# jnbraun/bcnn

Hardware: AMD Instinct MI355X
Metric: images/sec fwd+bwd (higher is better)
Workload: dtype f32; 1 GPU; ResNet-18 224x224 (BASELINE configs[2]), N=128 per GPU, fwd+bwd+SGD through bcnn_net C API; CIFAR-example topology + ImageNet stem, fc-1000; batch_per_gpu=128, global_batch=128, parallelism=dp1, comm=none (one rank)

## Files before the change

bcnn_amd/_lib.py:

```python
import ctypes as C
import os
import subprocess

_HERE = os.path.dirname(os.path.abspath(__file__))
LIB_PATH = os.environ.get("BCNN_HIP_LIB", os.path.join(_HERE, "lib", "libbcnn_hip.so"))
CSRC = os.path.join(_HERE, "csrc")

vp, i, f, sz, u64 = C.c_void_p, C.c_int, C.c_float, C.c_size_t, C.c_uint64

SIGNATURES = {
    "bcnn_hip_device_count": (i, []),
    "bcnn_hip_set_device": (None, [i]),
    "bcnn_hip_get_device": (i, []),
    "bcnn_hip_device_name": (C.c_char_p, []),
    "bcnn_hip_malloc_f32": (vp, [sz]),
    "bcnn_hip_malloc_i32": (vp, [sz]),
    "bcnn_hip_free": (None, [vp]),
    "bcnn_hip_memcpy_h2d": (None, [vp, vp, sz]),
    "bcnn_hip_memcpy_d2h": (None, [vp, vp, sz]),
    "bcnn_hip_memcpy_d2d": (None, [vp, vp, sz]),
    "bcnn_hip_fill_f32": (None, [vp, sz, f]),
    "bcnn_hip_sync": (None, []),
    "bcnn_hip_stream_create": (vp, []),
    "bcnn_hip_stream_destroy": (None, [vp]),
# ... 28 lines not shown
    "bcnn_hip_activation_backward": (None, [vp, vp, sz, i, vp, vp, i, i]),
    "bcnn_hip_activation_forward_keep": (None, [vp, vp, sz, i]),
    "bcnn_hip_activation_backward_from_input": (None, [vp, vp, sz, i]),
    "bcnn_hip_scale_channels_forward": (None, [vp, vp, vp, i, i, i, i]),
    "bcnn_hip_scale_channels_backward": (None, [vp, vp, vp, vp, vp, i, i, i, i]),
    "bcnn_hip_group_norm_forward": (None, [vp] * 6 + [i, i, i, i, f]),
    "bcnn_hip_group_norm_backward": (None, [vp] * 8 + [i, i, i, i, i]),
    "bcnn_hip_group_norm_path": (i, [i, i, i, i, i]),
    "bcnn_hip_batchnorm_forward": (None, [vp] * 10 + [i, i, i, i, i]),
    "bcnn_hip_batchnorm_backward": (None, [vp, vp, vp, i] + [vp] * 9 + [i, i, i]),
    "bcnn_hip_conv_workspace_size": (sz, [i] * 9),
    "bcnn_hip_conv_forward": (None, [vp, vp, vp, vp] + [i] * 10 + [vp, i, vp, vp, vp, vp, vp, vp, vp, i]),
    "bcnn_hip_conv_forward_bf16": (i, [vp, vp, vp, vp] + [i] * 10 + [vp, i, vp, vp, vp, vp, vp, vp, vp, i]),
    "bcnn_hip_conv_backward": (None, [vp] * 8 + [i] * 10 + [vp, vp, i] + [vp] * 8 + [vp, sz]),
    "bcnn_hip_maxpool_forward": (None, [vp, vp, vp] + [i] * 8),
    "bcnn_hip_maxpool_backward": (None, [vp, vp, vp] + [i] * 9),
    "bcnn_hip_avgpool_forward": (None, [vp, vp, i, i, i, i]),
    "bcnn_hip_avgpool_backward": (None, [vp, vp, i, i, i, i]),
    "bcnn_hip_pool2d_out_extent": (i, [vp, i]),
    "bcnn_hip_pool2d_forward": (None, [vp, vp, vp, vp, i, i, i, i]),
    "bcnn_hip_pool2d_backward": (None, [vp, vp, vp, vp, i, i, i, i, i]),
    "bcnn_hip_depthwise_forward": (None, [vp, vp, vp, vp] + [i] * 8),
    "bcnn_hip_depthwise_backward": (None, [vp] * 7 + [i] * 9),
    "bcnn_hip_depthwise_stats_size": (sz, [i] * 7),
    "bcnn_hip_depthwise_forward_stats": (i, [vp, vp, vp, vp] + [i] * 8 + [vp, sz]),
    "bcnn_hip_batchnorm_forward_stats": (None, [vp] * 10 + [i, i, i, i, i, vp, i]),
    "bcnn_hip_batchnorm_forward_stats_only": (None, [vp] * 7 + [i, i, i, vp, i]),
    "bcnn_hip_conv_bnfold_fusable": (i, [i] * 5), "bcnn_hip_conv_set_input_bnfold": (None, [vp] * 4),
    "bcnn_hip_depthwise_bn_fusable": (i, [i] * 8),
    "bcnn_hip_batchnorm_backward_sums": (None, [vp] * 9 + [i, i, i]),
    "bcnn_hip_depthwise_backward_bn": (None, [vp] * 7 + [i] * 9 + [vp] * 5),
    "bcnn_hip_batchnorm_backward_apply": (None, [vp] * 8 + [i, i, i]),
    "bcnn_hip_depthwise_bnin_fusable": (i, [i] * 9),
    "bcnn_hip_conv_bnsums_size": (sz, [i] * 4),
    "bcnn_hip_conv_backward_bnsums": (i, [vp] * 8 + [i] * 10 + [vp, vp, i] + [vp] * 8 + [vp, sz] + [vp, vp, vp, sz]),
    "bcnn_hip_batchnorm_backward_finalize": (None, [vp, i] + [vp] * 6 + [i]),
    "bcnn_hip_depthwise_forward_bnin": (i, [vp, vp, vp, vp] + [i] * 8 + [vp, sz] + [vp] * 4 + [i]),
    "bcnn_hip_depthwise_backward_bnin": (None, [vp] * 7 + [i] * 9 + [vp] * 4 + [i]),
    "bcnn_hip_depthwise_backward_bn_bnin": (None, [vp] * 7 + [i] * 9 + [vp] * 5 + [vp] * 4 + [i]),
    "bcnn_hip_conv_residual_fusable": (i, [i, i, i, i, vp, vp, vp]),
    "bcnn_hip_conv_forward_residual": (None, [vp, vp, vp] + [i] * 9 + [vp] * 7 + [sz, i, vp]),
    "bcnn_hip_conv_backward_residual": (None, [vp] * 7 + [i] * 9 + [vp] * 7 + [vp, sz, vp, vp, i, vp, vp, sz]),
    "bcnn_hip_batchnorm_apply": (None, [vp] * 6 + [i, i, i, i]),
    "bcnn_hip_conv_prepack": (None, [vp, i, i]),
    "bcnn_hip_maxpool_forward_bn_keep": (None, [vp, vp, vp] + [i] * 8 + [vp] * 4 + [i, vp]),
    "bcnn_hip_maxpool_bn_backward_fusable": (i, [i] * 9 + [vp] * 4),
    "bcnn_hip_maxpool_bn_backward": (None, [vp] * 5 + [i] * 8 + [vp] * 8 + [i]),
    "bcnn_hip_conv_backward_bn_done": (None, [vp] * 5 + [i] * 9 + [vp, sz]),
    "bcnn_hip_depthwise_insums_size": (sz, [i] * 7),
    "bcnn_hip_depthwise_backward_bnin_sums": (i, [vp] * 7 + [i] * 9 + [vp] * 5 + [vp] * 4 + [i] + [vp, sz]),
    "bcnn_hip_conv_backward_presummed": (i, [vp] * 8 + [i] * 10 + [vp, vp, i] + [vp] * 8 + [vp, sz] + [vp, i] + [vp, vp, vp, sz]),
    "bcnn_hip_conv_prepack_reset": (None, []),
    "bcnn_hip_conv_prepack_discard": (None, []),
    "bcnn_hip_maxpool_bn_fusable": (i, [i] * 9 + [vp]),
    "bcnn_hip_conv_forward_stats_only": (None, [vp, vp, vp] + [i] * 9 + [vp] * 6),
    "bcnn_hip_maxpool_forward_bn": (None, [vp, vp, vp] + [i] * 8 + [vp] * 4 + [i]),
    "bcnn_hip_sgd_update": (None, [vp, vp, vp, vp, sz, sz, i, f, f, f]),
    "bcnn_hip_sgd_update_chunks": (None, [vp, i, i, f, f, f]),
    "bcnn_hip_zero_chunks": (None, [vp, i]),
    "bcnn_hip_adam_update": (None, [vp, vp, vp, vp, vp, vp, sz, sz, i, i, f, f, f, f, f]),
    "bcnn_hip_eltwise_forward": (None, [vp, vp, vp, sz, sz, i]),
    "bcnn_hip_eltwise_backward": (None, [vp, vp, vp, vp, sz, sz, i, i]),
    "bcnn_hip_cost_metric": (None, [i, vp, vp, vp, i, i, vp]),
    "bcnn_hip_axpy_strided": (None, [i, f, vp, vp] + [i] * 11),
    "bcnn_hip_add_rowvec": (None, [vp, vp, i, i]),
    "bcnn_hip_softmax_forward": (None, [vp, vp, i, i, i]),
    "bcnn_hip_concat_forward": (None, [i, vp, vp, vp, i, i]),
    "bcnn_hip_concat_backward": (None, [i, vp, vp, vp, i, i]),
    "bcnn_hip_upsample_forward": (None, [vp, vp, i, i, i, i, i]),
    "bcnn_hip_upsample_backward": (None, [vp, vp, i, i, i, i, i]),
    "bcnn_hip_yolo_activate": (None, [vp, vp, i, i, i, i, i]),
    "bcnn_hip_yolo_nms_capacity": (i, []),
    "bcnn_hip_yolo_detect_result_words": (sz, [i, i, i]),
    "bcnn_hip_yolo_detect_batch": (i, [vp, i, i, vp, i, i, i, i, f, i, f, i, i, vp]),
    "bcnn_hip_yolo_train_workspace_size": (sz, [vp]),
    "bcnn_hip_yolo_train_forward": (i, [vp, vp, vp, vp, vp, vp, vp]),
    "bcnn_hip_fill_images": (i, [vp, i, i, i, i, i, vp, vp, vp, vp, i, f, i, f, f, f]),
    "bcnn_hip_jpeg_stage_begin": (i, [i, i, i, i, i, vp, i, vp, vp]),
    "bcnn_hip_jpeg_stage_run": (i, [vp, f, i, f, f, f]),
    "bcnn_hip_jpeg_stage_cancel": (None, []),
    "bcnn_hip_augment_batch": (i, [vp, i, i, i, i, i, i, i, vp, vp, vp, i]),
    "bcnn_hip_augment_label_batch": (i, [vp, i, i, i, i, vp, vp, vp, i]),
    "bcnn_hip_augment_jpeg_begin": (i, [i, i, i, i, i, vp, vp]),
    "bcnn_hip_augment_jpeg_run": (i, [vp, vp, vp, vp, vp, vp, i]),
    "bcnn_hip_augment_jpeg_cancel": (None, []),
    "bcnn_hip_augment_letterbox_batch": (i, [vp, i, i, i, i, i, vp, vp, vp, i]),
    "bcnn_hip_augment_effects_begin": (i, [i, i, i, vp, vp, vp, vp, i, vp, sz]),
    "bcnn_hip_augment_effects_cancel": (None, []),
    "bcnn_hip_deconv_workspace_size": (sz, [i] * 8),
    "bcnn_hip_deconv_forward": (None, [vp, vp, vp, vp] + [i] * 9),
    "bcnn_hip_deconv_backward": (None, [vp] * 7 + [i] * 9 + [vp, sz]),
    "bcnn_hip_dilated_conv_workspace_size": (sz, [i] * 10),
    "bcnn_hip_dilated_conv_forward": (None, [vp, vp, vp, vp] + [i] * 11),
    "bcnn_hip_dilated_conv_backward": (None, [vp] * 7 + [i] * 11 + [vp, sz]),
    "bcnn_hip_dilated_depthwise_workspace_size": (sz, [i] * 8),
    "bcnn_hip_dilated_depthwise_forward": (None, [vp, vp, vp, vp] + [i] * 9),
    "bcnn_hip_dilated_depthwise_backward": (None, [vp] * 7 + [i] * 10 + [vp, sz]),
    "bcnn_hip_dilated_depthwise_path": (i, [i] * 9),
    "bcnn_hip_interp_forward": (None, [vp, vp, vp, i, i, i, i]),
    "bcnn_hip_interp_backward": (None, [vp, vp, vp, i, i, i, i, i]),
    "bcnn_hip_interp_axis_taps": (None, [i, i, i, vp, vp, vp]),
    "bcnn_hip_softmax_loss_forward": (None, [vp, vp, vp, vp, vp, i, i, i]),
    "bcnn_hip_softmax_loss_backward": (None, [vp, vp, vp, vp, vp, i, i, i, i]),
    "bcnn_hip_softmax_loss_confusion": (None, [vp, vp, vp, vp, i, i, i]),
    "bcnn_hip_softmax_loss_c_reg": (i, []),
    "bcnn_hip_label_map_fit": (i, [i, i, i, i, i, vp]),
    "bcnn_hip_label_maps_plan": (i, [vp, i, i, i, i, i, vp, vp, vp]),
    "bcnn_hip_label_maps_batch": (i, [vp, i, i, i, i, i, vp, i, vp, vp, vp, vp, i, vp, vp, vp]),
    "bcnn_hip_label_maps_kernel_ms": (f, [i]),
    "bcnn_hip_lrn_forward": (None, [vp, vp] + [i] * 5 + [f] * 3),
    "bcnn_hip_lrn_backward": (None, [vp, vp, vp] + [i] * 5 + [f] * 3 + [i]),
    "bcnn_hip_dropout_forward": (None, [vp, sz, f, u64, u64]),
    "bcnn_hip_dropout_backward": (None, [vp, sz, f, u64, u64]),
    "bcnn_hip_lifted_struct_workspace_size": (sz, [i, i]),
    "bcnn_hip_lifted_struct_forward": (None, [vp, vp, vp, i, i, f, i, vp, vp]),
    "bcnn_hip_lifted_struct_backward": (None, [vp, i, i, f, vp]),
    "bcnn_hip_comm_init": (None, [i, i, C.c_char_p]),
    "bcnn_hip_comm_destroy": (None, []),
    "bcnn_hip_comm_retain": (None, []),
# ... 46 lines not shown
```

bcnn_amd/csrc/blas1.hip:

```cpp
#include "chan_reduce.h"

namespace bcnn_hip {

template <class Op>
__global__ __launch_bounds__(256) void map2_kernel(const float* __restrict__ x, float* __restrict__ y,
                                                   size_t n, Op op) {
    const size_t i = (size_t)blockIdx.x * blockDim.x + threadIdx.x;
    const size_t stride = (size_t)gridDim.x * blockDim.x;
    const bool al = ((reinterpret_cast<uintptr_t>(x) | reinterpret_cast<uintptr_t>(y)) & 15) == 0;
    if (al) {
        const size_t n4 = n / 4;
        const float4* x4 = reinterpret_cast<const float4*>(x);
        float4* y4 = reinterpret_cast<float4*>(y);
        for (size_t j = i; j < n4; j += stride) {
            const float4 a = x4[j];
            float4 b = y4[j];
            b.x = op(a.x, b.x); b.y = op(a.y, b.y); b.z = op(a.z, b.z); b.w = op(a.w, b.w);
            y4[j] = b;
        }
        for (size_t j = n4 * 4 + i; j < n; j += stride) y[j] = op(x[j], y[j]);
    } else {
        for (size_t j = i; j < n; j += stride) y[j] = op(x[j], y[j]);
    }
}
// ... 102 lines not shown
}

__global__ __launch_bounds__(256) void adam_kernel(float* __restrict__ w, float* __restrict__ g,
                                                   float* __restrict__ m, float* __restrict__ v, size_t n, float wd_b,
                                                   float one_m_b1, float b1, float one_m_b2, float b2, float step) {
    const size_t stride = (size_t)gridDim.x * blockDim.x;
    for (size_t i = (size_t)blockIdx.x * blockDim.x + threadIdx.x; i < n; i += stride) {
        float gi = g[i], wi = w[i];
        gi = __fadd_rn(__fmul_rn(wi, wd_b), gi);
        const float mi = __fadd_rn(__fmul_rn(one_m_b1, gi), __fmul_rn(b1, m[i]));
        const float vi = __fadd_rn(__fmul_rn(one_m_b2, __fmul_rn(gi, gi)), __fmul_rn(b2, v[i]));
        m[i] = mi;
        v[i] = vi;
        const float q = __fdiv_rn(mi, __fadd_rn(sqrtf(vi), 0.0000001f));
        w[i] = __fadd_rn(__fmul_rn(q, step), wi);
        g[i] = 0.f;
    }
}

__global__ __launch_bounds__(256) void sgd_chunks_kernel(const bcnn_hip_sgd_chunk* __restrict__ chunks, float wd_b,
                                                         float neg_lr_b, float momentum) {
    const bcnn_hip_sgd_chunk ch = chunks[blockIdx.x];
    const float wd = ch.use_decay ? wd_b : 0.f;
    for (unsigned i = threadIdx.x; i < ch.count; i += 256) {
        float gi = ch.g_d[i], wi = ch.w_d[i];
        if (wd != 0.f) gi = __fadd_rn(__fmul_rn(wi, wd), gi);
        wi = __fadd_rn(__fmul_rn(gi, neg_lr_b), wi);
        ch.w_d[i] = wi;
        ch.g_d[i] = (momentum == 0.0f) ? 0.f : ((momentum == 1.0f) ? gi : gi * momentum);
    }
}

__global__ __launch_bounds__(256) void zero_chunks_kernel(const bcnn_hip_fill_chunk* __restrict__ chunks) {
    const bcnn_hip_fill_chunk ch = chunks[blockIdx.x];
    float* p = ch.p_d;
    const unsigned n = ch.count;
    unsigned head = (unsigned)(((16 - (reinterpret_cast<uintptr_t>(p) & 15)) & 15) / 4);
    if (head > n) head = n;
    if (threadIdx.x < head) p[threadIdx.x] = 0.f;
    float4* b4 = reinterpret_cast<float4*>(p + head);
    const unsigned nb = n - head, n4 = nb / 4;
    for (unsigned j = threadIdx.x; j < n4; j += 256) b4[j] = make_float4(0.f, 0.f, 0.f, 0.f);
    for (unsigned j = n4 * 4 + threadIdx.x; j < nb; j += 256) p[head + j] = 0.f;
}

}

using namespace bcnn_hip;

extern "C" {

void bcnn_hip_axpy(size_t n, float a, const float* x, float* y) {
    if (!n) return;
    map2_kernel<<<stream_grid(n / 4 + 1, 256), 256, 0, current_stream()>>>(x, y, n, AxpyOp{a});
    KERNEL_CHECK();
}

void bcnn_hip_scal(size_t n, float a, float* x) {
    if (!n) return;
    if (a == 0.0f) { HIP_CHECK(hipMemsetAsync(x, 0, n * sizeof(float), current_stream())); return; }
    if (a == 1.0f) return;
    map2_kernel<<<stream_grid(n / 4 + 1, 256), 256, 0, current_stream()>>>((const float*)x, x, n, ScalOp{a});
    KERNEL_CHECK();
}

void bcnn_hip_copy_f32(size_t n, const float* x, float* y) {
    if (!n || x == y) return;
    HIP_CHECK(hipMemcpyAsync(y, x, n * sizeof(float), hipMemcpyDeviceToDevice, current_stream()));
}

void bcnn_hip_add_bias(float* y, const float* bias, int n, int c, int hw) {
    launch_chan_map(ChanMapBody{y, bias, 0, (reinterpret_cast<uintptr_t>(y) & 15) == 0}, n, c, hw);
}

void bcnn_hip_scales(float* y, const float* scales, int n, int c, int hw) {
    launch_chan_map(ChanMapBody{y, scales, 1, (reinterpret_cast<uintptr_t>(y) & 15) == 0}, n, c, hw);
}

void bcnn_hip_grad_bias(float* dbias, const float* g, int n, int c, int hw) {
    const long long M = (long long)n * hw;
    if (!M || !c) return;
    const int splits = chan_splits(c, M);
    float* part = scratch(SCRATCH_REDUCE, (size_t)c * splits);
    if ((reinterpret_cast<uintptr_t>(g) & 15) == 0) launch_chan_reduce<1>(SumF{g}, c, hw, M, splits, part);
    else launch_chan_reduce<1>(SumUnalignedF{g}, c, hw, M, splits, part);
    chan_accumulate_kernel<<<ceil_div(c, 256), 256, 0, current_stream()>>>(part, c, splits, dbias);
    KERNEL_CHECK();
}

}

namespace bcnn_hip {
void activation_backward_grad_bias(const float* y, float* dy, float* dbias, int n, int c, int hw, int act) {
    const long long M = (long long)n * hw;
    if (!M || !c) return;
    const bool al = ((reinterpret_cast<uintptr_t>(y) | reinterpret_cast<uintptr_t>(dy)) & 15) == 0;
    if (act == BCNN_HIP_ACT_NONE || !act_bwd_is_cheap(act) || act == BCNN_HIP_ACT_PRELU || !al) {
        bcnn_hip_activation_backward(y, dy, (size_t)(M * c), act, nullptr, nullptr, hw, c);
        bcnn_hip_grad_bias(dbias, dy, n, c, hw);
        return;
    }
    const int splits = chan_splits(c, M);
    float* part = scratch(SCRATCH_REDUCE, (size_t)c * splits);
    launch_chan_reduce<1>(ActBwdSumF{y, dy, act}, c, hw, M, splits, part);
    chan_accumulate_kernel<<<ceil_div(c, 256), 256, 0, current_stream()>>>(part, c, splits, dbias);
    KERNEL_CHECK();
}
}

extern "C" {

void bcnn_hip_grad_scales(const float* x_norm, const float* g, int n, int c, int hw, float* dscales) {
    const long long M = (long long)n * hw;
    if (!M || !c) return;
    const int splits = chan_splits(c, M);
    float* part = scratch(SCRATCH_REDUCE, (size_t)c * splits);
    if (((reinterpret_cast<uintptr_t>(x_norm) | reinterpret_cast<uintptr_t>(g)) & 15) == 0)
        launch_chan_reduce<1>(DotF{g, x_norm}, c, hw, M, splits, part);
    else launch_chan_reduce<1>(DotUnalignedF{g, x_norm}, c, hw, M, splits, part);
    chan_accumulate_kernel<<<ceil_div(c, 256), 256, 0, current_stream()>>>(part, c, splits, dscales);
// ... 54 lines not shown
```

bcnn_amd/csrc/common.h:

```cpp
#pragma once
#include <hip/hip_runtime.h>

#include <cstdio>
#include <cstdlib>

#include "../../include/bcnn_hip.h"

#define HIP_CHECK(expr)                                                                        \
    do {                                                                                       \
        hipError_t _e = (expr);                                                                \
        if (_e != hipSuccess) {                                                                \
            fprintf(stderr, "[bcnn_hip] %s:%d: %s failed: %s\n", __FILE__, __LINE__, #expr,    \
                    hipGetErrorString(_e));                                                    \
            exit((int)_e);                                                                     \
        }                                                                                      \
    } while (0)

#define KERNEL_CHECK() HIP_CHECK(hipGetLastError())

#ifdef BCNN_HIP_EXPERIMENT
#define BCNN_EXP_ENV(name) getenv(name)
#else
#define BCNN_EXP_ENV(name) ((const char*)nullptr)
#endif

namespace bcnn_hip {

hipStream_t current_stream();
void set_current_stream(hipStream_t st);

constexpr int kMaxDevices = 64;
int current_device();

enum ScratchSlot {
    SCRATCH_REDUCE,
    SCRATCH_BN_CONSTS,
    SCRATCH_FOLD_ROWCONST,
    SCRATCH_COL,
    SCRATCH_DMA,
    SCRATCH_DMA_DW,
    SCRATCH_WINO,
    SCRATCH_WINO_DW,
    SCRATCH_WINO43_U,
    SCRATCH_WINO43_TAIL,
    SCRATCH_WFUSED_U,
    SCRATCH_WFUSED_TAIL,
    SCRATCH_W43FF_U,
    SCRATCH_W43FF_TAIL,
    SCRATCH_DETECT,
    SCRATCH_IMAGES,
    SCRATCH_AUGMENT,
    SCRATCH_INTERP,
    SCRATCH_SOFTMAX_LOSS,
    SCRATCH_AUGMENT_LABEL,
    SCRATCH_LABEL_MAP,
    SCRATCH_SLOTS
};
float* scratch(ScratchSlot slot, size_t floats);
inline float4* scratch_f4(ScratchSlot slot, size_t n) { return reinterpret_cast<float4*>(scratch(slot, n * 4)); }

enum StageSlot {
    STAGE_IMAGES,
    STAGE_AUGMENT,
    STAGE_AUGMENT_LABEL,
    STAGE_LABEL_MAP,
    STAGE_SLOTS
};
uint8_t* host_stage(StageSlot slot, size_t bytes);
uint8_t* host_stage_extend(StageSlot slot, size_t keep, size_t bytes);
uint8_t* stage_upload(StageSlot slot, ScratchSlot device_slot, size_t upload_bytes, size_t device_bytes, hipStream_t st);
uint64_t stage_generation(StageSlot slot);

void activation_backward_grad_bias(const float* y, float* dy, float* dbias, int n, int c, int hw, int act);

enum KClass { K_CONV_FWD = 0, K_CONV_DW, K_CONV_DX, K_BN_FWD, K_BN_BWD, K_POOL, K_ELTWISE_ACT, K_GEMM, K_SGD,
              K_DEPTHWISE_FWD, K_DEPTHWISE_BWD,
              K_CONV_FWD_WINO, K_CONV_DX_WINO, K_CONV_DW_WINO,
              K_CONV_FWD_WINO43, K_CONV_DX_WINO43,
              K_CONV_DW_WINO43,
              K_NUM };
struct KTimer {
    int idx;
    KTimer(int cls, double flops, double bytes, double useful_flops = -1.0);
    ~KTimer();
};

extern thread_local bool g_trace_on;
void trace_kernel_slow(const char* name);
inline void trace_kernel(const char* name) { if (g_trace_on) trace_kernel_slow(name); }
inline void trace_kernel_count(const char* prefix, int count) {
    if (!g_trace_on) return;
    char name[64];
    snprintf(name, sizeof(name), "%s%d", prefix, count);
    trace_kernel_slow(name);
}

constexpr int kWave = 64;
constexpr int kCUs = 256;
constexpr int kXCDs = 8;

inline int ceil_div(long long a, long long b) { return (int)((a + b - 1) / b); }
inline size_t align_up(size_t v, size_t a) { return (v + a - 1) / a * a; }
inline bool al16(const void* p) { return (reinterpret_cast<uintptr_t>(p) & 15) == 0; }

#ifndef STREAM_GRID_PER_CU
#define STREAM_GRID_PER_CU 8
#endif
inline int stream_grid(size_t work_items, int block) {
    size_t need = (work_items + block - 1) / block;
    size_t cap = (size_t)kCUs * STREAM_GRID_PER_CU;
    if (need < 1) need = 1;
    return (int)(need < cap ? need : cap);
}

struct FastDiv {
    unsigned d, magic;
};
inline FastDiv make_fdiv(unsigned d, unsigned long long max_dividend) {
// ... 122 lines not shown
```

bcnn_amd/csrc/conv.hip:

```cpp
#include "batchnorm.h"
#include "conv_paths.h"
#include <algorithm>
#include <cstring>
#include <vector>

namespace bcnn_hip {
static thread_local BnFold g_fold_pending = {nullptr, nullptr, nullptr, nullptr};
static BnFold take_fold() {
    const BnFold f = g_fold_pending;
    g_fold_pending = BnFold{nullptr, nullptr, nullptr, nullptr};
    return f;
}
static bool bnfold_shape_ok(const ConvShape& s) {
    return s.ksz == 1 && s.stride == 1 && s.pad == 0 && s.groups == 1 && conv_dma_fwd_wanted(s) &&
           conv_dw_dma_workspace_floats(s) > 0;
}
__global__ __launch_bounds__(256) void bnfold_rowconst_kernel(const float* __restrict__ w, const BnFold fold, int F, int C,
                                                              float* __restrict__ rowc) {
    const int f = blockIdx.x * 4 + (threadIdx.x >> 6), lane = threadIdx.x & 63;
    if (f >= F) return;
    double acc = 0.0;
    for (int c = lane; c < C; c += 64) {
        float bv = fold.bias[c];
        if (bv == 1.0f) bv = 0.f;
        const float b = bv - fold.mean[c] * bnfold_a(fold.var, fold.scales, c);
        acc += (double)w[(size_t)f * C + c] * (double)b;
    }
#pragma unroll
    for (int o = 32; o > 0; o >>= 1) acc += __shfl_xor(acc, o);
    if (lane == 0) rowc[f] = (float)acc;
}
static float* fold_rowconst(const BnFold& fold, const float* w, int C, int F) {
    float* rowc = scratch(SCRATCH_FOLD_ROWCONST, (size_t)F);
    bnfold_rowconst_kernel<<<ceil_div(F, 4), 256, 0, current_stream()>>>(w, fold, F, C, rowc);
    KERNEL_CHECK();
    return rowc;
}


struct SideStream {
    hipStream_t stream = nullptr;
    hipEvent_t ready = nullptr, done = nullptr;
    bool pending = false;
};
static thread_local SideStream g_side[kMaxDevices];
static thread_local int g_side_mode = 0;
bool conv_side_stream_deferred() { return g_side_mode == 2; }
static SideStream* side_stream() {
    SideStream& ss = g_side[current_device()];
    if (ss.stream == nullptr) {
        int prio_lo = 0, prio_hi = 0;
        HIP_CHECK(hipDeviceGetStreamPriorityRange(&prio_lo, &prio_hi));
        HIP_CHECK(hipStreamCreateWithPriority(&ss.stream, hipStreamNonBlocking, BCNN_EXP_ENV("BCNN_HIP_SIDE_PRIO_SAME") ? prio_hi : prio_lo));
        HIP_CHECK(hipEventCreateWithFlags(&ss.ready, hipEventDisableTiming));
        HIP_CHECK(hipEventCreateWithFlags(&ss.done, hipEventDisableTiming));
    }
    return &ss;
}

struct PrepackEntry {
    const float* w;
    int kind, mode;
    float* buf;
    size_t cap, floats;
    unsigned long long epoch;
    bool fresh;
};
struct PrepackStore {
    std::vector<PrepackEntry> entries;
    unsigned long long epoch = 0;
    int dev = -1;
    void* table_dev[PREPACK_KINDS][2] = {{nullptr, nullptr}, {nullptr, nullptr}};
    size_t table_cap[PREPACK_KINDS][2] = {{0, 0}, {0, 0}};
    std::vector<char> table_host[PREPACK_KINDS][2];
};
static thread_local PrepackStore g_prepack;

float* prepack_take(const float* w, int kind, int mode, size_t floats) {
    PrepackStore& st = g_prepack;
    for (PrepackEntry& e : st.entries)
        if (e.w == w && e.kind == kind && e.mode == mode && e.fresh && e.epoch == st.epoch && e.floats == floats) {
            e.fresh = false;
            return e.buf;
        }
    return nullptr;
}

static void prepack_free_all(PrepackStore& st) {
    HIP_CHECK(hipDeviceSynchronize());
    for (PrepackEntry& e : st.entries)
        if (e.buf) HIP_CHECK(hipFree(e.buf));
    st.entries.clear();
    for (int k = 0; k < PREPACK_KINDS; ++k)
        for (int m = 0; m < 2; ++m) {
            if (st.table_dev[k][m]) HIP_CHECK(hipFree(st.table_dev[k][m]));
            st.table_dev[k][m] = nullptr;
            st.table_cap[k][m] = 0;
            st.table_host[k][m].clear();
        }
}

static PrepackEntry* prepack_entry(PrepackStore& st, const float* w, int kind, int mode, size_t floats) {
    PrepackEntry* e = nullptr;
    for (PrepackEntry& c : st.entries)
        if (c.w == w && c.kind == kind && c.mode == mode) { e = &c; break; }
    if (!e) {
        st.entries.push_back(PrepackEntry{w, kind, mode, nullptr, 0, 0, 0, false});
        e = &st.entries.back();
    }
    if (e->cap < floats) {
        if (e->buf) {
            HIP_CHECK(hipStreamSynchronize(current_stream()));
            HIP_CHECK(hipFree(e->buf));
        }
        HIP_CHECK(hipMalloc((void**)&e->buf, floats * sizeof(float)));
        e->cap = floats;
    }
    e->floats = floats;
    e->epoch = st.epoch;
    e->fresh = true;
    return e;
}

static const void* prepack_table(PrepackStore& st, int kind, int mode, const void* jobs, size_t bytes) {
    std::vector<char>& host = st.table_host[kind][mode];
    if (host.size() == bytes && memcmp(host.data(), jobs, bytes) == 0) return st.table_dev[kind][mode];
    HIP_CHECK(hipStreamSynchronize(current_stream()));
    if (st.table_cap[kind][mode] < bytes) {
        if (st.table_dev[kind][mode]) HIP_CHECK(hipFree(st.table_dev[kind][mode]));
        HIP_CHECK(hipMalloc(&st.table_dev[kind][mode], bytes * 2));
        st.table_cap[kind][mode] = bytes * 2;
    }
    HIP_CHECK(hipMemcpy(st.table_dev[kind][mode], jobs, bytes, hipMemcpyHostToDevice));
    host.assign((const char*)jobs, (const char*)jobs + bytes);
    return st.table_dev[kind][mode];
}

enum ConvGate { GATE_NONE, GATE_WINDOW, GATE_DMA, GATE_SMALLC_DX, GATE_COUNT };
static bool gate_open(ConvGate g) {
    static const bool off[GATE_COUNT] = {false, BCNN_EXP_ENV("BCNN_HIP_NO_WINDOW") != nullptr,
                                         BCNN_EXP_ENV("BCNN_HIP_NO_DMA") != nullptr,
                                         BCNN_EXP_ENV("BCNN_HIP_NO_SMALLC_DX") != nullptr};
    return !off[g];
}
struct ConvPack {
    bool (*wino)(const ConvShape& s, int dx_mode, WinoPackJob* job, size_t* floats);
    bool (*igemm)(const ConvShape& s, int dx_mode, IgemmPackJob* job, size_t* floats);
};
constexpr ConvPack kNoPack = {nullptr, nullptr};
template <class Call>
struct ConvFamily {
    bool (*wanted)(const ConvShape& s, int raw);
    bool (*usable)(const Call& c);
    void (*run)(const Call& c);
    ConvPack pack;
    ConvGate gate;
};
static const ConvFamily<ConvFwdCall> kConvFwdFamilies[] = {
    {conv_window_fwd_wanted, nullptr, conv_forward_window, kNoPack, GATE_WINDOW},
    {conv_stem_fwd_wanted, nullptr, conv_forward_stem, kNoPack, GATE_WINDOW},
    {conv_direct_fwd_wanted, nullptr, conv_forward_direct, kNoPack, GATE_NONE},
    {conv_winograd43_fwd_wanted, conv_winograd43_fwd_usable, conv_forward_winograd43, {wino43_pack_plan, nullptr}, GATE_NONE},
    {conv_winograd_fused_fwd_wanted, nullptr, conv_forward_winograd_fused, {wino_fused_pack_plan, nullptr}, GATE_NONE},
    {conv_winograd_fwd_wanted, nullptr, conv_forward_winograd, kNoPack, GATE_NONE},
    {conv_large_wanted, nullptr, conv_forward_large, kNoPack, GATE_NONE},
    {conv_dma_fwd_wanted, nullptr, conv_forward_dma_timed, {nullptr, dma_pack_plan}, GATE_DMA},
    {conv_small_c_fwd_wanted, nullptr, conv_forward_small_c, kNoPack, GATE_DMA},
    {[](const ConvShape&, int) { return true; }, nullptr, conv_forward_igemm, kNoPack, GATE_NONE},
};
static const ConvFamily<ConvDxCall> kConvDxFamilies[] = {
    {conv_winograd43_dx_wanted, conv_winograd43_dx_usable, conv_backward_data_winograd43, {wino43_pack_plan, nullptr}, GATE_NONE},
    {conv_winograd_fused_dx_wanted, nullptr, conv_backward_data_winograd_fused, {wino_fused_pack_plan, nullptr}, GATE_NONE},
    {conv_winograd_dx_wanted, nullptr, conv_backward_data_winograd, kNoPack, GATE_NONE},
// ... 152 lines not shown
            bcnn_hip_activation_backward(nd.y, nd.dy, ysize, act, nd.slopes, nd.dslopes, s.OHOW, f);
            b.act = BCNN_HIP_ACT_NONE;
        }
        if (nd.own_sums && nd.own_splits > 0 && b.act == act && act_bwd_is_cheap(act)) {
            b.sums = nd.own_sums; b.splits = nd.own_splits;
        }
        batchnorm_backward_impl(b);
    } else {
        bcnn_hip_activation_backward(nd.y, nd.dy, ysize, act, nd.slopes, nd.dslopes, s.OHOW, f);
    }
    SideStream* side = (nd.side_mode == 2 || (nd.side_mode == 1 && nd.dx)) ? side_stream() : nullptr;
    hipStream_t main_stream = current_stream();
    if (side) {
        HIP_CHECK(hipEventRecord(side->ready, main_stream));
        HIP_CHECK(hipStreamWaitEvent(side->stream, side->ready, 0));
        set_current_stream(side->stream);
    }
    bool bias_done = false;
    if (fold.mean) {
        trace_kernel("bnfold:dw");
        KTimer kt(K_CONV_DW, conv_gemm_flops(s), conv_gemm_bytes(s));
        if (!conv_backward_weights_dma(nd.x, nd.dy, nd.dw, s, nd.workspace, nd.workspace_elems, &fold)) {
            fprintf(stderr, "[bcnn_hip] conv backward: the LDS-DMA weight-gradient kernel refused a folded layer\n");
            exit(1);
        }
    } else {
        for (const DwFamily& fam : kDwFamilies)
            if (gate_open(fam.gate) && fam.run(nd.x, nd.dy, nd.dw, batch_norm ? nullptr : nd.g.dbias, s, nd.workspace,
                                               nd.workspace_elems, &bias_done))
                break;
    }
    if (side) {
        HIP_CHECK(hipEventRecord(side->done, side->stream));
        set_current_stream(main_stream);
    }
    if (!batch_norm && !bias_done) bcnn_hip_grad_bias(nd.g.dbias, nd.dy, n, f, s.OHOW);
    if (nd.dx) conv_dx_any(nd.w, nd.dy, nd.dx, s, nd.bs);
    else if (nd.bs) nd.bs->splits = 0;
    if (side) {
        if (nd.side_mode == 2) side->pending = true;
        else HIP_CHECK(hipStreamWaitEvent(main_stream, side->done, 0));
    }
}
static int side_mode_now() {
    static const int side_env = BCNN_EXP_ENV("BCNN_HIP_SIDE_STREAM") ? 1 : 0;
    return g_side_mode ? g_side_mode : side_env;
}
}

using namespace bcnn_hip;

extern "C" {

void bcnn_hip_conv_prepack(const bcnn_hip_conv_desc* layers, int count, int data_gradient) {
    PrepackStore& st = g_prepack;
    int dev = 0;
    HIP_CHECK(hipGetDevice(&dev));
    if (st.dev != dev) {
        if (st.dev >= 0) prepack_free_all(st);
        st.dev = dev;
    }
    ++st.epoch;
    (void)take_fold();
    const int mode = data_gradient ? 1 : 0;
    std::vector<WinoPackJob> wj;
    std::vector<IgemmPackJob> ij;
    int wmax = 0, imax = 0;
    for (int i = 0; i < count; ++i) {
        const bcnn_hip_conv_desc& d = layers[i];
        if (!d.w_d || d.groups <= 0 || d.n <= 0) continue;
        const ConvShape s = make_conv_shape(d.n, d.c, d.h, d.w, d.f, d.k, d.stride, d.pad, d.groups);
        if (s.total_q <= 0 || s.Mg == 0 || s.Cg == 0) continue;
        const ConvPack pack = mode ? conv_planned_pack(kConvDxFamilies, s) : conv_planned_pack(kConvFwdFamilies, s);
        WinoPackJob w1;
        IgemmPackJob i1;
        memset(&w1, 0, sizeof(w1));
        memset(&i1, 0, sizeof(i1));
        size_t floats = 0;
        if (pack.wino && pack.wino(s, mode, &w1, &floats)) {
            PrepackEntry* e = prepack_entry(st, d.w_d, PREPACK_WINO, mode, floats);
            w1.w = d.w_d; w1.u = e->buf;
            if (w1.blocks > wmax) wmax = w1.blocks;
            wj.push_back(w1);
        }
        if (pack.igemm && pack.igemm(s, mode, &i1, &floats)) {
            PrepackEntry* e = prepack_entry(st, d.w_d, PREPACK_IGEMM, mode, floats);
            i1.w = d.w_d; i1.at = e->buf;
            const int blocks = i1.gx * i1.gy * i1.gz;
            if (blocks > imax) imax = blocks;
            ij.push_back(i1);
        }
    }
    if (!wj.empty()) {
        const void* t = prepack_table(st, PREPACK_WINO, mode, wj.data(), wj.size() * sizeof(WinoPackJob));
        wino_fused_pack_launch((const WinoPackJob*)t, (int)wj.size(), wmax);
    }
    if (!ij.empty()) {
        const void* t = prepack_table(st, PREPACK_IGEMM, mode, ij.data(), ij.size() * sizeof(IgemmPackJob));
        dma_pack_launch((const IgemmPackJob*)t, (int)ij.size(), imax);
    }
}

void bcnn_hip_conv_prepack_discard(void) { ++g_prepack.epoch; }

void bcnn_hip_conv_prepack_reset(void) {
    PrepackStore& st = g_prepack;
    if (st.dev < 0) return;
    prepack_free_all(st);
    ++st.epoch;
}

size_t bcnn_hip_conv_workspace_size(int n, int c, int h, int w, int f, int k, int stride, int pad, int groups) {
    const ConvShape s = make_conv_shape(n, c, h, w, f, k, stride, pad, groups);
    size_t m = 0;
    for (const DwFamily& fam : kDwFamilies) m = std::max(m, fam.workspace_floats(s));
    return m;
}

int bcnn_hip_conv_bnfold_fusable(int n, int c, int h, int wd, int f) {
    if (n <= 0 || c <= 0 || h <= 0 || wd <= 0 || f <= 0) return 0;
    return bnfold_shape_ok(make_conv_shape(n, c, h, wd, f, 1, 1, 0, 1)) ? 1 : 0;
}

void bcnn_hip_conv_set_input_bnfold(const float* mean, const float* var, const float* scales, const float* bias) {
    g_fold_pending = BnFold{mean, var, scales, bias};
}

void bcnn_hip_conv_forward(const float* x, const float* w, const float* bias, float* y, int n, int c, int h,
                           int wd, int f, int k, int stride, int pad, int groups, int act, const float* slopes,
                           int batch_norm, float* run_mean, float* run_var, const float* scales,
                           float* saved_mean, float* saved_var, float* x_norm, float* bn_workspace, int mode) {
    ConvNodeFwd nd{};
    nd.s = make_conv_shape(n, c, h, wd, f, k, stride, pad, groups); nd.fold = take_fold();
    nd.x = x; nd.w = w; nd.y = y; nd.act = act; nd.slopes = slopes; nd.batch_norm = batch_norm; nd.mode = mode;
    nd.p.scales = scales; nd.p.bias = bias; nd.saved_mean = saved_mean; nd.saved_var = saved_var;
    nd.run.run_mean = run_mean; nd.run.run_var = run_var; nd.bn_workspace = bn_workspace;
    conv_forward_impl(nd);
}

int bcnn_hip_conv_forward_bf16(const float* x, const float* w, const float* bias, float* y, int n, int c, int h,
                               int wd, int f, int k, int stride, int pad, int groups, int act, const float* slopes,
                               int batch_norm, float* run_mean, float* run_var, const float* scales,
                               float* saved_mean, float* saved_var, float* x_norm, float* bn_workspace, int mode) {
    if (mode != BCNN_HIP_MODE_PREDICT && mode != BCNN_HIP_MODE_VALID) return 0;
    ConvNodeFwd nd{};
    nd.s = make_conv_shape(n, c, h, wd, f, k, stride, pad, groups); nd.fold = take_fold(); nd.bf16 = true;
    nd.x = x; nd.w = w; nd.y = y; nd.act = act; nd.slopes = slopes; nd.batch_norm = batch_norm; nd.mode = mode;
    nd.p.scales = scales; nd.p.bias = bias; nd.saved_mean = saved_mean; nd.saved_var = saved_var;
    nd.run.run_mean = run_mean; nd.run.run_var = run_var; nd.bn_workspace = bn_workspace;
    conv_forward_impl(nd);
    return 1;
}

// ... 127 lines not shown
```

bcnn_amd/csrc/gemm.hip:

```cpp
#include "conv_common.h"
#include "chan_reduce.h"

namespace bcnn_hip {

struct GemmArgs {
    const float* A;
    const float* B;
    float* C;
    int m, n, k;
    long long ars, acs, brs, bcs;
    int ldc;
    float alpha, beta;
    float* partials;
    int tiles_per_split;
};

__global__ __launch_bounds__(256) void gemm_kernel(const GemmArgs a) {
    constexpr int BM = 64, BN = 64, BK = 16;
    __shared__ float As[2][BK][BM + 1];
    __shared__ float Bs[2][BK][BN + 1];
    const int tid = threadIdx.x, lane = tid & 63, wid = tid >> 6;
    const int wm = wid >> 1, wn = wid & 1;
    const int i0 = blockIdx.y * BM, j0 = blockIdx.x * BN;
    const int nk_all = (a.k + BK - 1) / BK;
// ... 5 lines not shown
    const int ars_i = a_kc ? 16 : 0, aks_i = a_kc ? 0 : 4, brs_i = b_kc ? 16 : 0, bks_i = b_kc ? 0 : 4;
    float ra[4], rb[4];
    auto load = [&](int kt) {
#pragma unroll
        for (int i = 0; i < 4; ++i) {
            const int la = (kt0 + kt) * BK + ak + aks_i * i, rowa = i0 + ar + ars_i * i;
            const int lb = (kt0 + kt) * BK + bk + bks_i * i, rowb = j0 + br + brs_i * i;
            ra[i] = (rowa < a.m && la < a.k) ? a.A[(long long)rowa * a.ars + (long long)la * a.acs] : 0.f;
            rb[i] = (rowb < a.n && lb < a.k) ? a.B[(long long)lb * a.brs + (long long)rowb * a.bcs] : 0.f;
        }
    };
    auto store = [&](int buf) {
#pragma unroll
        for (int i = 0; i < 4; ++i) {
            As[buf][ak + aks_i * i][ar + ars_i * i] = ra[i];
            Bs[buf][bk + bks_i * i][br + brs_i * i] = rb[i];
        }
    };
    f32x16 acc;
#pragma unroll
    for (int q = 0; q < 16; ++q) acc[q] = 0.f;
    load(0);
    store(0);
    __syncthreads();
    const int l31 = lane & 31, lhi = lane >> 5;
    for (int kt = 0; kt < nk; ++kt) {
        const int cur = kt & 1;
        if (kt + 1 < nk) load(kt + 1);
#pragma unroll
        for (int ks = 0; ks < BK / 2; ++ks)
            acc = mfma32(As[cur][2 * ks + lhi][wm * 32 + l31], Bs[cur][2 * ks + lhi][wn * 32 + l31], acc);
        if (kt + 1 < nk) store(cur ^ 1);
        __syncthreads();
    }
    const int j = j0 + wn * 32 + l31;
    if (j < a.n) {
#pragma unroll
        for (int q = 0; q < 16; ++q) {
            const int i = i0 + wm * 32 + mfma_row(q, lane);
            if (i >= a.m) continue;
            if (gridDim.z > 1) {
                a.partials[((long long)blockIdx.z * a.m + i) * a.n + j] = acc[q];
                continue;
            }
            float* cp = a.C + (long long)i * a.ldc + j;
            float v = a.alpha * acc[q];
            if (a.beta != 0.0f) v += a.beta * (*cp);
            *cp = v;
        }
    }
}

__global__ __launch_bounds__(256) void gemm_splitk_finalize_kernel(const float* __restrict__ partials, int splits, float* C,
                                                                   int m, int n, int ldc, float alpha, float beta) {
    const long long total = (long long)m * n, stride = (long long)gridDim.x * blockDim.x;
    for (long long e = (long long)blockIdx.x * blockDim.x + threadIdx.x; e < total; e += stride) {
        float sum = partials[e];
        for (int sp = 1; sp < splits; ++sp) sum += partials[(long long)sp * total + e];
        float* cp = C + (e / n) * ldc + (e % n);
        float v = alpha * sum;
        if (beta != 0.0f) v += beta * (*cp);
        *cp = v;
    }
}

__global__ __launch_bounds__(256) void gemm_scale_kernel(float* C, int m, int n, int ldc, float beta) {
    const long long total = (long long)m * n, stride = (long long)gridDim.x * blockDim.x;
    for (long long i = (long long)blockIdx.x * blockDim.x + threadIdx.x; i < total; i += stride) {
        float* p = C + (i / n) * ldc + (i % n);
        *p = (beta == 0.0f) ? 0.f : (*p) * beta;
    }
}

__global__ __launch_bounds__(256) void im2col_kernel(const float* __restrict__ im, float* __restrict__ col, int C,
                                                     int H, int W, int ksz, int pad, int stride, int OH,
                                                     int OW, unsigned total) {
    const unsigned gs = gridDim.x * blockDim.x;
    for (unsigned i = blockIdx.x * blockDim.x + threadIdx.x; i < total; i += gs) {
        const unsigned ow = i % (unsigned)OW, t = i / (unsigned)OW;
        const unsigned oh = t % (unsigned)OH, row = t / (unsigned)OH;
        const int kc = (int)(row % (unsigned)ksz), kr = (int)((row / (unsigned)ksz) % (unsigned)ksz);
        const int c = (int)(row / (unsigned)(ksz * ksz));
        const int ih = (int)oh * stride - pad + kr, iw = (int)ow * stride - pad + kc;
        col[i] = ((unsigned)ih < (unsigned)H && (unsigned)iw < (unsigned)W) ? im[(c * H + ih) * W + iw] : 0.f;
    }
}

__global__ __launch_bounds__(256) void col2im_kernel(const float* __restrict__ col, float* __restrict__ im, int C,
                                                     int H, int W, int ksz, int pad, int stride, int OH,
                                                     int OW, unsigned total) {
    const unsigned gs = gridDim.x * blockDim.x;
    for (unsigned i = blockIdx.x * blockDim.x + threadIdx.x; i < total; i += gs) {
        const int iw = (int)(i % (unsigned)W), t = (int)(i / (unsigned)W);
        const int ih = t % H, c = t / H;
        float acc = 0.f;
        for (int kr = 0; kr < ksz; ++kr) {
            const int th = ih + pad - kr;
            if (th < 0 || th % stride) continue;
            const int oh = th / stride;
            if (oh >= OH) continue;
            for (int kc = 0; kc < ksz; ++kc) {
                const int tw = iw + pad - kc;
                if (tw < 0 || tw % stride) continue;
                const int ow = tw / stride;
                if (ow >= OW) continue;
                acc += col[(((long long)c * ksz + kr) * ksz + kc) * OH * OW + oh * OW + ow];
            }
        }
        im[i] = acc;
    }
}

}

using namespace bcnn_hip;

extern "C" {

void bcnn_hip_gemm(int ta, int tb, int m, int n, int k, float alpha, const float* A, int lda, const float* B,
                   int ldb, float beta, float* C, int ldc) {
    if (m <= 0 || n <= 0) return;
    if (k <= 0 || alpha == 0.0f) {
        if (beta != 1.0f) {
            gemm_scale_kernel<<<stream_grid((size_t)m * n, 256), 256, 0, current_stream()>>>(C, m, n, ldc, beta);
            KERNEL_CHECK();
        }
        return;
    }
    GemmArgs a;
    a.A = A; a.B = B; a.C = C; a.m = m; a.n = n; a.k = k; a.ldc = ldc; a.alpha = alpha; a.beta = beta;
    a.ars = ta ? 1 : lda; a.acs = ta ? lda : 1;
    a.brs = tb ? 1 : ldb; a.bcs = tb ? ldb : 1;
    const int tiles = ceil_div(n, 64) * ceil_div(m, 64), ktiles = ceil_div(k, 16);
    int splits = 1;
    if (tiles < kCUs / 2 && ktiles >= 16) {
        splits = (2 * kCUs) / tiles;
        if (splits > ktiles / 4) splits = ktiles / 4;
        if (splits > 32) splits = 32;
        if (splits < 1) splits = 1;
    }
    a.tiles_per_split = ceil_div(ktiles, splits);
    splits = ceil_div(ktiles, a.tiles_per_split);
    a.partials = splits > 1 ? scratch(SCRATCH_REDUCE, (size_t)splits * m * n) : nullptr;
    dim3 grid((unsigned)ceil_div(n, 64), (unsigned)ceil_div(m, 64), (unsigned)splits);
    gemm_kernel<<<grid, 256, 0, current_stream()>>>(a);
    KERNEL_CHECK();
    if (splits > 1) {
        gemm_splitk_finalize_kernel<<<stream_grid((size_t)m * n, 256), 256, 0, current_stream()>>>(a.partials, splits, C, m, n, ldc,
                                                                                                alpha, beta);
        KERNEL_CHECK();
    }
}

void bcnn_hip_im2col(const float* im, int channels, int height, int width, int ksize, int pad, int stride,
                     float* col) {
    const int oh = (height + 2 * pad - ksize) / stride + 1, ow = (width + 2 * pad - ksize) / stride + 1;
    if (oh <= 0 || ow <= 0) return;
    const long long total = (long long)channels * ksize * ksize * oh * ow;
    if (total <= 0) return;
    im2col_kernel<<<stream_grid((size_t)total, 256), 256, 0, current_stream()>>>(
        im, col, channels, height, width, ksize, pad, stride, oh, ow, (unsigned)total);
    KERNEL_CHECK();
}

void bcnn_hip_col2im(const float* col, int channels, int height, int width, int ksize, int pad, int stride,
                     float* im) {
    const int oh = (height + 2 * pad - ksize) / stride + 1, ow = (width + 2 * pad - ksize) / stride + 1;
    const long long total = (long long)channels * height * width;
    if (total <= 0) return;
    col2im_kernel<<<stream_grid((size_t)total, 256), 256, 0, current_stream()>>>(
        col, im, channels, height, width, ksize, pad, stride, oh, ow, (unsigned)total);
    KERNEL_CHECK();
}

}
```

bcnn_amd/csrc/next.hip:

```cpp
#include <cfloat>

#include "chan_reduce.h"
#include "common.h"

namespace bcnn_hip {

__global__ __launch_bounds__(256) void axpy_strided_kernel(float a, const float* __restrict__ x, float* __restrict__ y,
                                                           int sy, int sx, int xc, int xh, int xw, int yc, int yh,
                                                           int yw, int mc, int mh, int mw, unsigned total) {
    const unsigned gs = gridDim.x * blockDim.x;
    for (unsigned t = blockIdx.x * blockDim.x + threadIdx.x; t < total; t += gs) {
        const unsigned i = t % (unsigned)mw, t1 = t / (unsigned)mw;
        const unsigned j = t1 % (unsigned)mh, t2 = t1 / (unsigned)mh;
        const unsigned k = t2 % (unsigned)mc, n = t2 / (unsigned)mc;
        const size_t di = (size_t)i * sy + (size_t)yw * ((size_t)j * sy + (size_t)yh * ((size_t)yc * n + k));
        const size_t si = (size_t)i * sx + (size_t)xw * ((size_t)j * sx + (size_t)xh * ((size_t)xc * n + k));
        y[di] += a * x[si];
    }
}

__global__ __launch_bounds__(256) void add_rowvec_kernel(float* __restrict__ y, const float* __restrict__ v, int cols,
                                                         unsigned total) {
    const unsigned gs = gridDim.x * blockDim.x;
    for (unsigned t = blockIdx.x * blockDim.x + threadIdx.x; t < total; t += gs) y[t] += v[t % (unsigned)cols];
// ... 94 lines not shown
    double acc = 0.0;
    if (metric == 0) {
        for (int i = row0; i < B; i += nrow) {
            const float* row = pred + (size_t)i * per;
            float pm = FLT_MIN;
            int best = 0;
            for (int j = lane; j < per; j += 64)
                if (row[j] > pm) { pm = row[j]; best = j; }
#pragma unroll
            for (int off = 32; off > 0; off >>= 1) {
                const float om = __shfl_xor(pm, off);
                const int ob = __shfl_xor(best, off);
                if (om > pm || (om == pm && ob < best)) { pm = om; best = ob; }
            }
            if (lane == 0 && label[(size_t)i * per + best] == 0) acc += 1.0;
        }
    } else if (metric == 5) {
        for (int i = row0; i < B; i += nrow) {
            int n = 0, d = 0;
            for (int j = lane; j < per; j += 64) {
                const float l = label[(size_t)i * per + j];
                const float t = pred[(size_t)i * per + j] > 0.5f ? 1.f : 0.f;
                n += (int)(l * t);
                d += (int)(l + t);
            }
#pragma unroll
            for (int off = 32; off > 0; off >>= 1) { n += __shfl_xor(n, off); d += __shfl_xor(d, off); }
            if (lane == 0) acc += (2.0f * n + 1.0f) / (d + 1.0f);
        }
    } else {
        const size_t sz = (size_t)B * per;
        for (size_t i = (size_t)blockIdx.x * 1024 + threadIdx.x; i < sz; i += (size_t)gridDim.x * 1024) {
            if (metric == 1) {
                if (label[i] > 0.0f) {
                    float q = pred[i];
                    q = q < 1e-8f ? 1e-8f : (q > 1.0f - 1e-8f ? 1.0f - 1e-8f : q);
                    acc += -log((double)q);
                }
            } else {
                acc += (double)grad[i] * grad[i];
            }
        }
#pragma unroll
        for (int off = 32; off > 0; off >>= 1) acc += __shfl_xor(acc, off);
    }
    if (lane == 0) red[wave] = acc;
    __syncthreads();
    if (threadIdx.x == 0) {
        double t = 0.0;
        for (int w = 0; w < 16; ++w) t += red[w];
        partials[blockIdx.x] = t;
    }
}
__global__ void cost_metric_final_kernel(int metric, const double* __restrict__ partials, int n, int per,
                                         float* __restrict__ out) {
    double t = 0.0;
    for (int i = 0; i < n; ++i) t += partials[i];
    out[0] = (float)(metric == 3 ? t / per : t);
}

}

using namespace bcnn_hip;

extern "C" {

void bcnn_hip_axpy_strided(int num_batches, float a, const float* x, float* y, int stride_y, int stride_x, int x_c,
                           int x_h, int x_w, int y_c, int y_h, int y_w, int min_c, int min_h, int min_w) {
    const long long total = (long long)num_batches * min_c * min_h * min_w;
    if (total <= 0) return;
    axpy_strided_kernel<<<stream_grid((size_t)total, 256), 256, 0, current_stream()>>>(
        a, x, y, stride_y, stride_x, x_c, x_h, x_w, y_c, y_h, y_w, min_c, min_h, min_w, (unsigned)total);
    KERNEL_CHECK();
}

void bcnn_hip_add_rowvec(float* y, const float* v, int rows, int cols) {
    const long long total = (long long)rows * cols;
    if (total <= 0) return;
    add_rowvec_kernel<<<stream_grid((size_t)total, 256), 256, 0, current_stream()>>>(y, v, cols, (unsigned)total);
    KERNEL_CHECK();
}

void bcnn_hip_softmax_forward(const float* x, float* y, int n, int c, int hw) {
    const long long total = (long long)n * hw;
    if (total <= 0) return;
    softmax_kernel<<<stream_grid((size_t)total * 64, 256), 256, 0, current_stream()>>>(x, y, c, hw, (unsigned)total);
    KERNEL_CHECK();
}

static bool aligned16(const void* p) { return p == nullptr || (reinterpret_cast<uintptr_t>(p) & 15) == 0; }

void bcnn_hip_eltwise_forward(const float* a, const float* b, float* y, size_t n, size_t b_count, int act) {
    if (!n) return;
    if (!act_is_cheap(act) || !aligned16(a) || !aligned16(b) || !aligned16(y)) {
        bcnn_hip_copy_f32(n, a, y);
        bcnn_hip_axpy(b_count, 1.0f, b, y);
        bcnn_hip_activation_forward(y, n, act, nullptr, 1, 1);
        return;
    }
    eltwise_fwd_kernel<<<stream_grid(n / 4 + 1, 256), 256, 0, current_stream()>>>(a, b, y, n, b_count, act);
    KERNEL_CHECK();
}

void bcnn_hip_eltwise_backward(const float* y, float* dy, float* da, float* db, size_t n, size_t b_count, int act,
                               int overwrite_a) {
    if (!n) return;
    if (!act_bwd_is_cheap(act) || !aligned16(y) || !aligned16(dy) || !aligned16(da) || !aligned16(db)) {
        bcnn_hip_activation_backward(y, dy, n, act, nullptr, nullptr, 1, 1);
        if (da && overwrite_a) bcnn_hip_fill_f32(da, n, 0.f);
        if (da) bcnn_hip_axpy(n, 1.0f, dy, da);
        if (db) bcnn_hip_axpy(b_count, 1.0f, dy, db);
        return;
    }
    eltwise_bwd_kernel<<<stream_grid(n / 4 + 1, 256), 256, 0, current_stream()>>>(y, dy, da, db, n, b_count, act,
                                                                                   overwrite_a);
    KERNEL_CHECK();
}

void bcnn_hip_cost_metric(int metric, const float* pred, const float* label, const float* grad, int batch, int per,
                          float* out) {
    const long long sz = (long long)batch * per;
    int blocks = (int)((sz + 8191) / 8192);
    if (blocks > 64) blocks = 64;
    if (blocks < 1) blocks = 1;
    double* partials = reinterpret_cast<double*>(scratch(SCRATCH_REDUCE, 2 * 64));
    cost_metric_kernel<<<blocks, 1024, 0, current_stream()>>>(metric, pred, label, grad, batch, per, partials);
    KERNEL_CHECK();
    cost_metric_final_kernel<<<1, 1, 0, current_stream()>>>(metric, partials, blocks, per, out);
    KERNEL_CHECK();
}

}
```

bcnn_amd/csrc/runtime.hip:

```cpp
#include "common.h"

#include <cstring>
#include <vector>

namespace bcnn_hip {
static thread_local hipStream_t g_stream = nullptr;
hipStream_t current_stream() { return g_stream; }
void set_current_stream(hipStream_t st) { g_stream = st; }

int current_device() {
    int dev = 0;
    HIP_CHECK(hipGetDevice(&dev));
    if (dev < 0 || dev >= kMaxDevices) { fprintf(stderr, "[bcnn_hip] device ordinal %d out of range\n", dev); exit(1); }
    return dev;
}

struct ScratchPolicy { size_t min_floats; unsigned grow_num, grow_den; };
static constexpr ScratchPolicy kScratchPolicy[] = {
     {1u << 16, 2, 1},
     {4096 * 4, 2, 1},
     {8192, 2, 1},
     {0, 1, 1},
     {1u << 20, 3, 2},
     {1u << 20, 3, 2},
// ... 158 lines not shown
int bcnn_hip_device_count(void) {
    int n = 0;
    if (hipGetDeviceCount(&n) != hipSuccess) return 0;
    return n;
}

void bcnn_hip_set_device(int id) {
    HIP_CHECK(hipSetDevice(id));
    warm_device_keeping_rand_state();
}

int bcnn_hip_get_device(void) {
    int id = 0;
    HIP_CHECK(hipGetDevice(&id));
    return id;
}

const char* bcnn_hip_device_name(void) {
    static thread_local char name[256];
    hipDeviceProp_t prop;
    HIP_CHECK(hipGetDeviceProperties(&prop, bcnn_hip_get_device()));
    snprintf(name, sizeof(name), "%s", prop.gcnArchName);
    return name;
}

float* bcnn_hip_malloc_f32(size_t n) {
    float* p = nullptr;
    if (n == 0) return nullptr;
    warm_device_keeping_rand_state();
    HIP_CHECK(hipMalloc((void**)&p, n * sizeof(float)));
    HIP_CHECK(hipMemsetAsync(p, 0, n * sizeof(float), current_stream()));
    return p;
}

int* bcnn_hip_malloc_i32(size_t n) {
    int* p = nullptr;
    if (n == 0) return nullptr;
    warm_device_keeping_rand_state();
    HIP_CHECK(hipMalloc((void**)&p, n * sizeof(int)));
    HIP_CHECK(hipMemsetAsync(p, 0, n * sizeof(int), current_stream()));
    return p;
}

void bcnn_hip_free(void* p) {
    if (p) HIP_CHECK(hipFree(p));
}

void bcnn_hip_memcpy_h2d(void* dst, const void* src, size_t bytes) {
    HIP_CHECK(hipMemcpyAsync(dst, src, bytes, hipMemcpyHostToDevice, current_stream()));
    HIP_CHECK(hipStreamSynchronize(current_stream()));
}

void bcnn_hip_memcpy_d2h(void* dst, const void* src, size_t bytes) {
    HIP_CHECK(hipMemcpyAsync(dst, src, bytes, hipMemcpyDeviceToHost, current_stream()));
    HIP_CHECK(hipStreamSynchronize(current_stream()));
}

void bcnn_hip_memcpy_d2d(void* dst, const void* src, size_t bytes) {
    HIP_CHECK(hipMemcpyAsync(dst, src, bytes, hipMemcpyDeviceToDevice, current_stream()));
}

void bcnn_hip_fill_f32(float* x, size_t n, float value) {
    if (n == 0) return;
    if (value == 0.0f) {
        HIP_CHECK(hipMemsetAsync(x, 0, n * sizeof(float), current_stream()));
        return;
    }
    fill_f32_kernel<<<stream_grid(n / 4 + 1, 256), 256, 0, current_stream()>>>(x, n, value);
    KERNEL_CHECK();
}

void bcnn_hip_sync(void) { HIP_CHECK(hipStreamSynchronize(current_stream())); }

void* bcnn_hip_stream_create(void) {
    hipStream_t s;
    warm_device_keeping_rand_state();
    int prio_lo = 0, prio_hi = 0;
    HIP_CHECK(hipDeviceGetStreamPriorityRange(&prio_lo, &prio_hi));
    HIP_CHECK(hipStreamCreateWithPriority(&s, hipStreamNonBlocking, prio_hi));
    return (void*)s;
}

void bcnn_hip_stream_destroy(void* stream) {
    if (stream) HIP_CHECK(hipStreamDestroy((hipStream_t)stream));
}

void bcnn_hip_set_stream(void* stream) { g_stream = (hipStream_t)stream; }
void* bcnn_hip_get_stream(void) { return (void*)g_stream; }

void* bcnn_hip_event_create(void) {
    hipEvent_t e;
    HIP_CHECK(hipEventCreate(&e));
    return (void*)e;
}

void bcnn_hip_event_destroy(void* ev) {
    if (ev) HIP_CHECK(hipEventDestroy((hipEvent_t)ev));
}

void bcnn_hip_event_record(void* ev) { HIP_CHECK(hipEventRecord((hipEvent_t)ev, current_stream())); }
void bcnn_hip_event_sync(void* ev) { HIP_CHECK(hipEventSynchronize((hipEvent_t)ev)); }

float bcnn_hip_event_elapsed_ms(void* start, void* stop) {
    float ms = 0.f;
    HIP_CHECK(hipEventElapsedTime(&ms, (hipEvent_t)start, (hipEvent_t)stop));
    return ms;
}

// ... 62 lines not shown
```

bcnn_amd/host/bcnn_core.c:

```c
#include <math.h>
#include <stdarg.h>
#include <string.h>

#include "bcnn_internal.h"
#include "../../include/bcnn_hip.h"

#ifndef BCNN_USE_HIP
#error "this runtime is the device build: compile with -DBCNN_USE_HIP"
#endif

void bcnn_log(bcnn_log_context ctx, bcnn_log_level level, const char *fmt, ...) {
    if (level < ctx.lvl) return;
    char msg[2048];
    va_list ap;
    va_start(ap, fmt);
    vsnprintf(msg, sizeof(msg), fmt, ap);
    va_end(ap);
    if (ctx.fct) {
        ctx.fct("%s", msg);
        return;
    }
    static const char *tag[] = {"[INFO] ", "[WARNING] ", "[ERROR] ", ""};
    fprintf(stderr, "%s%s", tag[level > 3 ? 3 : level], msg);
}
// ... 198 lines not shown
    p->inputs = (int *)calloc(1, sizeof(int));
    p->num_threads = 1;
    *net = p;
    return BCNN_SUCCESS;
}

void bcnn_end_net(bcnn_net **pnet) {
    bcnn_net *net = *pnet;
    if (!net) return;
    bcnn_hip_sync();
    bcnn_hip_conv_prepack_reset();
    bcnn_hip_context *hc = hctx(net);
    if (hc->comm_active) bcnn_hip_comm_destroy();
    if (hc->compiled) {
        for (int i = 0; i < hc->arena_members; ++i) {
            bcnn_tensor *t = &net->tensors[hc->param_ids[i]];
            t->data_gpu = NULL;
            t->grad_data_gpu = NULL;
        }
        bcnn_hip_free(hc->param_arena_gpu);
        bcnn_hip_free(hc->grad_arena_gpu);
        bcnn_hip_free(hc->sgd_chunks_gpu);
        bcnn_hip_free(hc->fill_chunks_gpu);
        free(hc->sgd_chunks_host);
        free(hc->grad_fill_dead);
        free(hc->node_grad_first);
    }
    for (int i = 0; i < net->num_nodes; ++i) {
        bcnn_node *nd = &net->nodes[i];
        if (nd->release_param) nd->release_param(nd);
        free(nd->src); free(nd->dst); free(nd->param);
    }
    free(net->nodes);
    for (int i = 0; i < net->num_tensors; ++i) bcnn_tensor_destroy(&net->tensors[i]);
    free(net->tensors);
    bcnn_hip_free(hc->workspace_gpu);
    bcnn_free_loader_stage(net);
    free(hc->param_ids);
    free(hc);
    free(net->learner); free(net->data_aug); bcnn_destroy_data_loader(net); free(net->inputs);
    free(net);
    *pnet = NULL;
}

bcnn_status bcnn_set_num_threads(bcnn_net *net, int num_threads, const int *cpu_ids) {
    (void)cpu_ids;
    net->num_threads = num_threads > 0 ? num_threads : 1;
    return BCNN_SUCCESS;
}
int bcnn_get_num_threads(bcnn_net *net) { return net->num_threads; }
int bcnn_get_batch_size(bcnn_net *net) { return net->batch_size; }

void bcnn_set_input_shape(bcnn_net *net, int width, int height, int channels, int batch_size) {
    net->batch_size = batch_size;
    bcnn_tensor_set_shape(&net->tensors[0], batch_size, channels, height, width, 0);
}

bcnn_status bcnn_add_input(bcnn_net *net, int width, int height, int channels, const char *name) {
    bcnn_tensor t = {0};
    bcnn_tensor_set_shape(&t, net->batch_size, channels, height, width, 0);
    BCNN_CHECK_STATUS(bcnn_tensor_allocate(&t, net->mode));
    t.name = dup_name(name);
    BCNN_CHECK_STATUS(bcnn_net_add_tensor(net, t));
    int *p = (int *)realloc(net->inputs, (size_t)(net->num_inputs + 1) * sizeof(int));
    if (!p) return BCNN_FAILED_ALLOC;
    net->inputs = p;
    net->inputs[net->num_inputs++] = net->num_tensors - 1;
    return BCNN_SUCCESS;
}

static void build_arenas(bcnn_net *net) {
    bcnn_hip_context *hc = hctx(net);
    size_t total = 0;
    for (int i = 0; i < hc->num_params; ++i) {
        total += ((size_t)bcnn_tensor_size(&net->tensors[hc->param_ids[i]]) + 3) & ~(size_t)3;
    }
    if (total == 0) return;
    float *old_p = hc->param_arena_gpu, *old_g = hc->grad_arena_gpu;
    float *new_p = bcnn_hip_malloc_f32(total);
    float *new_g = (net->mode != BCNN_MODE_PREDICT) ? bcnn_hip_malloc_f32(total) : NULL;
    size_t off = 0;
    for (int i = 0; i < hc->num_params; ++i) {
        bcnn_tensor *t = &net->tensors[hc->param_ids[i]];
        const size_t sz = (size_t)bcnn_tensor_size(t);
        const int member = i < hc->arena_members;
        bcnn_hip_memcpy_d2d(new_p + off, t->data_gpu, sz * sizeof(float));
        bcnn_hip_sync();
        if (!member) bcnn_hip_free(t->data_gpu);
        t->data_gpu = new_p + off;
        if (new_g && t->grad_data_gpu) {
            bcnn_hip_memcpy_d2d(new_g + off, t->grad_data_gpu, sz * sizeof(float));
            bcnn_hip_sync();
            if (!member) bcnn_hip_free(t->grad_data_gpu);
            t->grad_data_gpu = new_g + off;
        }
        off += (sz + 3) & ~(size_t)3;
    }
    bcnn_hip_free(old_p);
    bcnn_hip_free(old_g);
    hc->param_arena_gpu = new_p;
    hc->grad_arena_gpu = new_g;
    hc->arena_size = total;
    hc->arena_members = hc->num_params;
}

static void mark_dead_grad_fills(bcnn_net *net) {
// ... 35 lines not shown
        if (nd->type == BCNN_LAYER_BATCHNORM) {
            hc->grad_fill_dead[t] = 1;
            continue;
        }
        if (nd->type != BCNN_LAYER_CONV2D) continue;
        const bcnn_conv_param *p = (const bcnn_conv_param *)nd->param;
        const bcnn_tensor *x = &net->tensors[t], *y = &net->tensors[nd->dst[0]];
        if (p->size == 1 && y->h * y->w != x->h * x->w) continue;
        hc->grad_fill_dead[t] = 1;
    }
}

int bcnn_grad_sole_writer(bcnn_net *net, int tensor) {
    const bcnn_hip_context *hc = hctx(net);
    return hc->grad_fill_dead && tensor >= 0 && tensor < hc->grad_fill_count && hc->grad_fill_dead[tensor] == 2;
}

static void comm_sync_parameters(bcnn_net *net);

bcnn_status bcnn_compile_net(bcnn_net *net) {
    bcnn_hip_context *hc = hctx(net);
    BCNN_CHECK_STATUS(bcnn_tensor_allocate(&net->tensors[0], net->mode));
    size_t need = 0;
    for (int i = 0; i < net->num_nodes; ++i) {
        if (net->nodes[i].type != BCNN_LAYER_CONV2D) continue;
        bcnn_conv_param *p = (bcnn_conv_param *)net->nodes[i].param;
        const bcnn_tensor *s = &net->tensors[net->nodes[i].src[0]];
        const size_t ws = bcnn_hip_conv_workspace_size(s->n, s->c, s->h, s->w, p->num, p->size, p->stride, p->pad,
                                                       p->num_groups);
        if (ws > need) need = ws;
    }
    if (need > hc->workspace_size) {
        bcnn_hip_free(hc->workspace_gpu);
        hc->workspace_gpu = bcnn_hip_malloc_f32(need);
        hc->workspace_size = need;
    }
    for (int i = 0; i < net->num_nodes; ++i)
        if (net->nodes[i].type == BCNN_LAYER_CONV2D)
            ((bcnn_conv_param *)net->nodes[i].param)->conv_workspace_gpu = hc->workspace_gpu;
    if (!hc->compiled || hc->num_params != hc->arena_members) {
        invalidate_sgd_table(net);
        build_arenas(net);
        hc->compiled = 1;
        if (hc->grad_ready_fn) bcnn_set_gradient_ready_callback(net, hc->grad_ready_fn, hc->grad_ready_user);
        comm_sync_parameters(net);
    }
    relink_graph(net);
    bcnn_hip_sync();
    return BCNN_SUCCESS;
}

static void relink_graph(bcnn_net *net) {
    bcnn_hip_context *hc = hctx(net);
    mark_dead_grad_fills(net);
    for (int i = 0; i < net->num_nodes; ++i) {
        if (net->nodes[i].type != BCNN_LAYER_CONV2D) continue;
        const int t = net->nodes[i].dst[0];
        int rewritten = 0;
        for (int j = 0; j < net->num_nodes; ++j)
            rewritten |= net->nodes[j].type == BCNN_LAYER_DROPOUT && net->nodes[j].dst[0] == t;
        ((bcnn_conv_param *)net->nodes[i].param)->out_rewritten = rewritten;
    }
    bcnn_link_depthwise_batchnorm(net);
    bcnn_link_conv_eltwise(net);
    bcnn_link_conv_maxpool(net);
    bcnn_link_conv_depthwise(net);
    bcnn_link_batchnorm_conv(net);
    if (hc->fill_chunks_gpu) {
        bcnn_hip_sync();
        bcnn_hip_free(hc->fill_chunks_gpu);
        hc->fill_chunks_gpu = NULL;
    }
    hc->num_fill_chunks = -1;
}

bcnn_status bcnn_reserve_device(void **buf, size_t *capacity, size_t elems, size_t elem_size, int may_grow) {
    if (!*buf || elems <= *capacity) return BCNN_SUCCESS;
    if (!may_grow) return BCNN_INVALID_PARAMETER;
    bcnn_hip_sync();
    bcnn_hip_free(*buf);
    *buf = bcnn_hip_malloc_f32((elems * elem_size + sizeof(float) - 1) / sizeof(float));
    *capacity = *buf ? elems : 0;
    return *buf ? BCNN_SUCCESS : BCNN_FAILED_ALLOC;
}

static bcnn_status node_reserve_buffers(const bcnn_node *nd, const bcnn_tensor *d, int may_grow) {
    size_t elems = (size_t)bcnn_tensor_size(d);
#define RESERVE(T, buf, cap) \
    bcnn_reserve_device((void **)&((T *)nd->param)->buf, &((T *)nd->param)->cap, elems, sizeof(*((T *)nd->param)->buf), may_grow)
    if (nd->type == BCNN_LAYER_GROUPNORM) {
        elems = 2 * (size_t)d->n * (size_t)((const bcnn_groupnorm_param *)nd->param)->num_groups;
        return RESERVE(bcnn_groupnorm_param, stats_gpu, stats_capacity);
    }
    switch (nd->type) {
        case BCNN_LAYER_CONV2D: return RESERVE(bcnn_conv_param, bn_workspace_gpu, bn_workspace_capacity);
        case BCNN_LAYER_BATCHNORM: return RESERVE(bcnn_batchnorm_param, workspace_gpu, workspace_capacity);
        case BCNN_LAYER_POOL2D: return RESERVE(bcnn_pool2d_param, indexes_gpu, indexes_capacity);
        case BCNN_LAYER_ACTIVATION: return RESERVE(bcnn_activation_param, x_saved_gpu, x_saved_capacity);
        case BCNN_LAYER_MAXPOOL:
            BCNN_CHECK_STATUS(RESERVE(bcnn_maxpool_param, indexes_gpu, indexes_capacity));
            return RESERVE(bcnn_maxpool_param, raw_at_max_gpu, raw_at_max_capacity);
        default: return BCNN_SUCCESS;
    }
#undef RESERVE
}

static int keeps_producer_shape(const bcnn_node *nd) {
    return nd->type == BCNN_LAYER_DROPOUT ||
           (nd->type == BCNN_LAYER_ACTIVATION && bcnn_act_needs_input(((const bcnn_activation_param *)nd->param)->activation));
}

static int node_dst_shape(const bcnn_node *nd, const bcnn_tensor *s, bcnn_tensor *d) {
    int oc = s->c, oh = s->h, ow = s->w;
    if (nd->type == BCNN_LAYER_CONV2D) {
        const bcnn_conv_param *p = (const bcnn_conv_param *)nd->param;
        oc = p->num;
        oh = (s->h + 2 * p->pad - p->size) / p->stride + 1;
        ow = (s->w + 2 * p->pad - p->size) / p->stride + 1;
    } else if (nd->type == BCNN_LAYER_MAXPOOL) {
        const bcnn_maxpool_param *p = (const bcnn_maxpool_param *)nd->param;
// ... 40 lines not shown
                           nd->type != BCNN_LAYER_SOFTMAX_LOSS || need_realloc ||
                               (size_t)d->n * d->h * d->w <= ((const bcnn_softmax_loss_param *)nd->param)->label_capacity,
                           BCNN_INVALID_PARAMETER,
                           "bcnn_resize_net: the label map of softmax-loss node %d would outgrow its allocation; call with "
                           "need_realloc\n", i);
    }
    return BCNN_SUCCESS;
}

static bcnn_status resize_commit(bcnn_net *net, int w, int h, int c, int need_realloc) {
    bcnn_set_input_shape(net, w, h, c, 1);
    for (int i = 0; i < net->num_nodes; ++i) {
        const bcnn_node *nd = &net->nodes[i];
        if (nd->num_src < 1 || nd->num_dst < 1) continue;
        bcnn_tensor *d = &net->tensors[nd->dst[0]];
        if (!keeps_producer_shape(nd)) {
            node_dst_shape(nd, &net->tensors[nd->src[0]], d);
            if (need_realloc && bcnn_tensor_allocate(d, net->mode) != BCNN_SUCCESS) return BCNN_FAILED_ALLOC;
        }
        if (nd->type == BCNN_LAYER_SOFTMAX_LOSS) {
            bcnn_softmax_loss_param *p = (bcnn_softmax_loss_param *)nd->param;
            bcnn_tensor *label = &net->tensors[1];
            bcnn_tensor_set_shape(label, d->n, 1, d->h, d->w, 0);
            if (need_realloc) {
                if (bcnn_tensor_allocate(label, net->mode) != BCNN_SUCCESS) return BCNN_FAILED_ALLOC;
                p->label_capacity = (size_t)d->n * d->h * d->w;
            }
        }
        if (!need_realloc) continue;
        if (node_reserve_buffers(nd, d, 1) != BCNN_SUCCESS) return BCNN_FAILED_ALLOC;
        if (nd->type == BCNN_LAYER_MAXPOOL) {
            bcnn_maxpool_param *p = (bcnn_maxpool_param *)nd->param;
            int *host = (int *)realloc(p->indexes, p->indexes_capacity * sizeof(int));
            if (!host) return BCNN_FAILED_ALLOC;
            p->indexes = host;
        }
    }
    return BCNN_SUCCESS;
}

bcnn_status bcnn_resize_net(bcnn_net *net, int w, int h, int c, int need_realloc) {
    if (!net || net->num_tensors < 1 || w <= 0 || h <= 0 || c <= 0) return BCNN_INVALID_PARAMETER;
    bcnn_tensor *plan = (bcnn_tensor *)malloc((size_t)net->num_tensors * sizeof(*plan));
    if (!plan) return BCNN_FAILED_ALLOC;
    const bcnn_status planned = resize_plan(net, w, h, c, need_realloc, plan);
    free(plan);
    BCNN_CHECK_STATUS(planned);
    BCNN_CHECK_STATUS(resize_commit(net, w, h, c, need_realloc));
    return hctx(net)->compiled ? bcnn_compile_net(net) : BCNN_SUCCESS;
}

bcnn_status bcnn_set_mode(bcnn_net *net, bcnn_mode mode) {
    if (net->mode == mode) return BCNN_SUCCESS;
    if (mode == BCNN_MODE_TRAIN && !hctx(net)->detector_training)
        for (int i = 0; i < net->num_nodes; ++i)
            BCNN_CHECK_AND_LOG(net->log_ctx, net->nodes[i].type != BCNN_LAYER_YOLOV3, BCNN_INVALID_PARAMETER,
                               "bcnn_set_mode: the net holds a YOLO node, whose TRAIN-mode loss is not built\n");
    if (mode == BCNN_MODE_TRAIN)
        BCNN_CHECK_AND_LOG(net->log_ctx, bcnn_yolo_heads_trainable(net), BCNN_INVALID_PARAMETER,
                           "bcnn_set_mode: a YOLO node was built without detector training or has no gradient buffer\n");
    net->mode = mode;
    if (net->data_loader) bcnn_switch_data_handles(net, net->data_loader);
    return BCNN_SUCCESS;
}

static void build_fill_table(bcnn_net *net) {
    bcnn_hip_context *hc = hctx(net);
    int cap = 256, n = 0;
    bcnn_hip_fill_chunk *tab = (bcnn_hip_fill_chunk *)malloc((size_t)cap * sizeof(*tab));
    unsigned char *seen = (unsigned char *)calloc((size_t)net->num_tensors + 1, 1);
    for (int i = 0; i < net->num_nodes; ++i)
        for (int d = 0; d < net->nodes[i].num_dst; ++d) {
            const int id = net->nodes[i].dst[d];
            bcnn_tensor *t = &net->tensors[id];
            if (seen[id] || !t->grad_data_gpu) continue;
            seen[id] = 1;
            if (hc->grad_fill_dead && id < hc->grad_fill_count && hc->grad_fill_dead[id]) continue;
            const size_t sz = (size_t)bcnn_tensor_size(t);
            for (size_t off = 0; off < sz; off += BCNN_HIP_FILL_CHUNK) {
                if (n == cap) {
                    cap *= 2;
                    tab = (bcnn_hip_fill_chunk *)realloc(tab, (size_t)cap * sizeof(*tab));
                }
                tab[n].p_d = t->grad_data_gpu + off;
                tab[n].count = (unsigned int)((sz - off < BCNN_HIP_FILL_CHUNK) ? (sz - off) : BCNN_HIP_FILL_CHUNK);
                tab[n].reserved = 0;
                ++n;
            }
        }
    free(seen);
    hc->num_fill_chunks = n;
    if (n > 0) {
        hc->fill_chunks_gpu = bcnn_hip_malloc_f32(((size_t)n * sizeof(*tab) + 3) / 4);
        bcnn_hip_memcpy_h2d(hc->fill_chunks_gpu, tab, (size_t)n * sizeof(*tab));
    }
    free(tab);
}

void bcnn_forward(bcnn_net *net) {
    bcnn_hip_context *hc = hctx(net);
    if (net->mode == BCNN_MODE_TRAIN) {
        if (hc->num_fill_chunks < 0) build_fill_table(net);
        bcnn_hip_zero_chunks((const bcnn_hip_fill_chunk *)hc->fill_chunks_gpu, hc->num_fill_chunks);
    }
    bcnn_drop_pending_gradients(net);
    bcnn_prepack_conv_weights(net, 0);
    hc->in_pass = 1;
    for (int i = 0; i < net->num_nodes; ++i) net->nodes[i].forward(net, &net->nodes[i]);
    hc->in_pass = 0;
    bcnn_hip_conv_prepack_discard();
}

static void comm_flush(bcnn_hip_context *hc) {
    if (hc->comm_lo < hc->comm_hi) {
        bcnn_hip_allreduce_sum(hc->grad_arena_gpu + hc->comm_lo, hc->comm_hi - hc->comm_lo);
        hc->comm_hi = hc->comm_lo;
    }
}

static void comm_on_ready(size_t first, size_t count, void *user) {
    bcnn_hip_context *hc = (bcnn_hip_context *)user;
    (void)count;
    hc->comm_lo = first;
    if (hc->comm_hi - hc->comm_lo >= hc->comm_bucket) comm_flush(hc);
}

void bcnn_backward(bcnn_net *net) {
    bcnn_hip_context *hc = hctx(net);
    size_t ready_from = hc->arena_size;
    if (hc->comm_active) hc->comm_lo = hc->comm_hi = hc->arena_size;
    bcnn_prepack_conv_weights(net, 1);
    hc->in_pass = 2;
    const int side_prev = bcnn_hip_conv_side_stream_mode((hc->no_side_stream || BCNN_EXP_ENV("BCNN_NO_SIDE_STREAM")) ? 0 : 2);
    for (int i = net->num_nodes - 1; i >= 0; --i) {
        net->nodes[i].backward(net, &net->nodes[i]);
        if (hc->grad_ready_fn && hc->node_grad_first && hc->node_grad_first[i] < ready_from) {
            bcnn_hip_conv_side_join();
            hc->grad_ready_fn(hc->node_grad_first[i], ready_from - hc->node_grad_first[i], hc->grad_ready_user);
            ready_from = hc->node_grad_first[i];
        }
    }
    hc->in_pass = 0;
    bcnn_hip_conv_side_join();
    bcnn_hip_conv_side_stream_mode(side_prev);
    bcnn_hip_conv_prepack_discard();
    if (hc->grad_ready_fn && ready_from > 0 && hc->arena_size > 0)
        hc->grad_ready_fn(0, ready_from, hc->grad_ready_user);
    if (hc->comm_active) {
        comm_flush(hc);
        bcnn_hip_comm_join();
    }
}

void bcnn_set_weight_gradient_stream(bcnn_net *net, int enable) { hctx(net)->no_side_stream = enable ? 0 : 1; }

bcnn_status bcnn_set_inference_precision(bcnn_net *net, bcnn_precision p) {
    if (!net || (p != BCNN_PRECISION_FP32 && p != BCNN_PRECISION_BF16)) return BCNN_INVALID_PARAMETER;
    hctx(net)->inference_precision = (int)p;
    return BCNN_SUCCESS;
}

bcnn_precision bcnn_get_inference_precision(const bcnn_net *net) {
    return (bcnn_precision)((const bcnn_hip_context *)net->hip_ctx)->inference_precision;
}

bcnn_status bcnn_set_loader_on_device(bcnn_net *net, int on) {
    if (!net) return BCNN_INVALID_PARAMETER;
    hctx(net)->loader_on_device = on ? 1 : 0;
    return BCNN_SUCCESS;
}

int bcnn_get_loader_on_device(const bcnn_net *net) {
    return net ? ((const bcnn_hip_context *)net->hip_ctx)->loader_on_device : 0;
}

bcnn_status bcnn_set_loader_decode_on_device(bcnn_net *net, int on) {
    if (!net) return BCNN_INVALID_PARAMETER;
    hctx(net)->loader_decode_on_device = on ? 1 : 0;
    return BCNN_SUCCESS;
}

int bcnn_get_loader_decode_on_device(const bcnn_net *net) {
    return net ? ((const bcnn_hip_context *)net->hip_ctx)->loader_decode_on_device : 0;
}
// ... 61 lines not shown
        hc->node_grad_first[i] = first;
    }
}

static void step_learning_rate(bcnn_net *net) {
    bcnn_learner *ln = net->learner;
    const int global_batch = net->batch_size * hctx(net)->dp_world;
    ln->seen += global_batch;
    const int iter = ln->seen / global_batch;
    switch (ln->decay_type) {
        case BCNN_LR_DECAY_STEP:
            ln->learning_rate = ln->base_learning_rate * (float)pow(ln->scale, iter / ln->step);
            break;
        case BCNN_LR_DECAY_INV:
            ln->learning_rate = ln->base_learning_rate * (float)pow(1.0f + ln->gamma * iter, -ln->power);
            break;
        case BCNN_LR_DECAY_EXP:
            ln->learning_rate = ln->base_learning_rate * (float)pow(ln->gamma, iter);
            break;
        case BCNN_LR_DECAY_POLY:
            ln->learning_rate = ln->base_learning_rate * (float)pow(1 - (float)iter / ln->max_batches, ln->power);
            break;
        case BCNN_LR_DECAY_SIGMOID:
            ln->learning_rate = ln->base_learning_rate * (1.0f / (1.0f + (float)exp(ln->gamma * (iter - ln->step))));
            break;
        default:
            break;
    }
}

static void sgd_table_add(bcnn_hip_context *hc, float *w, float *g, size_t n, int use_decay) {
    for (size_t off = 0; off < n; off += BCNN_HIP_SGD_CHUNK) {
        if (hc->num_sgd_chunks == hc->cap_sgd_chunks) {
            hc->cap_sgd_chunks = hc->cap_sgd_chunks ? 2 * hc->cap_sgd_chunks : 1024;
            hc->sgd_chunks_host = (bcnn_hip_sgd_chunk *)realloc(hc->sgd_chunks_host,
                                                                (size_t)hc->cap_sgd_chunks * sizeof(bcnn_hip_sgd_chunk));
        }
        bcnn_hip_sgd_chunk *c = &hc->sgd_chunks_host[hc->num_sgd_chunks++];
        c->w_d = w + off;
        c->g_d = g + off;
        c->count = (unsigned int)((n - off < BCNN_HIP_SGD_CHUNK) ? (n - off) : BCNN_HIP_SGD_CHUNK);
        c->use_decay = (unsigned int)use_decay;
    }
}

static int update_is_tabled(const bcnn_node *nd) {
    return nd->update == bcnn_update_conv_layer || nd->update == bcnn_update_depthwise_conv_layer ||
           nd->update == bcnn_update_fullc_layer || nd->update == bcnn_update_deconv_layer ||
           nd->update == bcnn_update_dilated_conv_layer || nd->update == bcnn_update_dilated_depthwise_layer;
}

void bcnn_update(bcnn_net *net) {
    bcnn_hip_context *hc = hctx(net);
    step_learning_rate(net);
    if (net->learner->optimizer == BCNN_OPTIM_ADAM) {
        for (int i = 0; i < net->num_nodes; ++i)
            if (net->nodes[i].update) net->nodes[i].update(net, &net->nodes[i]);
        return;
    }
    if (hc->sgd_chunks_gpu == NULL) {
        hc->sgd_collecting = 1;
        hc->num_sgd_chunks = 0;
        for (int i = 0; i < net->num_nodes; ++i)
            if (net->nodes[i].update && update_is_tabled(&net->nodes[i])) net->nodes[i].update(net, &net->nodes[i]);
        hc->sgd_collecting = 0;
        if (hc->num_sgd_chunks > 0) {
            hc->sgd_chunks_gpu = bcnn_hip_malloc_f32(((size_t)hc->num_sgd_chunks * sizeof(bcnn_hip_sgd_chunk) + 3) / 4);
            bcnn_hip_memcpy_h2d(hc->sgd_chunks_gpu, hc->sgd_chunks_host,
                                (size_t)hc->num_sgd_chunks * sizeof(bcnn_hip_sgd_chunk));
        }
    }
    const bcnn_learner *ln = net->learner;
    if (hc->num_sgd_chunks > 0)
        bcnn_hip_sgd_update_chunks((const bcnn_hip_sgd_chunk *)hc->sgd_chunks_gpu, hc->num_sgd_chunks,
                                   net->batch_size * hc->dp_world, ln->learning_rate,
                                   ln->momentum / (float)hc->dp_world, ln->decay);
    for (int i = 0; i < net->num_nodes; ++i)
        if (net->nodes[i].update && !update_is_tabled(&net->nodes[i])) net->nodes[i].update(net, &net->nodes[i]);
}

void bcnn_node_sgd_step(bcnn_net *net, bcnn_tensor *weights, bcnn_tensor *biases) {
    const bcnn_learner *ln = net->learner;
    const int world = hctx(net)->dp_world;
    if (hctx(net)->sgd_collecting) {
        if (biases && biases->data_gpu && biases->grad_data_gpu)
            sgd_table_add(hctx(net), biases->data_gpu, biases->grad_data_gpu, (size_t)bcnn_tensor_size(biases), 0);
        if (weights && weights->data_gpu && weights->grad_data_gpu)
            sgd_table_add(hctx(net), weights->data_gpu, weights->grad_data_gpu, (size_t)bcnn_tensor_size(weights), 1);
        return;
    }
    bcnn_hip_sgd_update(weights ? weights->data_gpu : NULL, biases ? biases->data_gpu : NULL,
                        weights ? weights->grad_data_gpu : NULL, biases ? biases->grad_data_gpu : NULL,
                        weights ? (size_t)bcnn_tensor_size(weights) : 0, biases ? (size_t)bcnn_tensor_size(biases) : 0,
                        net->batch_size * world, ln->learning_rate, ln->momentum / (float)world, ln->decay);
}

void bcnn_node_optim_step(bcnn_net *net, bcnn_tensor *weights, bcnn_tensor *biases, float **adam_m_gpu,
                          float **adam_v_gpu) {
    const bcnn_learner *ln = net->learner;
    if (ln->optimizer != BCNN_OPTIM_ADAM || adam_m_gpu == NULL) {
        bcnn_node_sgd_step(net, weights, biases);
        return;
    }
    const int world = hctx(net)->dp_world;
    const size_t wsz = (size_t)bcnn_tensor_size(weights);
    if (*adam_m_gpu == NULL) {
// ... 18 lines not shown
            loss += ((const bcnn_yolo_param *)net->nodes[i].param)->cost[0];
            ++n;
        } else if (net->nodes[i].type == BCNN_LAYER_SOFTMAX_LOSS) {
            loss += bcnn_softmax_loss_read_loss(net, &net->nodes[i]);
            ++n;
        }
    return n ? loss / n : 0.f;
}

static void next_batch_or_die(bcnn_net *net) {
    const bcnn_status st = bcnn_loader_next(net);
    if (st != BCNN_SUCCESS) {
        fprintf(stderr, "[bcnn] the data loader could not fill a batch (status %d)\n", (int)st);
        exit(1);
    }
}

float bcnn_train_on_batch(bcnn_net *net) {
    next_batch_or_die(net);
    bcnn_forward(net);
    bcnn_backward(net);
    bcnn_update(net);
    return current_loss(net);
}

float bcnn_predict_on_batch(bcnn_net *net, bcnn_tensor **out) {
    next_batch_or_die(net);
    bcnn_forward(net);
    const bcnn_node *last = &net->nodes[net->num_nodes - 1];
    const int out_id = (last->type == BCNN_LAYER_COST) ? last->src[0] : last->dst[0];
    bcnn_tensor *t = &net->tensors[out_id];
    bcnn_hip_memcpy_d2h(t->data, t->data_gpu, (size_t)bcnn_tensor_size(t) * sizeof(float));
    *out = t;
    return current_loss(net);
}

int bcnn_get_tensor_index_by_name(bcnn_net *net, const char *name) { return bcnn_net_find_tensor(net, name); }

bcnn_tensor *bcnn_get_tensor_by_index(bcnn_net *net, int index) {
    if (index < 0 || index >= net->num_tensors) return NULL;
    bcnn_download_tensor(net, index, 1);
    return &net->tensors[index];
}

bcnn_tensor *bcnn_get_tensor_by_name(bcnn_net *net, const char *name) {
    return bcnn_get_tensor_by_index(net, bcnn_net_find_tensor(net, name));
}

bcnn_status bcnn_upload_tensor(bcnn_net *net, int index, int with_grad) {
    if (index < 0 || index >= net->num_tensors) return BCNN_INVALID_PARAMETER;
    bcnn_tensor *t = &net->tensors[index];
    const size_t bytes = (size_t)bcnn_tensor_size(t) * sizeof(float);
    bcnn_materialize_data(net, index);
    if (t->data && t->data_gpu) bcnn_hip_memcpy_h2d(t->data_gpu, t->data, bytes);
    if (with_grad) bcnn_materialize_gradients(net, -1);
    if (with_grad && t->grad_data && t->grad_data_gpu) bcnn_hip_memcpy_h2d(t->grad_data_gpu, t->grad_data, bytes);
    return BCNN_SUCCESS;
}

bcnn_status bcnn_fill_tensor_with_images(bcnn_net *net, int tensor_index, int num_images, const uint8_t *const *images,
                                         const int *widths, const int *heights, const int *strides, int c,
                                         bcnn_image_fit fit, float norm_coeff, int swap_to_bgr, float mean_r,
                                         float mean_g, float mean_b) {
    BCNN_CHECK_AND_LOG(net->log_ctx, tensor_index >= 0 && tensor_index < net->num_tensors, BCNN_INVALID_PARAMETER,
                       "Fill with images: invalid tensor index %d\n", tensor_index);
    bcnn_tensor *t = &net->tensors[tensor_index];
    BCNN_CHECK_AND_LOG(net->log_ctx, t->data_gpu != NULL, BCNN_INVALID_PARAMETER,
                       "Fill with images: tensor %d has no device buffer\n", tensor_index);
    BCNN_CHECK_AND_LOG(net->log_ctx, num_images >= 1 && num_images <= t->n, BCNN_INVALID_PARAMETER,
                       "Fill with images: %d images for a batch of %d\n", num_images, t->n);
    BCNN_CHECK_AND_LOG(net->log_ctx, c == t->c && c >= 1 && c <= 4, BCNN_INVALID_PARAMETER,
                       "Fill with images: %d channels (tensor: %d; supported: 1 to 4)\n", c, t->c);
    BCNN_CHECK_AND_LOG(net->log_ctx, images && widths && heights, BCNN_INVALID_PARAMETER,
                       "Fill with images: NULL images, widths or heights\n");
    BCNN_CHECK_AND_LOG(net->log_ctx, fit == BCNN_IMAGE_FIT_STRETCH || fit == BCNN_IMAGE_FIT_LETTERBOX,
                       BCNN_INVALID_PARAMETER, "Fill with images: unknown fit %d\n", (int)fit);
    for (int b = 0; b < num_images; ++b) {
        BCNN_CHECK_AND_LOG(net->log_ctx, images[b] && widths[b] >= 1 && heights[b] >= 1, BCNN_INVALID_PARAMETER,
                           "Fill with images: image %d is NULL or has an extent below 1\n", b);
        BCNN_CHECK_AND_LOG(net->log_ctx, !strides || (long long)strides[b] >= (long long)widths[b] * c,
                           BCNN_INVALID_PARAMETER, "Fill with images: image %d: stride %d below width * channels\n", b,
                           strides[b]);
    }
    bcnn_materialize_data(net, tensor_index);
    if (bcnn_hip_fill_images(t->data_gpu, t->n, t->c, t->h, t->w, num_images, images, widths, heights, strides, (int)fit,
                             norm_coeff, swap_to_bgr, mean_r, mean_g, mean_b) != 0)
        BCNN_ERROR(net->log_ctx, BCNN_INVALID_PARAMETER,
                   "Fill with images: an image does not fit the %d x %d input (letterbox extent of 0, or more than 2 GiB "
                   "to stage)\n", t->w, t->h);
    return BCNN_SUCCESS;
}

bcnn_status bcnn_download_tensor(bcnn_net *net, int index, int with_grad) {
    if (index < 0 || index >= net->num_tensors) return BCNN_INVALID_PARAMETER;
    bcnn_tensor *t = &net->tensors[index];
    const size_t bytes = (size_t)bcnn_tensor_size(t) * sizeof(float);
    bcnn_materialize_data(net, index);
    if (t->data && t->data_gpu) bcnn_hip_memcpy_d2h(t->data, t->data_gpu, bytes);
    if (with_grad) bcnn_materialize_gradients(net, index);
    if (with_grad && t->grad_data && t->grad_data_gpu) bcnn_hip_memcpy_d2h(t->grad_data, t->grad_data_gpu, bytes);
    return BCNN_SUCCESS;
}

bcnn_tensor *bcnn_peek_tensor(bcnn_net *net, int index) {
    return (index < 0 || index >= net->num_tensors) ? NULL : &net->tensors[index];
}

int bcnn_get_num_nodes(bcnn_net *net) { return net->num_nodes; }

int bcnn_get_node_tensor(bcnn_net *net, int node, int is_dst, int slot) {
    if (node < 0 || node >= net->num_nodes || slot < 0) return -1;
    const bcnn_node *nd = &net->nodes[node];
    if (is_dst) return slot < nd->num_dst ? nd->dst[slot] : -1;
    return slot < nd->num_src ? nd->src[slot] : -1;
}

int bcnn_get_node_type(bcnn_net *net, int node) {
    return (node < 0 || node >= net->num_nodes) ? -1 : (int)net->nodes[node].type;
}

int bcnn_get_node_activation(bcnn_net *net, int node) {
    if (node < 0 || node >= net->num_nodes) return -1;
    const bcnn_node *nd = &net->nodes[node];
    if (nd->type == BCNN_LAYER_DILATED_CONV2D)
        return (int)((const bcnn_dilated_conv_param *)nd->param)->activation;
    if (nd->type == BCNN_LAYER_DILATED_DEPTHWISE_CONV2D)
        return (int)((const bcnn_dilated_depthwise_param *)nd->param)->activation;
    switch (nd->type) {
        case BCNN_LAYER_CONV2D: return (int)((const bcnn_conv_param *)nd->param)->activation;
        case BCNN_LAYER_TRANSPOSE_CONV2D: return (int)((const bcnn_deconv_param *)nd->param)->activation;
        case BCNN_LAYER_DEPTHWISE_CONV2D: return (int)((const bcnn_depthwise_conv_param *)nd->param)->activation;
        case BCNN_LAYER_ACTIVATION: return (int)((const bcnn_activation_param *)nd->param)->activation;
        case BCNN_LAYER_FULL_CONNECTED: return (int)((const bcnn_fullc_param *)nd->param)->activation;
        case BCNN_LAYER_ELTWISE: return (int)((const bcnn_eltwise_param *)nd->param)->activation;
        default: return -1;
    }
}
// ... 14 lines not shown
    } else if (nd->type == BCNN_LAYER_BATCHNORM) {
        sm = &((bcnn_batchnorm_param *)nd->param)->saved_mean;
        sv = &((bcnn_batchnorm_param *)nd->param)->saved_variance;
    }
    if (!sm) return NULL;
    if (which == 5) {
        if (nd->type == BCNN_LAYER_CONV2D) return ((bcnn_conv_param *)nd->param)->bn_workspace_gpu;
        const bcnn_batchnorm_param *bp = (const bcnn_batchnorm_param *)nd->param;
        return (bp->input_kept || !bp->workspace_gpu) ? net->tensors[nd->src[0]].data_gpu : bp->workspace_gpu;
    }
    switch (which) {
        case 1: return sm->data_gpu;
        case 2: return sv->data_gpu;
        case 3: return sm->grad_data_gpu;
        case 4: return sv->grad_data_gpu;
    }
    return NULL;
}

bcnn_status bcnn_forward_node(bcnn_net *net, int node) {
    if (node < 0 || node >= net->num_nodes || !net->nodes[node].forward) return BCNN_INVALID_PARAMETER;
    bcnn_materialize_data(net, -1);
    net->nodes[node].forward(net, &net->nodes[node]);
    return BCNN_SUCCESS;
}

bcnn_status bcnn_backward_node(bcnn_net *net, int node) {
    if (node < 0 || node >= net->num_nodes || !net->nodes[node].backward) return BCNN_INVALID_PARAMETER;
    bcnn_hip_context *hc = hctx(net);
    bcnn_materialize_data(net, -1);
    bcnn_materialize_gradients(net, -1);
    unsigned char *saved = hc->grad_fill_dead;
    hc->grad_fill_dead = NULL;
    net->nodes[node].backward(net, &net->nodes[node]);
    hc->grad_fill_dead = saved;
    return BCNN_SUCCESS;
}

void bcnn_synchronize(bcnn_net *net) {
    (void)net;
    bcnn_hip_sync();
}

bcnn_status bcnn_set_data_parallel(bcnn_net *net, int rank, int world_size) {
    if (world_size < 1 || rank < 0 || rank >= world_size) return BCNN_INVALID_PARAMETER;
    hctx(net)->dp_rank = rank;
    hctx(net)->dp_world = world_size;
    return BCNN_SUCCESS;
}

static void comm_sync_parameters(bcnn_net *net) {
    bcnn_hip_context *hc = hctx(net);
    if (!hc->comm_active || !hc->param_arena_gpu || hc->arena_size == 0) return;
    bcnn_hip_broadcast(hc->param_arena_gpu, hc->arena_size, 0);
    bcnn_hip_comm_join();
}

bcnn_status bcnn_set_data_parallel_comm(bcnn_net *net, int rank, int world_size, const char *id_path) {
    if (world_size < 1 || rank < 0 || rank >= world_size) return BCNN_INVALID_PARAMETER;
    if (world_size > 1 && (!id_path || !id_path[0])) return BCNN_INVALID_PARAMETER;
    bcnn_hip_context *hc = hctx(net);
    if (hc->comm_active)
        return (bcnn_hip_comm_world() == world_size && bcnn_hip_comm_rank() == rank) ? BCNN_SUCCESS
                                                                                       : BCNN_INVALID_PARAMETER;
    if (bcnn_hip_comm_world() == 0) {
        bcnn_hip_comm_init(rank, world_size, id_path);
    } else {
        if (bcnn_hip_comm_world() != world_size || bcnn_hip_comm_rank() != rank) return BCNN_INVALID_PARAMETER;
        bcnn_hip_comm_retain();
    }
    hc->dp_rank = rank;
    hc->dp_world = world_size;
    hc->comm_active = 1;
    hc->comm_bucket = (size_t)(8u << 20) / sizeof(float);
    bcnn_set_gradient_ready_callback(net, comm_on_ready, hc);
    comm_sync_parameters(net);
    return BCNN_SUCCESS;
}

float *bcnn_get_gradient_arena(bcnn_net *net, size_t *num_floats) {
    if (num_floats) *num_floats = hctx(net)->arena_size;
    return hctx(net)->grad_arena_gpu;
}

float *bcnn_get_parameter_arena(bcnn_net *net, size_t *num_floats) {
    if (num_floats) *num_floats = hctx(net)->arena_size;
    return hctx(net)->param_arena_gpu;
}

static bcnn_learner *learner_of(bcnn_net *net) {
    if (!net->learner) net->learner = (bcnn_learner *)calloc(1, sizeof(bcnn_learner));
    return net->learner;
}

void bcnn_set_learning_rate_policy(bcnn_net *net, bcnn_lr_decay decay_type, float gamma, float scale, float power,
                                   int max_batches, int step) {
    bcnn_learner *ln = learner_of(net);
    ln->decay_type = decay_type; ln->gamma = gamma; ln->scale = scale; ln->power = power;
    ln->max_batches = max_batches; ln->step = step;
}

void bcnn_set_adam_optimizer(bcnn_net *net, float learning_rate, float beta1, float beta2) {
    bcnn_learner *ln = learner_of(net);
    ln->base_learning_rate = ln->learning_rate = learning_rate;
    ln->beta1 = beta1; ln->beta2 = beta2;
    ln->momentum = 0.9f;
// ... 10 lines not shown
```

bcnn_amd/host/bcnn_internal.h:

```cpp
#ifndef BCNN_INTERNAL_H
#define BCNN_INTERNAL_H

#include <stdbool.h>
#include <stdio.h>
#include <stdlib.h>

#include <bcnn/bcnn.h>
#include <bip/bip.h>

#ifdef __cplusplus
extern "C" {
#endif

typedef struct {
    bcnn_log_callback fct;
    bcnn_log_level lvl;
} bcnn_log_context;

void bcnn_log(bcnn_log_context ctx, bcnn_log_level level, const char *fmt, ...);

#define BCNN_CHECK(exp, err) do { if (!(exp)) return (err); } while (0)
#define BCNN_CHECK_AND_LOG(ctx, exp, err, fmt, ...) \
    do { if (!(exp)) { bcnn_log((ctx), BCNN_LOG_ERROR, (fmt), ##__VA_ARGS__); return (err); } } while (0)
#define BCNN_CHECK_STATUS(s) do { bcnn_status ret_ = (s); if (ret_ != BCNN_SUCCESS) return ret_; } while (0)
// ... 79 lines not shown
bcnn_status bcnn_open_dataset(bcnn_loader *iter, struct bcnn_net *net, const char *train_path, const char *train_path_extra,
                              const char *test_path, const char *test_path_extra, bool has_extra);
bcnn_status bcnn_switch_data_handles(struct bcnn_net *net, bcnn_loader *iter);
void bcnn_fill_input_tensor(struct bcnn_net *net, bcnn_loader *iter, char *path_img, int idx);
void bcnn_destroy_data_loader(struct bcnn_net *net);
void bcnn_free_loader_stage(struct bcnn_net *net);
struct bcnn_hip_augment_record;
int bcnn_loader_line_tokens(FILE *f, char ***tok);
void bcnn_loader_free_tokens(char **tok, int n);
void bcnn_loader_crop_origin(struct bcnn_net *net, int wi, int hi, int w, int h, int *x_ul, int *y_ul);
bcnn_status bcnn_loader_crop_to_input(unsigned char *buf, int wi, int hi, int x_ul, int y_ul, unsigned char *img, int w, int h,
                                      int c);
int bcnn_loader_effects_on(const struct bcnn_net *net);
int bcnn_loader_staging(struct bcnn_net *net);
bcnn_status bcnn_loader_stage_sample(struct bcnn_net *net, bcnn_loader *it, int idx,
                                     const struct bcnn_hip_augment_record **record, const int32_t **taps);
void bcnn_loader_staged_records(struct bcnn_net *net, const struct bcnn_hip_augment_record **records, const int32_t **taps);
bcnn_status bcnn_loader_augment_recorded(struct bcnn_net *net, unsigned char *img, int w, int h, int c,
                                         struct bcnn_hip_augment_record *record, int32_t *taps);
void bcnn_loader_fill_record(int flip, int shift, int x_ul, int y_ul, int scale, float scale_factor, int rotate, float theta,
                             int w, int h, struct bcnn_hip_augment_record *record, int32_t *taps);
bcnn_status bcnn_segmentation_init(bcnn_loader *it, struct bcnn_net *net);
bcnn_status bcnn_segmentation_check(struct bcnn_net *net);
bcnn_status bcnn_segmentation_next(bcnn_loader *it, struct bcnn_net *net, int idx);
int bcnn_segmentation_labels(struct bcnn_net *net, bcnn_loader *it, int device_ok);

typedef struct bcnn_hip_context {
    size_t workspace_size;
    float *workspace_gpu;
    float *param_arena_gpu;
    float *grad_arena_gpu;
    size_t arena_size;
    int *param_ids;
    int num_params;
    int arena_members;
    int dp_rank;
    int dp_world;
    int compiled;
    void (*grad_ready_fn)(size_t, size_t, void *);
    void *grad_ready_user;
    size_t *node_grad_first;
    unsigned char *grad_fill_dead;
    int grad_fill_count;
    struct bcnn_hip_sgd_chunk *sgd_chunks_host;
    void *sgd_chunks_gpu;
    int num_sgd_chunks, cap_sgd_chunks;
    int sgd_collecting;
    void *fill_chunks_gpu;
    int num_fill_chunks;
    int comm_active;
    size_t comm_bucket, comm_lo, comm_hi;
    int in_pass;
    int no_side_stream;
    uint64_t dropout_seed;
    int inference_precision;
    int loader_on_device;
    void *loader_stage;
    int loader_decode_on_device;
    int loader_device_decoded;
    int loader_detection_on_device;
    int loader_device_letterboxed;
    int loader_effects;
    int loader_device_labels;
    int detector_training;
    int detect_capacity;
} bcnn_hip_context;

struct bcnn_net {
    int batch_size;
    int num_nodes;
    int num_tensors;
    int num_inputs;
    int *inputs;
    bcnn_mode mode;
    bcnn_log_context log_ctx;
    bcnn_node *nodes;
    bcnn_tensor *tensors;
    bcnn_learner *learner;
    bcnn_loader *data_loader;
    bcnn_data_augmenter *data_aug;
    void *gemm_ctx;
#ifdef BCNN_USE_HIP
    void *hip_ctx;
#endif
    int num_threads;
};

bcnn_status bcnn_net_add_node(bcnn_net *net, bcnn_node node);
bcnn_status bcnn_net_add_tensor(bcnn_net *net, bcnn_tensor tensor);
bcnn_status bcnn_node_add_input(bcnn_net *net, bcnn_node *node, int index);
bcnn_status bcnn_node_add_output(bcnn_net *net, bcnn_node *node, int index);
bcnn_status bcnn_node_new_output(bcnn_net *net, bcnn_node *node, int n, int c, int h, int w, const char *dst_id);
bcnn_status bcnn_node_new_vector_param(bcnn_net *net, bcnn_node *node, int count, int has_grad, const char *src_id,
                                       const char *suffix, float fill, int trainable);

typedef struct tensor_filler {
    int range;
    float value;
    bcnn_filler_type type;
} bcnn_tensor_filler;

void bcnn_tensor_create(bcnn_tensor *t, int n, int c, int h, int w, int has_grad, const char *name, int net_state);
void bcnn_tensor_fill(bcnn_tensor *t, bcnn_tensor_filler filler);
void bcnn_tensor_destroy(bcnn_tensor *t);
void bcnn_tensor_set_shape(bcnn_tensor *t, int n, int c, int h, int w, int has_grad);
bcnn_status bcnn_tensor_allocate_buffer(bcnn_tensor *t, int net_state, size_t size);
bcnn_status bcnn_tensor_allocate(bcnn_tensor *t, int net_state);
bcnn_status bcnn_reserve_device(void **buf, size_t *capacity, size_t elems, size_t elem_size, int may_grow);
void bcnn_tensor_free(bcnn_tensor *t);
int bcnn_tensor_size(const bcnn_tensor *t);
int bcnn_tensor_size3d(const bcnn_tensor *t);
int bcnn_tensor_size2d(const bcnn_tensor *t);

void bcnn_net_register_param(bcnn_net *net, int index);
int bcnn_net_find_tensor(bcnn_net *net, const char *name);

bcnn_status bcnn_loader_next(bcnn_net *net);
void bcnn_convert_img_to_float(const uint8_t *src, int w, int h, int c, float norm_coeff, int swap_to_bgr,
                               float mean_r, float mean_g, float mean_b, float *dst);
// ... 114 lines not shown
} bcnn_maxpool_param;

typedef struct bcnn_activation_param {
    bcnn_activation activation;
#ifdef BCNN_USE_HIP
    float *x_saved_gpu;
    size_t x_saved_capacity;
#endif
} bcnn_activation_param;

typedef struct bcnn_scale_channels_param {
    int same_shape;
} bcnn_scale_channels_param;

typedef struct bcnn_groupnorm_param {
    int num_groups;
    float eps;
#ifdef BCNN_USE_HIP
    float *stats_gpu;
    size_t stats_capacity;
    float *adam_m_gpu, *adam_v_gpu;
#endif
} bcnn_groupnorm_param;

typedef struct bcnn_eltwise_param {
    bcnn_activation activation;
    int stride[2];
    int min_dim[3];
#ifdef BCNN_USE_HIP
    int conv_node;
    int done_forward;
    int deferred;
    int grad_pending;
#endif
} bcnn_eltwise_param;

typedef struct bcnn_fullc_param {
    bcnn_activation activation;
    float *adam_m, *adam_v;
#ifdef BCNN_USE_HIP
    float *adam_m_gpu, *adam_v_gpu;
#endif
} bcnn_fullc_param;

typedef struct bcnn_cost_param {
    float scale;
    bcnn_loss loss;
    bcnn_loss_metric loss_metric;
    float num_constraints;
#ifdef BCNN_USE_HIP
    float *lifted_workspace_gpu;
    size_t lifted_workspace_size;
    void *lifted_record_gpu;
#endif
} bcnn_cost_param;

typedef struct bcnn_upsample_param {
    int size;
} bcnn_upsample_param;

typedef struct bcnn_deconv_param {
    int num, size, stride, pad;
    bcnn_activation activation;
    float *conv_workspace;
    float *adam_m, *adam_v;
#ifdef BCNN_USE_HIP
    float *conv_workspace_gpu;
    size_t workspace_size;
    float *adam_m_gpu, *adam_v_gpu;
#endif
} bcnn_deconv_param;

typedef struct bcnn_dilated_conv_param {
    int num, size, stride, pad, dilation, num_groups;
    bcnn_activation activation;
    int section_bn;
#ifdef BCNN_USE_HIP
    float *conv_workspace_gpu;
    size_t workspace_size;
    float *adam_m_gpu, *adam_v_gpu;
#endif
} bcnn_dilated_conv_param;

typedef struct bcnn_dilated_depthwise_param {
    int size, stride, pad, dilation;
    bcnn_activation activation;
#ifdef BCNN_USE_HIP
    float *workspace_gpu;
    size_t workspace_size;
    float *adam_m_gpu, *adam_v_gpu;
#endif
} bcnn_dilated_depthwise_param;

typedef struct bcnn_lrn_param {
    int local_size;
    float alpha;
    float beta;
    float k;
} bcnn_lrn_param;

typedef struct bcnn_pool2d_param {
    bcnn_pool2d_kind kind;
    int size, stride, pad, ceil_mode, count_include_pad;
#ifdef BCNN_USE_HIP
    int *indexes_gpu;
    size_t indexes_capacity;
#endif
} bcnn_pool2d_param;
// ... 67 lines not shown
void bcnn_release_param_cost_layer(bcnn_node *node);
void bcnn_forward_concat_layer(bcnn_net *net, bcnn_node *node);
void bcnn_backward_concat_layer(bcnn_net *net, bcnn_node *node);
void bcnn_forward_upsample_layer(bcnn_net *net, bcnn_node *node);
void bcnn_backward_upsample_layer(bcnn_net *net, bcnn_node *node);
void bcnn_forward_yolo_layer(bcnn_net *net, bcnn_node *node);
void bcnn_backward_yolo_layer(bcnn_net *net, bcnn_node *node);
void bcnn_release_param_yolo_layer(bcnn_node *node);
int bcnn_yolo_heads_trainable(bcnn_net *net);
int bcnn_yolo_refresh_costs(bcnn_net *net);
bcnn_status bcnn_yolo_detections_batch_worker(bcnn_net *net, const int *widths, const int *heights, int netw, int neth,
                                              float thresh, int relative, int record_cap, int nms_cap,
                                              bcnn_output_detection **dets, int *num_dets, int *passes);
void bcnn_forward_deconv_layer(bcnn_net *net, bcnn_node *node);
void bcnn_backward_deconv_layer(bcnn_net *net, bcnn_node *node);
void bcnn_update_deconv_layer(bcnn_net *net, bcnn_node *node);
void bcnn_release_param_deconv_layer(bcnn_node *node);
void bcnn_forward_dilated_conv_layer(bcnn_net *net, bcnn_node *node);
void bcnn_backward_dilated_conv_layer(bcnn_net *net, bcnn_node *node);
void bcnn_update_dilated_conv_layer(bcnn_net *net, bcnn_node *node);
void bcnn_release_param_dilated_conv_layer(bcnn_node *node);
void bcnn_forward_dilated_depthwise_layer(bcnn_net *net, bcnn_node *node);
void bcnn_backward_dilated_depthwise_layer(bcnn_net *net, bcnn_node *node);
void bcnn_update_dilated_depthwise_layer(bcnn_net *net, bcnn_node *node);
void bcnn_release_param_dilated_depthwise_layer(bcnn_node *node);
void bcnn_forward_lrn_layer(bcnn_net *net, bcnn_node *node);
void bcnn_backward_lrn_layer(bcnn_net *net, bcnn_node *node);
void bcnn_release_param_lrn_layer(bcnn_node *node);
void bcnn_forward_dropout_layer(bcnn_net *net, bcnn_node *node);
void bcnn_backward_dropout_layer(bcnn_net *net, bcnn_node *node);
void bcnn_release_param_dropout_layer(bcnn_node *node);
uint64_t bcnn_dropout_key(uint64_t seed, int node, int rank);
void bcnn_forward_scale_channels_layer(bcnn_net *net, bcnn_node *node);
void bcnn_backward_scale_channels_layer(bcnn_net *net, bcnn_node *node);
void bcnn_forward_groupnorm_layer(bcnn_net *net, bcnn_node *node);
void bcnn_backward_groupnorm_layer(bcnn_net *net, bcnn_node *node);
void bcnn_update_groupnorm_layer(bcnn_net *net, bcnn_node *node);
void bcnn_release_param_groupnorm_layer(bcnn_node *node);
void bcnn_release_param_activation_layer(bcnn_node *node);
void bcnn_forward_pool2d_layer(bcnn_net *net, bcnn_node *node);
void bcnn_backward_pool2d_layer(bcnn_net *net, bcnn_node *node);
void bcnn_release_param_pool2d_layer(bcnn_node *node);
int bcnn_pool2d_out_extents(const bcnn_pool2d_param *p, int h, int w, int *out_h, int *out_w);
void bcnn_forward_interp_layer(bcnn_net *net, bcnn_node *node);
void bcnn_backward_interp_layer(bcnn_net *net, bcnn_node *node);
int bcnn_interp_out_extents(const bcnn_interp_param *p, int h, int w, int *out_h, int *out_w);
void bcnn_forward_softmax_loss_layer(bcnn_net *net, bcnn_node *node);
void bcnn_backward_softmax_loss_layer(bcnn_net *net, bcnn_node *node);
void bcnn_release_param_softmax_loss_layer(bcnn_node *node);
float bcnn_softmax_loss_read_loss(bcnn_net *net, bcnn_node *node);

void bcnn_link_depthwise_batchnorm(bcnn_net *net);
void bcnn_link_conv_eltwise(bcnn_net *net);
void bcnn_link_conv_maxpool(bcnn_net *net);
void bcnn_link_conv_depthwise(bcnn_net *net);
void bcnn_link_batchnorm_conv(bcnn_net *net);
int bcnn_jpeg_read_batch(int num_images, const uint8_t *const *buffers, const size_t *lengths, const bip_jpeg_info *infos,
                         int16_t *const *coeff, int num_threads);
struct bcnn_hip_jpeg_frame;
void bcnn_jpeg_frame_from_info(const bip_jpeg_info *info, struct bcnn_hip_jpeg_frame *f);
int bcnn_jpeg_read_batch_each(int num_images, const uint8_t *const *buffers, const size_t *lengths,
                              const bip_jpeg_info *infos, int16_t *const *coeff, int num_threads, int *status);
void bcnn_materialize_data(bcnn_net *net, int tensor);
void bcnn_materialize_gradients(bcnn_net *net, int tensor);
void bcnn_drop_pending_gradients(bcnn_net *net);
void bcnn_prepack_conv_weights(bcnn_net *net, int data_gradient);
int bcnn_grad_sole_writer(bcnn_net *net, int tensor);
void bcnn_node_sgd_step(bcnn_net *net, bcnn_tensor *weights, bcnn_tensor *biases);
void bcnn_node_optim_step(bcnn_net *net, bcnn_tensor *weights, bcnn_tensor *biases, float **adam_m_gpu,
                          float **adam_v_gpu);

#ifdef __cplusplus
}
#endif
#endif
```

bcnn_amd/host/bcnn_layers_hot.c:

```c
#include <math.h>
#include <string.h>

#include "bcnn_internal.h"
#include "../../include/bcnn_hip.h"

static bcnn_hip_context *hctx(bcnn_net *net) { return (bcnn_hip_context *)net->hip_ctx; }

static bcnn_status attach_source(bcnn_net *net, bcnn_node *node, const char *src_id, const char *what) {
    if (net->num_nodes == 0) return bcnn_node_add_input(net, node, 0);
    const int idx = bcnn_net_find_tensor(net, src_id);
    BCNN_CHECK_AND_LOG(net->log_ctx, idx >= 0, BCNN_INVALID_PARAMETER, "%s layer: invalid input node name %s\n",
                       what, src_id);
    return bcnn_node_add_input(net, node, idx);
}

bcnn_status bcnn_node_new_vector_param(bcnn_net *net, bcnn_node *node, int count, int has_grad, const char *src_id,
                                       const char *suffix, float fill, int trainable) {
    char name[256];
    snprintf(name, sizeof(name), "%s_%s", src_id, suffix);
    bcnn_tensor t = {0};
    bcnn_tensor_create(&t, 1, 1, 1, count, has_grad, name, net->mode);
    if (fill != 0.0f) {
        bcnn_tensor_filler f = {.value = fill, .type = BCNN_FILLER_FIXED};
        bcnn_tensor_fill(&t, f);
// ... 195 lines not shown
                                     p->saved_mean.grad_data_gpu, p->saved_variance.grad_data_gpu, (int)p->activation);
        bcnn_hip_conv_backward_bn_done(xin, io.w->data_gpu, io.y->grad_data_gpu, io.x->grad_data_gpu,
                                       io.w->grad_data_gpu, io.x->n, io.x->c, io.x->h, io.x->w, p->num, p->size, p->stride,
                                       p->pad, p->num_groups, p->conv_workspace_gpu, hctx(net)->workspace_size);
        return;
    }
    if (hctx(net)->in_pass == 2 && p->elt_node >= 0 && ((bcnn_eltwise_param *)net->nodes[p->elt_node].param)->deferred) {
        bcnn_node *en = &net->nodes[p->elt_node];
        bcnn_eltwise_param *ep = (bcnn_eltwise_param *)en->param;
        bcnn_tensor *r = &net->tensors[en->src[1]], *out = &net->tensors[en->dst[0]];
        ep->deferred = 0;
        ep->grad_pending = 1;
        bcnn_hip_conv_backward_residual(xin, io.w->data_gpu, io.b->data_gpu, io.y->grad_data_gpu, io.x->grad_data_gpu,
                                        io.w->grad_data_gpu, io.b->grad_data_gpu, io.x->n, io.x->c, io.x->h, io.x->w,
                                        p->num, p->size, p->stride, p->pad, p->num_groups, io.scales->data_gpu,
                                        io.scales->grad_data_gpu, p->saved_mean.data_gpu, p->saved_variance.data_gpu,
                                        p->saved_mean.grad_data_gpu, p->saved_variance.grad_data_gpu, p->bn_workspace_gpu,
                                        p->conv_workspace_gpu, hctx(net)->workspace_size, out->data_gpu,
                                        out->grad_data_gpu, (int)ep->activation, r->data_gpu, r->grad_data_gpu,
                                        (size_t)ep->min_dim[0] * out->h * out->w);
        return;
    }
    const int own_splits = hctx(net)->in_pass == 2 ? p->insums_splits : 0;
    p->insums_splits = 0;
    const int to_bn = hctx(net)->in_pass == 2 && p->bnsums_node >= 0 && io.x->grad_data_gpu;
    if (to_bn || own_splits > 0) {
        bcnn_node *bn = to_bn ? &net->nodes[p->bnsums_node] : NULL;
        bcnn_batchnorm_param *bp = bn ? (bcnn_batchnorm_param *)bn->param : NULL;
        const int splits = bcnn_hip_conv_backward_presummed(
            xin, io.w->data_gpu, p->out_rewritten ? NULL : io.b->data_gpu, io.y->data_gpu, io.y->grad_data_gpu, io.x->grad_data_gpu,
            io.w->grad_data_gpu, io.b->grad_data_gpu, io.x->n, io.x->c, io.x->h, io.x->w, p->num, p->size, p->stride, p->pad,
            p->num_groups, (int)p->activation, io.slopes ? io.slopes->data_gpu : NULL,
            io.slopes ? io.slopes->grad_data_gpu : NULL, p->batch_norm, io.scales ? io.scales->data_gpu : NULL,
            io.scales ? io.scales->grad_data_gpu : NULL, p->saved_mean.data_gpu, p->saved_variance.data_gpu,
            p->saved_mean.grad_data_gpu, p->saved_variance.grad_data_gpu, p->x_norm_gpu, p->bn_workspace_gpu,
            p->conv_workspace_gpu, hctx(net)->workspace_size, own_splits > 0 ? p->insums_gpu : NULL, own_splits,
            bn ? net->tensors[bn->src[0]].data_gpu : NULL, bp ? bp->saved_mean.data_gpu : NULL, bp ? bp->bsums_gpu : NULL,
            bp ? bp->bsums_floats : 0);
        if (bp) bp->bsums_splits = splits;
        return;
    }
    bcnn_hip_conv_backward(xin, io.w->data_gpu, p->out_rewritten ? NULL : io.b->data_gpu ,
                           io.y->data_gpu, io.y->grad_data_gpu,
                           io.x->grad_data_gpu , io.w->grad_data_gpu,
                           io.b->grad_data_gpu, io.x->n, io.x->c, io.x->h, io.x->w, p->num, p->size, p->stride,
                           p->pad, p->num_groups, (int)p->activation, io.slopes ? io.slopes->data_gpu : NULL,
                           io.slopes ? io.slopes->grad_data_gpu : NULL, p->batch_norm,
                           io.scales ? io.scales->data_gpu : NULL, io.scales ? io.scales->grad_data_gpu : NULL,
                           p->saved_mean.data_gpu, p->saved_variance.data_gpu, p->saved_mean.grad_data_gpu,
                           p->saved_variance.grad_data_gpu, p->x_norm_gpu, p->bn_workspace_gpu,
                           p->conv_workspace_gpu, hctx(net)->workspace_size);
}

void bcnn_prepack_conv_weights(bcnn_net *net, int data_gradient) {
    int n = 0;
    if (BCNN_EXP_ENV("BCNN_NO_PREPACK")) return;
    if (net->num_nodes < 1) return;
    const int none = !data_gradient && bcnn_bf16_inference(net);
    bcnn_hip_conv_desc *d = (bcnn_hip_conv_desc *)malloc((size_t)net->num_nodes * sizeof(*d));
    if (!d) return;
    for (int i = 0; i < net->num_nodes; ++i) {
        bcnn_node *node = &net->nodes[i];
        if (node->type != BCNN_LAYER_CONV2D || none) continue;
        const bcnn_conv_param *p = (const bcnn_conv_param *)node->param;
        const bcnn_tensor *x = &net->tensors[node->src[0]], *w = &net->tensors[node->src[1]];
        if (!w->data_gpu || (data_gradient && !x->grad_data_gpu)) continue;
        if (!data_gradient && net->mode == BCNN_MODE_TRAIN && p->fold_bn >= 0) continue;
        d[n].w_d = w->data_gpu;
        d[n].n = x->n; d[n].c = x->c; d[n].h = x->h; d[n].w = x->w;
        d[n].f = p->num; d[n].k = p->size; d[n].stride = p->stride; d[n].pad = p->pad; d[n].groups = p->num_groups;
        ++n;
    }
    bcnn_hip_conv_prepack(d, n, data_gradient);
    free(d);
}

void bcnn_update_conv_layer(bcnn_net *net, bcnn_node *node) {
    bcnn_conv_param *p = (bcnn_conv_param *)node->param;
    bcnn_node_optim_step(net, &net->tensors[node->src[1]], &net->tensors[node->src[2]], &p->adam_m_gpu, &p->adam_v_gpu);
}

void bcnn_release_param_conv_layer(bcnn_node *node) {
    bcnn_conv_param *p = (bcnn_conv_param *)node->param;
    bcnn_tensor_destroy(&p->saved_mean);
    bcnn_tensor_destroy(&p->saved_variance);
    bcnn_hip_free(p->bn_workspace_gpu);
    bcnn_hip_free(p->insums_gpu);
    bcnn_hip_free(p->x_norm_gpu);
    bcnn_hip_free(p->adam_m_gpu);
    bcnn_hip_free(p->adam_v_gpu);
}

bcnn_status bcnn_add_depthwise_conv_layer(bcnn_net *net, int size, int stride, int pad, int batch_norm,
                                          bcnn_filler_type init, bcnn_activation activation, const char *src_id,
                                          const char *dst_id) {
    (void)batch_norm;
    bcnn_node node = {0};
    BCNN_REFUSE_INPUT_ACTIVATION(net, activation, "Depthwise convolution");
    BCNN_CHECK_STATUS(attach_source(net, &node, src_id, "Depthwise convolution"));
    const bcnn_tensor s = net->tensors[node.src[0]];
    char name[256];
    snprintf(name, sizeof(name), "%s_w", src_id);
    bcnn_tensor weights = {0};
    bcnn_tensor_create(&weights, 1, 1, 1, s.c * size * size, 1, name, net->mode);
    bcnn_tensor_filler wf = {.range = size * size * s.c, .type = init};
    bcnn_tensor_fill(&weights, wf);
    BCNN_CHECK_STATUS(bcnn_net_add_tensor(net, weights));
    BCNN_CHECK_STATUS(bcnn_node_add_input(net, &node, net->num_tensors - 1));
    bcnn_net_register_param(net, net->num_tensors - 1);
    BCNN_CHECK_STATUS(bcnn_node_new_vector_param(net, &node, s.c, 1, src_id, "b", 0.0f, 1));
    node.type = BCNN_LAYER_DEPTHWISE_CONV2D;
    node.param_size = sizeof(bcnn_depthwise_conv_param);
    bcnn_depthwise_conv_param *param = (bcnn_depthwise_conv_param *)calloc(1, node.param_size);
    node.param = param;
    param->activation = activation; param->size = size; param->stride = stride; param->pad = pad;
    param->bn_node = -1;
    param->conv_node = -1;
    node.forward = bcnn_forward_depthwise_conv_layer;
    node.backward = bcnn_backward_depthwise_conv_layer;
    node.update = bcnn_update_depthwise_conv_layer;
    node.release_param = bcnn_release_param_depthwise_conv_layer;
    const int oh = (s.h + 2 * pad - size) / stride + 1, ow = (s.w + 2 * pad - size) / stride + 1;
    BCNN_CHECK_STATUS(add_output(net, &node, s.n, s.c, oh, ow, dst_id));
    BCNN_CHECK_STATUS(bcnn_net_add_node(net, node));
    BCNN_INFO(net->log_ctx, "[DepthwiseConv2D] %-8s (%4d x%4d x%4d) -> %-8s (%4d x%4d x%4d) %d x %d / %d\n", src_id,
              s.w, s.h, s.c, dst_id, ow, oh, s.c, size, size, stride);
// ... 681 lines not shown
```

bcnn_amd/host/bcnn_layers_next.c:

```c
#include <float.h>
#include <math.h>
#include <string.h>

#include "bcnn_internal.h"
#include "../../include/bcnn_hip.h"

static int imin(int a, int b) { return a < b ? a : b; }
static int imax(int a, int b) { return a > b ? a : b; }

bcnn_status bcnn_node_new_output(bcnn_net *net, bcnn_node *node, int n, int c, int h, int w, const char *dst_id) {
    bcnn_tensor t = {0};
    bcnn_tensor_set_shape(&t, n, c, h, w, 1);
    BCNN_CHECK_STATUS(bcnn_tensor_allocate(&t, net->mode));
    t.name = (char *)malloc(strlen(dst_id) + 1);
    strcpy(t.name, dst_id);
    BCNN_CHECK_STATUS(bcnn_net_add_tensor(net, t));
    return bcnn_node_add_output(net, node, net->num_tensors - 1);
}

static bcnn_hip_context *hctx(bcnn_net *net) { return (bcnn_hip_context *)net->hip_ctx; }

bcnn_status bcnn_add_eltwise_layer(bcnn_net *net, bcnn_activation activation, const char *src_id1,
                                   const char *src_id2, const char *dst_id) {
    bcnn_node node = {0};
// ... 70 lines not shown
                              y->w, b->c, b->h, b->w, p->min_dim[0], p->min_dim[1], p->min_dim[2]);
    }
}

bcnn_status bcnn_add_fullc_layer(bcnn_net *net, int output_size, bcnn_filler_type init, bcnn_activation activation,
                                 int quantize, const char *src_id, const char *dst_id) {
    (void)quantize;
    bcnn_node node = {0};
    BCNN_REFUSE_INPUT_ACTIVATION(net, activation, "Full-connected");
    if (net->num_nodes > 0) {
        const int idx = bcnn_net_find_tensor(net, src_id);
        BCNN_CHECK_AND_LOG(net->log_ctx, idx >= 0, BCNN_INVALID_PARAMETER,
                           "Full-connected layer: invalid input node name %s\n", src_id);
        bcnn_node_add_input(net, &node, idx);
    } else {
        bcnn_node_add_input(net, &node, 0);
    }
    const bcnn_tensor s = net->tensors[node.src[0]];
    char name[256];
    snprintf(name, sizeof(name), "%s_w", src_id);
    bcnn_tensor weights = {0};
    bcnn_tensor_create(&weights, output_size, s.c, s.h, s.w, 1, name, net->mode);
    bcnn_tensor_filler wf = {.range = bcnn_tensor_size3d(&s), .type = init};
    bcnn_tensor_fill(&weights, wf);
    BCNN_CHECK_STATUS(bcnn_net_add_tensor(net, weights));
    BCNN_CHECK_STATUS(bcnn_node_add_input(net, &node, net->num_tensors - 1));
    bcnn_net_register_param(net, net->num_tensors - 1);
    snprintf(name, sizeof(name), "%s_b", src_id);
    bcnn_tensor biases = {0};
    bcnn_tensor_create(&biases, 1, 1, 1, output_size, 1, name, net->mode);
    BCNN_CHECK_STATUS(bcnn_net_add_tensor(net, biases));
    BCNN_CHECK_STATUS(bcnn_node_add_input(net, &node, net->num_tensors - 1));
    bcnn_net_register_param(net, net->num_tensors - 1);
    BCNN_CHECK_STATUS(bcnn_node_new_output(net, &node, s.n, output_size, 1, 1, dst_id));
    node.type = BCNN_LAYER_FULL_CONNECTED;
    node.param_size = sizeof(bcnn_fullc_param);
    bcnn_fullc_param *param = (bcnn_fullc_param *)calloc(1, node.param_size);
    node.param = param;
    param->activation = activation;
    node.forward = bcnn_forward_fullc_layer;
    node.backward = bcnn_backward_fullc_layer;
    node.update = bcnn_update_fullc_layer;
    node.release_param = bcnn_release_param_fullc_layer;
    BCNN_CHECK_STATUS(bcnn_net_add_node(net, node));
    BCNN_INFO(net->log_ctx, "[Dense] %-8s (%4d x%4d x%4d) -> %-8s (%d)\n", src_id, s.w, s.h, s.c, dst_id, output_size);
    return BCNN_SUCCESS;
}

void bcnn_forward_fullc_layer(bcnn_net *net, bcnn_node *node) {
    bcnn_fullc_param *p = (bcnn_fullc_param *)node->param;
    bcnn_tensor *x = &net->tensors[node->src[0]], *w = &net->tensors[node->src[1]];
    bcnn_tensor *b = &net->tensors[node->src[2]], *y = &net->tensors[node->dst[0]];
    const int B = y->n, S = bcnn_tensor_size3d(x), P = y->c;
    bcnn_hip_gemm(0, 1, B, P, S, 1.0f, x->data_gpu, S, w->data_gpu, S, 0.0f, y->data_gpu, P);
    bcnn_hip_add_rowvec(y->data_gpu, b->data_gpu, B, P);
    bcnn_hip_activation_forward(y->data_gpu, (size_t)B * P, (int)p->activation, NULL, 1, P);
}

void bcnn_backward_fullc_layer(bcnn_net *net, bcnn_node *node) {
    bcnn_fullc_param *p = (bcnn_fullc_param *)node->param;
    bcnn_tensor *x = &net->tensors[node->src[0]], *w = &net->tensors[node->src[1]];
    bcnn_tensor *b = &net->tensors[node->src[2]], *y = &net->tensors[node->dst[0]];
    const int B = y->n, S = bcnn_tensor_size3d(x), P = y->c;
    bcnn_hip_activation_backward(y->data_gpu, y->grad_data_gpu, (size_t)B * P, (int)p->activation, NULL, NULL, 1, P);
    bcnn_hip_grad_bias(b->grad_data_gpu, y->grad_data_gpu, B, P, 1);
    bcnn_hip_gemm(1, 0, P, S, B, 1.0f, y->grad_data_gpu, P, x->data_gpu, S, 1.0f, w->grad_data_gpu, S);
    if (x->grad_data_gpu)
        bcnn_hip_gemm(0, 0, B, S, P, 1.0f, y->grad_data_gpu, P, w->data_gpu, S, 1.0f, x->grad_data_gpu, S);
}

void bcnn_update_fullc_layer(bcnn_net *net, bcnn_node *node) {
    bcnn_fullc_param *p = (bcnn_fullc_param *)node->param;
    bcnn_node_optim_step(net, &net->tensors[node->src[1]], &net->tensors[node->src[2]], &p->adam_m_gpu, &p->adam_v_gpu);
}

void bcnn_release_param_fullc_layer(bcnn_node *node) {
    bcnn_fullc_param *p = (bcnn_fullc_param *)node->param;
    bcnn_hip_free(p->adam_m_gpu);
    bcnn_hip_free(p->adam_v_gpu);
}

bcnn_status bcnn_add_softmax_layer(bcnn_net *net, const char *src_id, const char *dst_id) {
    bcnn_node node = {0};
    if (net->num_nodes > 0) {
        const int idx = bcnn_net_find_tensor(net, src_id);
        BCNN_CHECK_AND_LOG(net->log_ctx, idx >= 0, BCNN_INVALID_PARAMETER, "Softmax layer: invalid input node name %s\n", src_id);
        bcnn_node_add_input(net, &node, idx);
    } else {
        bcnn_node_add_input(net, &node, 0);
    }
    const bcnn_tensor s = net->tensors[node.src[0]];
    BCNN_CHECK_STATUS(bcnn_node_new_output(net, &node, s.n, s.c, s.h, s.w, dst_id));
    node.type = BCNN_LAYER_SOFTMAX;
    node.forward = bcnn_forward_softmax_layer;
    node.backward = bcnn_backward_softmax_layer;
    BCNN_CHECK_STATUS(bcnn_net_add_node(net, node));
    BCNN_INFO(net->log_ctx, "[Softmax] %-8s -> %-8s (%4d x%4d x%4d)\n", src_id, dst_id, s.w, s.h, s.c);
    return BCNN_SUCCESS;
}

void bcnn_forward_softmax_layer(bcnn_net *net, bcnn_node *node) {
    bcnn_tensor *x = &net->tensors[node->src[0]], *y = &net->tensors[node->dst[0]];
    bcnn_hip_softmax_forward(x->data_gpu, y->data_gpu, x->n, x->c, x->h * x->w);
}

void bcnn_backward_softmax_layer(bcnn_net *net, bcnn_node *node) {
    bcnn_tensor *x = &net->tensors[node->src[0]], *y = &net->tensors[node->dst[0]];
    if (x->grad_data_gpu) bcnn_hip_axpy((size_t)bcnn_tensor_size(x), 1.0f, y->grad_data_gpu, x->grad_data_gpu);
}

bcnn_status bcnn_add_cost_layer(bcnn_net *net, bcnn_loss loss, bcnn_loss_metric loss_metric, float scale,
                                const char *src_id, const char *label_id, const char *dst_id) {
    (void)label_id;
    bcnn_node node = {0};
    BCNN_CHECK_AND_LOG(net->log_ctx, net->num_nodes >= 1, BCNN_INVALID_PARAMETER,
                       "Cost layer can't be the first layer of the network\n");
    BCNN_CHECK_AND_LOG(net->log_ctx, loss == BCNN_LOSS_EUCLIDEAN || loss == BCNN_LOSS_LIFTED_STRUCT, BCNN_INVALID_PARAMETER,
                       "Cost layer: unknown loss %d\n", (int)loss);
    const int idx = bcnn_net_find_tensor(net, src_id);
    BCNN_CHECK_AND_LOG(net->log_ctx, idx >= 0, BCNN_INVALID_PARAMETER, "Cost layer: invalid input node name %s\n", src_id);
    BCNN_CHECK_AND_LOG(net->log_ctx,
                       loss != BCNN_LOSS_LIFTED_STRUCT || (net->tensors[idx].h == 1 && net->tensors[idx].w == 1),
                       BCNN_INVALID_PARAMETER,
                       "Cost layer: the lifted-structure loss needs a [n][c][1][1] embedding, %s is %d x %d x %d\n", src_id,
                       net->tensors[idx].w, net->tensors[idx].h, net->tensors[idx].c);
    bcnn_node_add_input(net, &node, idx);
    node.type = BCNN_LAYER_COST;
    node.param_size = sizeof(bcnn_cost_param);
    bcnn_cost_param *param = (bcnn_cost_param *)calloc(1, node.param_size);
    node.param = param;
    param->scale = scale; param->loss = loss; param->loss_metric = loss_metric;
    node.forward = bcnn_forward_cost_layer;
    node.backward = bcnn_backward_cost_layer;
    node.release_param = bcnn_release_param_cost_layer;
    const bcnn_tensor s = net->tensors[idx];
    bcnn_tensor_set_shape(&net->tensors[1], s.n, s.c, s.h, s.w, 0);
    BCNN_CHECK_STATUS(bcnn_tensor_allocate(&net->tensors[1], net->mode));
    bcnn_node_add_input(net, &node, 1);
    BCNN_CHECK_STATUS(bcnn_node_new_output(net, &node, s.n, s.c, s.h, s.w, dst_id));
    return bcnn_net_add_node(net, node);
}

static float host_metric(const bcnn_cost_param *p, const bcnn_tensor *pred, const bcnn_tensor *label,
                         const bcnn_tensor *dst) {
    const int per = pred->w * pred->h * pred->c, B = pred->n, sz = per * B;
    double acc = 0.0;
    switch (p->loss_metric) {
        case BCNN_METRIC_ERROR_RATE:
            for (int i = 0; i < B; ++i) {
                float pm = FLT_MIN;
                int best = 0;
                for (int j = 0; j < per; ++j)
                    if (pred->data[i * per + j] > pm) { pm = pred->data[i * per + j]; best = j; }
                if (label->data[i * per + best] == 0) acc += 1.0;
            }
            return (float)acc;
        case BCNN_METRIC_LOGLOSS:
            for (int i = 0; i < sz; ++i)
                if (label->data[i] > 0.0f) {
                    float q = pred->data[i];
                    q = q < 1e-8f ? 1e-8f : (q > 1.0f - 1e-8f ? 1.0f - 1e-8f : q);
                    acc += -log(q);
                }
            return (float)acc;
        case BCNN_METRIC_MSE:
        case BCNN_METRIC_SSE:
        case BCNN_METRIC_CRPS:
            for (int i = 0; i < sz; ++i) acc += (double)dst->grad_data[i] * dst->grad_data[i];
            return (float)(p->loss_metric == BCNN_METRIC_MSE ? acc / per : acc);
        case BCNN_METRIC_DICE:
            for (int i = 0; i < B; ++i) {
                int n = 0, d = 0;
                for (int j = 0; j < per; ++j) {
                    n += (int)(label->data[i * per + j] * (pred->data[i * per + j] > 0.5f));
                    d += (int)(label->data[i * per + j] + (pred->data[i * per + j] > 0.5f));
                }
                acc += (2.0f * n + 1.0f) / (d + 1.0f);
            }
            return (float)acc;
    }
    return 0.f;
}

void bcnn_forward_cost_layer(bcnn_net *net, bcnn_node *node) {
    bcnn_cost_param *p = (bcnn_cost_param *)node->param;
    bcnn_tensor *pred = &net->tensors[node->src[0]], *label = &net->tensors[1], *dst = &net->tensors[node->dst[0]];
    if (!label->data) return;
    const size_t sz = (size_t)bcnn_tensor_size(pred);
    if (p->loss == BCNN_LOSS_LIFTED_STRUCT) {
        if (pred->grad_data_gpu && label->data_gpu && net->mode != BCNN_MODE_PREDICT) {
            const size_t need = bcnn_hip_lifted_struct_workspace_size(pred->n, pred->c);
            if (p->lifted_workspace_size < need) {
                bcnn_hip_sync();
                bcnn_hip_free(p->lifted_workspace_gpu);
                p->lifted_workspace_gpu = bcnn_hip_malloc_f32(need);
                p->lifted_workspace_size = need;
            }
            if (!p->lifted_record_gpu) p->lifted_record_gpu = bcnn_hip_malloc_f32(2);
            bcnn_hip_lifted_struct_forward(pred->data_gpu, label->data_gpu, pred->grad_data_gpu, pred->n, pred->c, 1.0f, 1,
                                           (bcnn_hip_lifted_struct_record *)p->lifted_record_gpu,
                                           p->lifted_workspace_gpu);
        }
    } else if (dst->grad_data_gpu) {
        bcnn_hip_copy_f32(sz, pred->data_gpu, dst->grad_data_gpu);
        bcnn_hip_axpy(sz, -1.0f, label->data_gpu, dst->grad_data_gpu);
    }
    if (net->mode == BCNN_MODE_PREDICT) return;
    static int host_loop = -1;
    if (host_loop < 0) host_loop = BCNN_EXP_ENV("BCNN_HOST_COST_METRIC") != NULL;
    if (host_loop || !label->data_gpu || !dst->grad_data_gpu) {
        if (dst->grad_data_gpu) bcnn_hip_memcpy_d2h(dst->grad_data, dst->grad_data_gpu, sz * sizeof(float));
        bcnn_hip_memcpy_d2h(pred->data, pred->data_gpu, sz * sizeof(float));
        dst->data[0] = host_metric(p, pred, label, dst);
        bcnn_hip_memcpy_h2d(dst->data_gpu, dst->data, sizeof(float));
        return;
    }
    bcnn_hip_cost_metric((int)p->loss_metric, pred->data_gpu, label->data_gpu, dst->grad_data_gpu, pred->n,
                         pred->w * pred->h * pred->c, dst->data_gpu);
    bcnn_hip_memcpy_d2h(dst->data, dst->data_gpu, sizeof(float));
}

void bcnn_backward_cost_layer(bcnn_net *net, bcnn_node *node) {
    bcnn_cost_param *p = (bcnn_cost_param *)node->param;
    bcnn_tensor *pred = &net->tensors[node->src[0]], *dst = &net->tensors[node->dst[0]];
    if (p->loss == BCNN_LOSS_LIFTED_STRUCT) {
        if (pred->grad_data_gpu && p->lifted_record_gpu)
            bcnn_hip_lifted_struct_backward(pred->grad_data_gpu, pred->n, pred->c, p->scale,
                                            (const bcnn_hip_lifted_struct_record *)p->lifted_record_gpu);
        return;
    }
    if (pred->grad_data_gpu)
        bcnn_hip_axpy((size_t)bcnn_tensor_size(pred), p->scale, dst->grad_data_gpu, pred->grad_data_gpu);
}

void bcnn_release_param_cost_layer(bcnn_node *node) {
    bcnn_cost_param *p = (bcnn_cost_param *)node->param;
    bcnn_hip_free(p->lifted_workspace_gpu);
    bcnn_hip_free(p->lifted_record_gpu);
}

bcnn_status bcnn_get_lifted_struct_loss(bcnn_net *net, float *loss, int *num_constraints) {
    if (!net) return BCNN_INVALID_PARAMETER;
    for (int i = net->num_nodes - 1; i >= 0; --i) {
        if (net->nodes[i].type != BCNN_LAYER_COST) continue;
        bcnn_cost_param *p = (bcnn_cost_param *)net->nodes[i].param;
        if (p->loss != BCNN_LOSS_LIFTED_STRUCT) continue;
        bcnn_hip_lifted_struct_record rec = {0.f, 0};
        if (p->lifted_record_gpu) bcnn_hip_memcpy_d2h(&rec, p->lifted_record_gpu, sizeof(rec));
        p->num_constraints = (float)rec.num_constraints;
        if (loss) *loss = rec.loss;
        if (num_constraints) *num_constraints = rec.num_constraints;
        return BCNN_SUCCESS;
    }
    return BCNN_INVALID_PARAMETER;
}
```

bcnn_amd/host/bcnn_weights_io.c:

```c
#include <math.h>
#include <stdint.h>
#include <stdio.h>
#include <string.h>

#include "bcnn_internal.h"
#include "bcnn_hip.h"

static const char kMagic[4] = {0x42, 0x43, 0x4E, 0x4E};

static void pull(bcnn_tensor *t, int count) {
    if (t->data && t->data_gpu) bcnn_hip_memcpy_d2h(t->data, t->data_gpu, (size_t)count * sizeof(float));
}
static void push(bcnn_tensor *t, int count) {
    if (t->data && t->data_gpu) bcnn_hip_memcpy_h2d(t->data_gpu, t->data, (size_t)count * sizeof(float));
}
static int put(FILE *fp, bcnn_tensor *t, int count) {
    pull(t, count);
    return fwrite(t->data, sizeof(float), (size_t)count, fp) == (size_t)count;
}

bcnn_status bcnn_save_weights(bcnn_net *net, const char *filename) {
    FILE *fp = filename ? fopen(filename, "wb") : NULL;
    BCNN_CHECK_AND_LOG(net->log_ctx, fp, BCNN_INVALID_PARAMETER, "Could not open model file %s\n",
                       filename ? filename : "(null)");
// ... 86 lines not shown
}

static bcnn_status load_batchnorm(bcnn_net *net, bcnn_node *nd, FILE *fp, int format) {
    bcnn_tensor *m = &net->tensors[nd->src[1]], *v = &net->tensors[nd->src[2]], *s = &net->tensors[nd->src[3]],
                *b = &net->tensors[nd->src[4]];
    const int c = net->tensors[nd->dst[0]].c;
    if (format == 1) READ_OR_FAIL(net, fp, s, c, "scales");
    READ_OR_FAIL(net, fp, m, c, "means");
    READ_OR_FAIL(net, fp, v, c, "variances");
    if (format == 0) {
        READ_OR_FAIL(net, fp, s, c, "scales");
        READ_OR_FAIL(net, fp, b, c, "biases");
    }
    if (net->mode == BCNN_MODE_PREDICT) fold_batchnorm(m, v, s, b, c);
    push(m, c); push(v, c); push(s, c); push(b, c);
    return BCNN_SUCCESS;
}

static bcnn_status load_groupnorm(bcnn_net *net, bcnn_node *nd, FILE *fp, int format) {
    if (format != 0) return BCNN_SUCCESS;
    bcnn_tensor *s = &net->tensors[nd->src[1]], *b = &net->tensors[nd->src[2]];
    const int c = net->tensors[nd->dst[0]].c;
    READ_OR_FAIL(net, fp, b, c, "group-norm biases");
    READ_OR_FAIL(net, fp, s, c, "group-norm scales");
    push(s, c); push(b, c);
    return BCNN_SUCCESS;
}

static void transpose_inplace(float *a, int rows, int cols) {
    float *t = (float *)calloc((size_t)rows * cols, sizeof(float));
    if (!t) return;
    for (int x = 0; x < rows; ++x)
        for (int y = 0; y < cols; ++y) t[(size_t)y * rows + x] = a[(size_t)x * cols + y];
    memcpy(a, t, (size_t)rows * cols * sizeof(float));
    free(t);
}

static bcnn_status load_fullc(bcnn_net *net, bcnn_node *nd, FILE *fp, int need_transpose) {
    bcnn_tensor *w = &net->tensors[nd->src[1]], *b = &net->tensors[nd->src[2]];
    const int w_sz = bcnn_tensor_size(w), b_sz = bcnn_tensor_size(b);
    READ_OR_FAIL(net, fp, b, b_sz, "biases");
    READ_OR_FAIL(net, fp, w, w_sz, "weights");
    if (need_transpose) {
        const bcnn_tensor *x = &net->tensors[nd->src[0]], *y = &net->tensors[nd->dst[0]];
        transpose_inplace(w->data, x->c * x->h * x->w, y->c * y->h * y->w);
    }
    push(w, w_sz); push(b, b_sz);
    return BCNN_SUCCESS;
}

bcnn_status bcnn_load_weights(bcnn_net *net, const char *filename) {
    BCNN_CHECK_AND_LOG(net->log_ctx, filename, BCNN_INVALID_PARAMETER, "Can not open file %s\n", "(null)");
    const int format = model_format(filename);
    for (int i = 0; format == 1 && i < net->num_nodes; ++i)
        BCNN_CHECK_AND_LOG(net->log_ctx,
                           net->nodes[i].type != BCNN_LAYER_DILATED_CONV2D ||
                               !((const bcnn_dilated_conv_param *)net->nodes[i].param)->section_bn,
                           BCNN_INVALID_MODEL,
                           "Node %d is a dilated convolution whose section has batch-norm: Darknet .weights files are not "
                           "supported for it, use the native model format\n", i);
    FILE *fp = fopen(filename, "rb");
    BCNN_CHECK_AND_LOG(net->log_ctx, fp, BCNN_INVALID_PARAMETER, "Can not open file %s\n", filename);
    int need_transpose = 0;
    if (format == 0) {
        char magic[4] = {0, 0, 0, 0};
        uint32_t ver[3] = {0, 0, 0};
        size_t nr = fread(magic, 1, 4, fp);
        nr += fread(ver, sizeof(uint32_t), 3, fp);
        if (nr != 7 || memcmp(magic, kMagic, 4) != 0) {
            bcnn_log(net->log_ctx, BCNN_LOG_ERROR, "Invalid format for model file %s\n", filename);
            fclose(fp);
            return BCNN_INVALID_MODEL;
        }
        BCNN_INFO(net->log_ctx, "BCNN version %d.%d.%d used for model %s\n", (int)ver[0], (int)ver[1], (int)ver[2],
                  filename);
    } else if (format == 1) {
        int hdr[3] = {0, 0, 0};
        size_t nr = fread(hdr, sizeof(int), 3, fp);
        uint64_t seen = 0;
        if ((hdr[0] * 10 + hdr[1]) >= 2 && hdr[0] < 1000 && hdr[1] < 1000) {
            nr += fread(&seen, sizeof(uint64_t), 1, fp);
        } else {
            int iseen = 0;
            nr += fread(&iseen, sizeof(int), 1, fp);
            seen = (uint64_t)iseen;
        }
        (void)nr;
        BCNN_INFO(net->log_ctx, "Darknet version %d.%d seen %lu\n", hdr[0], hdr[1], (unsigned long)seen);
        need_transpose = (hdr[0] > 1000) || (hdr[1] > 1000);
    } else {
        bcnn_log(net->log_ctx, BCNN_LOG_ERROR, "Model file %s format is not yet supported\n", filename);
        fclose(fp);
        return BCNN_INVALID_MODEL;
    }
    bcnn_status st = BCNN_SUCCESS;
    for (int i = 0; st == BCNN_SUCCESS && i < net->num_nodes; ++i) {
        bcnn_node *nd = &net->nodes[i];
        if (nd->type == BCNN_LAYER_CONV2D || nd->type == BCNN_LAYER_TRANSPOSE_CONV2D ||
            nd->type == BCNN_LAYER_DILATED_CONV2D || nd->type == BCNN_LAYER_DEPTHWISE_CONV2D ||
            nd->type == BCNN_LAYER_DILATED_DEPTHWISE_CONV2D) {
            st = load_conv(net, nd, fp, format);
        } else if (nd->type == BCNN_LAYER_ACTIVATION) {
            if (((bcnn_activation_param *)nd->param)->activation == BCNN_ACT_PRELU && format == 0) {
                bcnn_tensor *w = &net->tensors[nd->src[1]];
                size_t nr = fread(w->data, sizeof(float), (size_t)bcnn_tensor_size(w), fp);
                if (nr != (size_t)bcnn_tensor_size(w)) {
// ... 22 lines not shown
```

include/bcnn_hip.h:

```cpp
#ifndef BCNN_HIP_H
#define BCNN_HIP_H

#include <stddef.h>
#include <stdint.h>

#ifdef __cplusplus
extern "C" {
#endif

enum {
    BCNN_HIP_ACT_NONE = 0, BCNN_HIP_ACT_TANH, BCNN_HIP_ACT_RELU, BCNN_HIP_ACT_RAMP,
    BCNN_HIP_ACT_SOFTPLUS, BCNN_HIP_ACT_LRELU, BCNN_HIP_ACT_ABS, BCNN_HIP_ACT_CLAMP,
    BCNN_HIP_ACT_PRELU, BCNN_HIP_ACT_LOGISTIC,
    BCNN_HIP_ACT_RELU6, BCNN_HIP_ACT_HARD_SIGMOID, BCNN_HIP_ACT_HARD_SWISH, BCNN_HIP_ACT_SWISH, BCNN_HIP_ACT_MISH
};
enum { BCNN_HIP_MODE_PREDICT = 0, BCNN_HIP_MODE_TRAIN = 1, BCNN_HIP_MODE_VALID = 2 };

int bcnn_hip_device_count(void);
void bcnn_hip_set_device(int id);
int bcnn_hip_get_device(void);
const char *bcnn_hip_device_name(void);
float *bcnn_hip_malloc_f32(size_t n);
int *bcnn_hip_malloc_i32(size_t n);
void bcnn_hip_free(void *p_d);
void bcnn_hip_memcpy_h2d(void *dst_d, const void *src_h, size_t bytes);
void bcnn_hip_memcpy_d2h(void *dst_h, const void *src_d, size_t bytes);
void bcnn_hip_memcpy_d2d(void *dst_d, const void *src_d, size_t bytes);
void bcnn_hip_fill_f32(float *x_d, size_t n, float value);
void bcnn_hip_sync(void);
void *bcnn_hip_stream_create(void);
void bcnn_hip_stream_destroy(void *stream);
void bcnn_hip_set_stream(void *stream);
void *bcnn_hip_get_stream(void);
void *bcnn_hip_event_create(void);
void bcnn_hip_event_destroy(void *ev);
void bcnn_hip_event_record(void *ev);
void bcnn_hip_event_sync(void *ev);
float bcnn_hip_event_elapsed_ms(void *start, void *stop);

void bcnn_hip_profile_enable(int on);
void bcnn_hip_profile_reset(void);
int bcnn_hip_profile_num_classes(void);
const char *bcnn_hip_profile_class_name(int cls);
void bcnn_hip_profile_read(int cls, double *ms, long long *launches, double *flops, double *bytes);
double bcnn_hip_profile_read_useful_flops(int cls);

int bcnn_hip_conv_side_stream_mode(int mode);
void bcnn_hip_conv_side_join(void);

void bcnn_hip_trace_enable(int on);
size_t bcnn_hip_trace_read(char *buf, size_t cap);

void bcnn_hip_axpy(size_t n, float a, const float *x_d, float *y_d);
void bcnn_hip_scal(size_t n, float a, float *x_d);
void bcnn_hip_copy_f32(size_t n, const float *x_d, float *y_d);
void bcnn_hip_add_bias(float *y_d, const float *bias_d, int n, int c, int hw);
void bcnn_hip_grad_bias(float *dbias_d, const float *g_d, int n, int c, int hw);
void bcnn_hip_scales(float *y_d, const float *scales_d, int n, int c, int hw);
void bcnn_hip_grad_scales(const float *x_norm_d, const float *g_d, int n, int c, int hw,
                          float *dscales_d);

void bcnn_hip_gemm(int trans_a, int trans_b, int m, int n, int k, float alpha, const float *a_d,
                   int lda, const float *b_d, int ldb, float beta, float *c_d, int ldc);
void bcnn_hip_im2col(const float *im_d, int channels, int height, int width, int ksize, int pad,
                     int stride, float *col_d);
void bcnn_hip_col2im(const float *col_d, int channels, int height, int width, int ksize, int pad,
                     int stride, float *im_d);

void bcnn_hip_activation_forward(float *x_d, size_t size, int act, const float *slopes_d,
                                 int spatial, int channels);
void bcnn_hip_activation_backward(const float *x_d, float *dx_d, size_t size, int act,
                                  const float *slopes_d, float *dslopes_d, int spatial, int channels);
void bcnn_hip_activation_forward_keep(float *x_d, float *x_saved_d, size_t size, int act);
void bcnn_hip_activation_backward_from_input(const float *x_saved_d, float *dx_d, size_t size, int act);

void bcnn_hip_batchnorm_forward(const float *x_d, float *y_d, float *run_mean_d, float *run_var_d,
                                const float *scales_d, const float *bias_d, float *saved_mean_d,
                                float *saved_var_d, float *x_norm_d, float *workspace_d, int n, int c,
                                int hw, int mode, int act);
void bcnn_hip_batchnorm_backward(float *dy_d, float *dx_d, const float *y_d, int act,
                                 const float *scales_d, float *dscales_d, float *dbias_d,
                                 const float *saved_mean_d, const float *saved_var_d, float *dmean_d,
                                 float *dvar_d, const float *x_norm_d, const float *workspace_d, int n,
                                 int c, int hw);

size_t bcnn_hip_conv_workspace_size(int n, int c, int h, int w, int f, int k, int stride, int pad,
                                    int groups);
void bcnn_hip_conv_forward(const float *x_d, const float *w_d, const float *bias_d, float *y_d, int n,
                           int c, int h, int w, int f, int k, int stride, int pad, int groups, int act,
                           const float *slopes_d,
                           int batch_norm, float *run_mean_d, float *run_var_d, const float *scales_d,
                           float *saved_mean_d, float *saved_var_d, float *x_norm_d,
                           float *bn_workspace_d, int mode);
void bcnn_hip_conv_backward(const float *x_d, const float *w_d, const float *bias_d, const float *y_d,
                            float *dy_d, float *dx_d, float *dw_d, float *dbias_d, int n, int c, int h, int w, int f,
                            int k, int stride, int pad, int groups, int act, const float *slopes_d,
                            float *dslopes_d, int batch_norm, const float *scales_d, float *dscales_d,
                            const float *saved_mean_d, const float *saved_var_d, float *dmean_d,
                            float *dvar_d, const float *x_norm_d, const float *bn_workspace_d,
                            float *workspace_d, size_t workspace_elems);
int bcnn_hip_conv_forward_bf16(const float *x_d, const float *w_d, const float *bias_d, float *y_d, int n, int c, int h,
                               int w, int f, int k, int stride, int pad, int groups, int act, const float *slopes_d,
                               int batch_norm, float *run_mean_d, float *run_var_d, const float *scales_d,
                               float *saved_mean_d, float *saved_var_d, float *x_norm_d, float *bn_workspace_d,
                               int mode);

int bcnn_hip_conv_residual_fusable(int batch_norm, int act, int res_act, int mode, const float *bn_workspace_d,
                                   const float *res_d, const float *res_out_d);
void bcnn_hip_conv_forward_residual(const float *x_d, const float *w_d, const float *bias_d, int n, int c, int h, int w,
                                    int f, int k, int stride, int pad, int groups, float *run_mean_d, float *run_var_d,
                                    const float *scales_d, float *saved_mean_d, float *saved_var_d,
                                    float *bn_workspace_d, const float *res_d, size_t res_count, int res_act,
                                    float *res_out_d);
void bcnn_hip_conv_backward_residual(const float *x_d, const float *w_d, const float *bias_d, float *dy_d, float *dx_d,
                                     float *dw_d, float *dbias_d, int n, int c, int h, int w, int f, int k, int stride,
                                     int pad, int groups, const float *scales_d, float *dscales_d,
                                     const float *saved_mean_d, const float *saved_var_d, float *dmean_d, float *dvar_d,
                                     const float *bn_workspace_d, float *workspace_d, size_t workspace_elems,
                                     const float *res_out_d, const float *dres_out_d, int res_act, const float *res_d,
                                     float *dres_d, size_t res_count);
void bcnn_hip_batchnorm_apply(const float *x_d, float *y_d, const float *scales_d, const float *bias_d,
                              const float *saved_mean_d, const float *saved_var_d, int n, int c, int hw, int act);

typedef struct {
    const float *w_d;
    int n, c, h, w, f, k, stride, pad, groups;
} bcnn_hip_conv_desc;
void bcnn_hip_conv_prepack(const bcnn_hip_conv_desc *layers, int count, int data_gradient);
void bcnn_hip_conv_prepack_reset(void);
void bcnn_hip_conv_prepack_discard(void);

void bcnn_hip_maxpool_forward(const float *x_d, float *y_d, int *indexes_d, int n, int c, int h, int w,
                              int out_h, int out_w, int size, int stride);
void bcnn_hip_maxpool_backward(const float *dy_d, const int *indexes_d, float *dx_d, int n, int c,
                               int h, int w, int out_h, int out_w, int size, int stride, int overwrite);
size_t bcnn_hip_conv_bnsums_size(int n, int c, int h, int w);
int bcnn_hip_conv_backward_bnsums(const float *x_d, const float *w_d, const float *bias_d, const float *y_d, float *dy_d,
                                  float *dx_d, float *dw_d, float *dbias_d, int n, int c, int h, int w, int f, int k,
                                  int stride, int pad, int groups, int act, const float *slopes_d, float *dslopes_d,
                                  int batch_norm, const float *scales_d, float *dscales_d, const float *saved_mean_d,
                                  const float *saved_var_d, float *dmean_d, float *dvar_d, const float *x_norm_d,
                                  const float *bn_workspace_d, float *workspace_d, size_t workspace_elems,
                                  const float *prev_y_d, const float *prev_mean_d, float *sums_d, size_t sums_floats);
size_t bcnn_hip_depthwise_insums_size(int n, int c, int h, int w, int k, int stride, int pad);
int bcnn_hip_depthwise_backward_bnin_sums(const float *x_raw_d, const float *w_d, const float *y_d, float *dy_d, float *dx_d,
                                          float *dw_d, float *dbias_d, int n, int c, int h, int w, int k, int stride, int pad,
                                          int act, int overwrite, const float *bn_mean_d, const float *bn_var_d,
                                          const float *bn_scales_d, const float *bn_dmean_d, const float *bn_dvar_d,
                                          const float *in_mean_d, const float *in_var_d, const float *in_scale_d,
                                          const float *in_bias_d, int in_act, float *in_sums_d, size_t in_sums_floats);
int bcnn_hip_conv_backward_presummed(const float *x_d, const float *w_d, const float *bias_d, const float *y_d, float *dy_d,
                                     float *dx_d, float *dw_d, float *dbias_d, int n, int c, int h, int w, int f, int k,
                                     int stride, int pad, int groups, int act, const float *slopes_d, float *dslopes_d,
                                     int batch_norm, const float *scales_d, float *dscales_d, const float *saved_mean_d,
                                     const float *saved_var_d, float *dmean_d, float *dvar_d, const float *x_norm_d,
                                     const float *bn_workspace_d, float *workspace_d, size_t workspace_elems,
                                     const float *own_sums_d, int own_splits, const float *prev_y_d,
                                     const float *prev_mean_d, float *prev_sums_d, size_t prev_sums_floats);
void bcnn_hip_batchnorm_backward_finalize(const float *sums_d, int splits, const float *scales_d, float *dscales_d,
                                          float *dbias_d, const float *saved_var_d, float *dmean_d, float *dvar_d, int c);

void bcnn_hip_conv_forward_stats_only(const float *x_d, const float *w_d, const float *bias_d, int n, int c, int h, int w,
                                      int f, int k, int stride, int pad, int groups, float *run_mean_d, float *run_var_d,
                                      const float *scales_d, float *saved_mean_d, float *saved_var_d,
                                      float *bn_workspace_d);
int bcnn_hip_maxpool_bn_fusable(int n, int c, int h, int w, int out_h, int out_w, int size, int stride, int act,
                                const float *x_d);
void bcnn_hip_maxpool_forward_bn(const float *x_d, float *y_d, int *indexes_d, int n, int c, int h, int w, int out_h,
                                 int out_w, int size, int stride, const float *scales_d, const float *bias_d,
                                 const float *saved_mean_d, const float *saved_var_d, int act);
void bcnn_hip_maxpool_forward_bn_keep(const float *x_d, float *y_d, int *indexes_d, int n, int c, int h, int w, int out_h,
                                      int out_w, int size, int stride, const float *scales_d, const float *bias_d,
                                      const float *saved_mean_d, const float *saved_var_d, int act, float *raw_at_max_d);
int bcnn_hip_maxpool_bn_backward_fusable(int n, int c, int h, int w, int out_h, int out_w, int size, int stride, int act,
                                         const float *raw_d, const float *dpool_d, const int *indexes_d, const float *dx_d);
void bcnn_hip_maxpool_bn_backward(const float *dpool_d, const int *indexes_d, const float *raw_at_max_d, const float *raw_d,
                                  float *dx_d, int n, int c, int h, int w, int out_h, int out_w, int size, int stride,
                                  const float *scales_d, float *dscales_d, const float *bias_d, float *dbias_d,
                                  const float *saved_mean_d, const float *saved_var_d, float *dmean_d, float *dvar_d, int act);
void bcnn_hip_conv_backward_bn_done(const float *x_d, const float *w_d, float *dy_d, float *dx_d, float *dw_d, int n, int c,
                                    int h, int w, int f, int k, int stride, int pad, int groups, float *workspace_d,
                                    size_t workspace_elems);
void bcnn_hip_avgpool_forward(const float *x_d, float *y_d, int n, int c, int h, int w);
// ... 98 lines not shown

int bcnn_hip_depthwise_bnin_fusable(int n, int c, int h, int w, int k, int stride, int pad, int act, int in_act);
int bcnn_hip_depthwise_forward_bnin(const float *x_raw_d, const float *w_d, const float *bias_d, float *y_d, int n, int c,
                                    int h, int w, int k, int stride, int pad, int act, float *stats_d, size_t stats_floats,
                                    const float *in_mean_d, const float *in_var_d, const float *in_scale_d,
                                    const float *in_bias_d, int in_act);
void bcnn_hip_depthwise_backward_bnin(const float *x_raw_d, const float *w_d, const float *y_d, float *dy_d, float *dx_d,
                                      float *dw_d, float *dbias_d, int n, int c, int h, int w, int k, int stride, int pad,
                                      int act, int overwrite, const float *in_mean_d, const float *in_var_d,
                                      const float *in_scale_d, const float *in_bias_d, int in_act);
void bcnn_hip_depthwise_backward_bn_bnin(const float *x_raw_d, const float *w_d, const float *y_d, const float *dz_d,
                                         float *dx_d, float *dw_d, float *dbias_d, int n, int c, int h, int w, int k,
                                         int stride, int pad, int act, int overwrite, const float *bn_mean_d,
                                         const float *bn_var_d, const float *bn_scales_d, const float *bn_dmean_d,
                                         const float *bn_dvar_d, const float *in_mean_d, const float *in_var_d,
                                         const float *in_scale_d, const float *in_bias_d, int in_act);

void bcnn_hip_sgd_update(float *w_d, float *b_d, float *dw_d, float *db_d, size_t w_size,
                         size_t b_size, int batch_size, float learning_rate, float momentum,
                         float decay);

void bcnn_hip_adam_update(float *w_d, float *b_d, float *dw_d, float *db_d, float *adam_m_d,
                          float *adam_v_d, size_t w_size, size_t b_size, int batch_size, int iter,
                          float beta1, float beta2, float learning_rate, float momentum, float decay);

#define BCNN_HIP_SGD_CHUNK 2048
typedef struct bcnn_hip_sgd_chunk {
    float *w_d;
    float *g_d;
    unsigned int count;
    unsigned int use_decay;
} bcnn_hip_sgd_chunk;
void bcnn_hip_sgd_update_chunks(const bcnn_hip_sgd_chunk *chunks_d, int num_chunks, int batch_size,
                                float learning_rate, float momentum, float decay);

#define BCNN_HIP_FILL_CHUNK 16384
typedef struct bcnn_hip_fill_chunk {
    float *p_d;
    unsigned int count;
    unsigned int reserved;
} bcnn_hip_fill_chunk;
void bcnn_hip_zero_chunks(const bcnn_hip_fill_chunk *chunks_d, int num_chunks);

void bcnn_hip_eltwise_forward(const float *a_d, const float *b_d, float *y_d, size_t n, size_t b_count, int act);
void bcnn_hip_eltwise_backward(const float *y_d, float *dy_d, float *da_d, float *db_d, size_t n, size_t b_count,
                               int act, int overwrite_a);
void bcnn_hip_cost_metric(int metric, const float *pred_d, const float *label_d, const float *grad_d, int batch,
                          int per, float *out_d);
void bcnn_hip_axpy_strided(int num_batches, float a, const float *x_d, float *y_d, int stride_y,
                           int stride_x, int x_c, int x_h, int x_w, int y_c, int y_h, int y_w, int min_c,
                           int min_h, int min_w);
void bcnn_hip_add_rowvec(float *y_d, const float *v_d, int rows, int cols);
void bcnn_hip_softmax_forward(const float *x_d, float *y_d, int n, int c, int hw);

void bcnn_hip_concat_forward(int num_src, const float *const *src_d, const int *src_size3d, float *dst_d,
                             int dst_size3d, int n);
void bcnn_hip_concat_backward(int num_src, float *const *src_grad_d, const int *src_size3d, const float *dst_grad_d,
                              int dst_size3d, int n);
void bcnn_hip_upsample_forward(const float *x_d, float *y_d, int n, int c, int h, int w, int size);
void bcnn_hip_upsample_backward(float *dx_d, const float *dy_d, int n, int c, int h, int w, int size);
void bcnn_hip_yolo_activate(const float *x_d, float *y_d, int n, int num, int coords, int classes, int hw);

#define BCNN_HIP_YOLO_MAX_HEADS 8
#define BCNN_HIP_YOLO_MAX_ANCHORS 16
#define BCNN_HIP_YOLO_RECORD_HEAD 6
typedef struct bcnn_hip_yolo_head {
    const float *out_d;
    int h, w, num, coords, classes;
    float anchor_w[BCNN_HIP_YOLO_MAX_ANCHORS], anchor_h[BCNN_HIP_YOLO_MAX_ANCHORS];
} bcnn_hip_yolo_head;
int bcnn_hip_yolo_nms_capacity(void);
size_t bcnn_hip_yolo_detect_result_words(int n, int record_cap, int max_classes);
int bcnn_hip_yolo_detect_batch(const bcnn_hip_yolo_head *heads, int num_heads, int n, const int *image_geom, int in_w,
                               int in_h, int netw, int neth, float thresh, int relative, float nms_thresh,
                               int record_cap, int nms_cap, void *result_host);

#define BCNN_HIP_YOLO_TRAIN_MAX_TRUTHS 50
#define BCNN_HIP_YOLO_TRAIN_MAX_TOTAL 32
typedef struct bcnn_hip_yolo_train_head {
    int n, h, w, num, coords, classes, total;
    int in_w, in_h;
    int label_stride;
    int mask[BCNN_HIP_YOLO_MAX_ANCHORS];
    float biases[2 * BCNN_HIP_YOLO_TRAIN_MAX_TOTAL];
} bcnn_hip_yolo_train_head;
typedef struct bcnn_hip_yolo_train_record {
    float cost, avg_iou, avg_cat, avg_obj, avg_anyobj, recall, recall75;
    int count;
} bcnn_hip_yolo_train_record;
size_t bcnn_hip_yolo_train_workspace_size(const bcnn_hip_yolo_train_head *head);
int bcnn_hip_yolo_train_forward(const bcnn_hip_yolo_train_head *head, const float *x_d, const float *label_d, float *y_d,
                                float *grad_d, bcnn_hip_yolo_train_record *record_d, float *workspace_d);

#define BCNN_HIP_IMAGE_FIT_STRETCH 0
#define BCNN_HIP_IMAGE_FIT_LETTERBOX 1
int bcnn_hip_fill_images(float *dst_d, int n, int c, int h, int w, int num_images, const uint8_t *const *images,
                         const int *widths, const int *heights, const int *strides, int fit, float norm_coeff,
                         int swap_to_bgr, float mean_r, float mean_g, float mean_b);

typedef struct bcnn_hip_jpeg_component {
    int h, v;
    int width, height;
    int pitch, rows;
    int blocks_w, blocks_h;
    int idct_w, idct_h;
} bcnn_hip_jpeg_component;
// ... 122 lines not shown
```

Measured before the change: 14140 images/s.

## Overlap loss readback with early dx weight prepack; fuse softmax+cost and FC bias

Replaces the blocking loss device-to-host copy with an async read plus event. Between starting and waiting on that read, the data-gradient conv weight prepack is enqueued early under a token and adopted later, so the host sync no longer leaves the GPU idle before backward. It also fuses softmax with the Euclidean cost and error-rate metric into one kernel, and folds the FC bias add into the gemm split-k finalize. The cost is extra bookkeeping: prepack entries gain an early token and weight-generation tracking, which risks stale packs if weights change between forward and backward.

```diff
diff --git a/bcnn_amd/_lib.py b/bcnn_amd/_lib.py
--- a/bcnn_amd/_lib.py
+++ b/bcnn_amd/_lib.py
@@ -104,6 +104,10 @@
     "bcnn_hip_conv_backward_presummed": (i, [vp] * 8 + [i] * 10 + [vp, vp, i] + [vp] * 8 + [vp, sz] + [vp, i] + [vp, vp, vp, sz]),
     "bcnn_hip_conv_prepack_reset": (None, []),
     "bcnn_hip_conv_prepack_discard": (None, []),
+    "bcnn_hip_read_begin": (None, [vp, sz]),
+    "bcnn_hip_read_end": (None, [vp, sz]),
+    "bcnn_hip_conv_prepack_early": (C.c_ulonglong, [vp, i]),
+    "bcnn_hip_conv_prepack_adopt": (None, [C.c_ulonglong]),
     "bcnn_hip_maxpool_bn_fusable": (i, [i] * 9 + [vp]),
     "bcnn_hip_conv_forward_stats_only": (None, [vp, vp, vp] + [i] * 9 + [vp] * 6),
     "bcnn_hip_maxpool_forward_bn": (None, [vp, vp, vp] + [i] * 8 + [vp] * 4 + [i]),
@@ -117,6 +121,8 @@
     "bcnn_hip_axpy_strided": (None, [i, f, vp, vp] + [i] * 11),
     "bcnn_hip_add_rowvec": (None, [vp, vp, i, i]),
     "bcnn_hip_softmax_forward": (None, [vp, vp, i, i, i]),
+    "bcnn_hip_softmax_cost_forward": (None, [vp, vp, vp, vp, i, i, vp]),
+    "bcnn_hip_gemm_bias": (None, [i, i, i, i, i, f, vp, i, vp, i, f, vp, vp, i]),
     "bcnn_hip_concat_forward": (None, [i, vp, vp, vp, i, i]),
     "bcnn_hip_concat_backward": (None, [i, vp, vp, vp, i, i]),
     "bcnn_hip_upsample_forward": (None, [vp, vp, i, i, i, i, i]),
diff --git a/bcnn_amd/csrc/blas1.hip b/bcnn_amd/csrc/blas1.hip
--- a/bcnn_amd/csrc/blas1.hip
+++ b/bcnn_amd/csrc/blas1.hip
@@ -178,6 +178,7 @@
 
 void bcnn_hip_axpy(size_t n, float a, const float* x, float* y) {
     if (!n) return;
+    trace_kernel("axpy");
     map2_kernel<<<stream_grid(n / 4 + 1, 256), 256, 0, current_stream()>>>(x, y, n, AxpyOp{a});
     KERNEL_CHECK();
 }
@@ -192,6 +193,7 @@
 
 void bcnn_hip_copy_f32(size_t n, const float* x, float* y) {
     if (!n || x == y) return;
+    trace_kernel("copy_f32");
     HIP_CHECK(hipMemcpyAsync(y, x, n * sizeof(float), hipMemcpyDeviceToDevice, current_stream()));
 }
 
diff --git a/bcnn_amd/csrc/common.h b/bcnn_amd/csrc/common.h
--- a/bcnn_amd/csrc/common.h
+++ b/bcnn_amd/csrc/common.h
@@ -64,6 +64,7 @@
     STAGE_AUGMENT,
     STAGE_AUGMENT_LABEL,
     STAGE_LABEL_MAP,
+    STAGE_READ,
     STAGE_SLOTS
 };
 uint8_t* host_stage(StageSlot slot, size_t bytes);
diff --git a/bcnn_amd/csrc/conv.hip b/bcnn_amd/csrc/conv.hip
--- a/bcnn_amd/csrc/conv.hip
+++ b/bcnn_amd/csrc/conv.hip
@@ -65,10 +65,12 @@
     size_t cap, floats;
     unsigned long long epoch;
     bool fresh;
+    unsigned long long early;
 };
 struct PrepackStore {
     std::vector<PrepackEntry> entries;
     unsigned long long epoch = 0;
+    unsigned long long early_tokens = 0;
     int dev = -1;
     void* table_dev[PREPACK_KINDS][2] = {{nullptr, nullptr}, {nullptr, nullptr}};
     size_t table_cap[PREPACK_KINDS][2] = {{0, 0}, {0, 0}};
@@ -79,7 +81,7 @@
 float* prepack_take(const float* w, int kind, int mode, size_t floats) {
     PrepackStore& st = g_prepack;
     for (PrepackEntry& e : st.entries)
-        if (e.w == w && e.kind == kind && e.mode == mode && e.fresh && e.epoch == st.epoch && e.floats == floats) {
+        if (e.w == w && e.kind == kind && e.mode == mode && e.fresh && !e.early && e.epoch == st.epoch && e.floats == floats) {
             e.fresh = false;
             return e.buf;
         }
@@ -105,7 +107,7 @@
     for (PrepackEntry& c : st.entries)
         if (c.w == w && c.kind == kind && c.mode == mode) { e = &c; break; }
     if (!e) {
-        st.entries.push_back(PrepackEntry{w, kind, mode, nullptr, 0, 0, 0, false});
+        st.entries.push_back(PrepackEntry{w, kind, mode, nullptr, 0, 0, 0, false, 0});
         e = &st.entries.back();
     }
     if (e->cap < floats) {
@@ -119,6 +121,7 @@
     e->floats = floats;
     e->epoch = st.epoch;
     e->fresh = true;
+    e->early = 0;
     return e;
 }
 
@@ -377,7 +380,7 @@
 
 extern "C" {
 
-void bcnn_hip_conv_prepack(const bcnn_hip_conv_desc* layers, int count, int data_gradient) {
+static void prepack_batch(const bcnn_hip_conv_desc* layers, int count, int mode, unsigned long long early) {
     PrepackStore& st = g_prepack;
     int dev = 0;
     HIP_CHECK(hipGetDevice(&dev));
@@ -385,9 +388,10 @@
         if (st.dev >= 0) prepack_free_all(st);
         st.dev = dev;
     }
-    ++st.epoch;
-    (void)take_fold();
-    const int mode = data_gradient ? 1 : 0;
+    if (!early) {
+        ++st.epoch;
+        (void)take_fold();
+    }
     std::vector<WinoPackJob> wj;
     std::vector<IgemmPackJob> ij;
     int wmax = 0, imax = 0;
@@ -404,12 +408,14 @@
         size_t floats = 0;
         if (pack.wino && pack.wino(s, mode, &w1, &floats)) {
             PrepackEntry* e = prepack_entry(st, d.w_d, PREPACK_WINO, mode, floats);
+            e->early = early;
             w1.w = d.w_d; w1.u = e->buf;
             if (w1.blocks > wmax) wmax = w1.blocks;
             wj.push_back(w1);
         }
         if (pack.igemm && pack.igemm(s, mode, &i1, &floats)) {
             PrepackEntry* e = prepack_entry(st, d.w_d, PREPACK_IGEMM, mode, floats);
+            e->early = early;
             i1.w = d.w_d; i1.at = e->buf;
             const int blocks = i1.gx * i1.gy * i1.gz;
             if (blocks > imax) imax = blocks;
@@ -418,12 +424,36 @@
     }
     if (!wj.empty()) {
         const void* t = prepack_table(st, PREPACK_WINO, mode, wj.data(), wj.size() * sizeof(WinoPackJob));
+        trace_kernel(mode ? "wino_pack_weights_multi:dx" : "wino_pack_weights_multi:fwd");
         wino_fused_pack_launch((const WinoPackJob*)t, (int)wj.size(), wmax);
     }
     if (!ij.empty()) {
         const void* t = prepack_table(st, PREPACK_IGEMM, mode, ij.data(), ij.size() * sizeof(IgemmPackJob));
+        trace_kernel(mode ? "conv_pack_weights_multi:dx" : "conv_pack_weights_multi:fwd");
         dma_pack_launch((const IgemmPackJob*)t, (int)ij.size(), imax);
     }
+}
+
+void bcnn_hip_conv_prepack(const bcnn_hip_conv_desc* layers, int count, int data_gradient) {
+    prepack_batch(layers, count, data_gradient ? 1 : 0, 0);
+}
+
+unsigned long long bcnn_hip_conv_prepack_early(const bcnn_hip_conv_desc* layers, int count) {
+    const unsigned long long token = ++g_prepack.early_tokens;
+    prepack_batch(layers, count, 1, token);
+    return token;
+}
+
+void bcnn_hip_conv_prepack_adopt(unsigned long long token) {
+    PrepackStore& st = g_prepack;
+    ++st.epoch;
+    (void)take_fold();
+    if (!token) return;
+    for (PrepackEntry& e : st.entries)
+        if (e.early == token && e.fresh) {
+            e.early = 0;
+            e.epoch = st.epoch;
+        }
 }
 
 void bcnn_hip_conv_prepack_discard(void) { ++g_prepack.epoch; }
diff --git a/bcnn_amd/csrc/gemm.hip b/bcnn_amd/csrc/gemm.hip
--- a/bcnn_amd/csrc/gemm.hip
+++ b/bcnn_amd/csrc/gemm.hip
@@ -81,7 +81,8 @@
 }
 
 __global__ __launch_bounds__(256) void gemm_splitk_finalize_kernel(const float* __restrict__ partials, int splits, float* C,
-                                                                   int m, int n, int ldc, float alpha, float beta) {
+                                                                   int m, int n, int ldc, float alpha, float beta,
+                                                                   const float* __restrict__ bias_row) {
     const long long total = (long long)m * n, stride = (long long)gridDim.x * blockDim.x;
     for (long long e = (long long)blockIdx.x * blockDim.x + threadIdx.x; e < total; e += stride) {
         float sum = partials[e];
@@ -89,6 +90,7 @@
         float* cp = C + (e / n) * ldc + (e % n);
         float v = alpha * sum;
         if (beta != 0.0f) v += beta * (*cp);
+        if (bias_row) v = __fadd_rn(v, bias_row[e % n]);
         *cp = v;
     }
 }
@@ -144,16 +146,33 @@
 
 using namespace bcnn_hip;
 
-extern "C" {
-
-void bcnn_hip_gemm(int ta, int tb, int m, int n, int k, float alpha, const float* A, int lda, const float* B,
-                   int ldb, float beta, float* C, int ldc) {
+struct GemmCall {
+    int ta, tb, m, n, k;
+    float alpha;
+    const float* A;
+    int lda;
+    const float* B;
+    int ldb;
+    float beta;
+    float* C;
+    int ldc;
+    const float* bias_row;
+    int force_splits;
+};
+static void gemm_launch(const GemmCall& g) {
+    const int ta = g.ta, tb = g.tb, m = g.m, n = g.n, k = g.k, lda = g.lda, ldb = g.ldb, ldc = g.ldc;
+    const float alpha = g.alpha, beta = g.beta;
+    const float *A = g.A, *B = g.B, *bias_row = g.bias_row;
+    float* C = g.C;
+    const int force_splits = g.force_splits;
     if (m <= 0 || n <= 0) return;
     if (k <= 0 || alpha == 0.0f) {
         if (beta != 1.0f) {
+            trace_kernel("gemm_scale_kernel");
             gemm_scale_kernel<<<stream_grid((size_t)m * n, 256), 256, 0, current_stream()>>>(C, m, n, ldc, beta);
             KERNEL_CHECK();
         }
+        if (bias_row) bcnn_hip_add_rowvec(C, bias_row, m, n);
         return;
     }
     GemmArgs a;
@@ -168,17 +187,34 @@
         if (splits > 32) splits = 32;
         if (splits < 1) splits = 1;
     }
+    if (force_splits > 0) splits = force_splits < ktiles ? force_splits : ktiles;
     a.tiles_per_split = ceil_div(ktiles, splits);
     splits = ceil_div(ktiles, a.tiles_per_split);
     a.partials = splits > 1 ? scratch(SCRATCH_REDUCE, (size_t)splits * m * n) : nullptr;
     dim3 grid((unsigned)ceil_div(n, 64), (unsigned)ceil_div(m, 64), (unsigned)splits);
+    trace_kernel("gemm_kernel");
     gemm_kernel<<<grid, 256, 0, current_stream()>>>(a);
     KERNEL_CHECK();
     if (splits > 1) {
+        trace_kernel(bias_row ? "gemm_splitk_finalize_kernel:bias" : "gemm_splitk_finalize_kernel");
         gemm_splitk_finalize_kernel<<<stream_grid((size_t)m * n, 256), 256, 0, current_stream()>>>(a.partials, splits, C, m, n, ldc,
-                                                                                                alpha, beta);
+                                                                                                alpha, beta, bias_row);
         KERNEL_CHECK();
-    }
+    } else if (bias_row) {
+        bcnn_hip_add_rowvec(C, bias_row, m, n);
+    }
+}
+
+extern "C" {
+
+void bcnn_hip_gemm(int ta, int tb, int m, int n, int k, float alpha, const float* A, int lda, const float* B,
+                   int ldb, float beta, float* C, int ldc) {
+    gemm_launch(GemmCall{ta, tb, m, n, k, alpha, A, lda, B, ldb, beta, C, ldc, nullptr, 0});
+}
+
+void bcnn_hip_gemm_bias(int ta, int tb, int m, int n, int k, float alpha, const float* A, int lda, const float* B, int ldb,
+                        float beta, float* C, const float* bias_row, int force_splits) {
+    gemm_launch(GemmCall{ta, tb, m, n, k, alpha, A, lda, B, ldb, beta, C, n, bias_row, force_splits});
 }
 
 void bcnn_hip_im2col(const float* im, int channels, int height, int width, int ksize, int pad, int stride,
diff --git a/bcnn_amd/csrc/next.hip b/bcnn_amd/csrc/next.hip
--- a/bcnn_amd/csrc/next.hip
+++ b/bcnn_amd/csrc/next.hip
@@ -170,6 +170,53 @@
         partials[blockIdx.x] = t;
     }
 }
+constexpr int kSoftmaxCostWaves = 4, kSoftmaxCostMaxBlocks = 64;
+__global__ __launch_bounds__(256) void softmax_cost_kernel(const float* __restrict__ x, float* __restrict__ y,
+                                                            const float* __restrict__ label, float* __restrict__ grad,
+                                                            int B, int C, double* __restrict__ partials) {
+    __shared__ double red[kSoftmaxCostWaves];
+    const int lane = threadIdx.x & 63, wave = threadIdx.x >> 6;
+    const int nrow = kSoftmaxCostWaves * gridDim.x, row0 = blockIdx.x * kSoftmaxCostWaves + wave;
+    double acc = 0.0;
+    for (int i = row0; i < B; i += nrow) {
+        const float* px = x + (size_t)i * C;
+        const float* pl = label + (size_t)i * C;
+        float* py = y + (size_t)i * C;
+        float* pg = grad + (size_t)i * C;
+        float vmax = -FLT_MAX;
+        for (int c = lane; c < C; c += 64) vmax = fmaxf(vmax, px[c]);
+#pragma unroll
+        for (int o = 32; o > 0; o >>= 1) vmax = fmaxf(vmax, __shfl_xor(vmax, o));
+        double part = 0.0;
+        for (int c = lane; c < C; c += 64) part += (double)(float)exp((double)(px[c] - vmax));
+#pragma unroll
+        for (int o = 32; o > 0; o >>= 1) part += __shfl_xor(part, o);
+        float sum = (float)part;
+        sum = (sum != 0.f) ? vmax + (float)log((double)sum) : vmax - 100.0f;
+        float pm = FLT_MIN;
+        int best = 0;
+        for (int c = lane; c < C; c += 64) {
+            const float p = (float)exp((double)(px[c] - sum));
+            py[c] = p;
+            pg[c] = __fadd_rn(__fmul_rn(pl[c], -1.0f), p);
+            if (p > pm) { pm = p; best = c; }
+        }
+#pragma unroll
+        for (int off = 32; off > 0; off >>= 1) {
+            const float om = __shfl_xor(pm, off);
+            const int ob = __shfl_xor(best, off);
+            if (om > pm || (om == pm && ob < best)) { pm = om; best = ob; }
+        }
+        if (lane == 0 && pl[best] == 0) acc += 1.0;
+    }
+    if (lane == 0) red[wave] = acc;
+    __syncthreads();
+    if (threadIdx.x == 0) {
+        double t = 0.0;
+        for (int w = 0; w < kSoftmaxCostWaves; ++w) t += red[w];
+        partials[blockIdx.x] = t;
+    }
+}
 __global__ void cost_metric_final_kernel(int metric, const double* __restrict__ partials, int n, int per,
                                          float* __restrict__ out) {
     double t = 0.0;
@@ -195,6 +242,7 @@
 void bcnn_hip_add_rowvec(float* y, const float* v, int rows, int cols) {
     const long long total = (long long)rows * cols;
     if (total <= 0) return;
+    trace_kernel("add_rowvec_kernel");
     add_rowvec_kernel<<<stream_grid((size_t)total, 256), 256, 0, current_stream()>>>(y, v, cols, (unsigned)total);
     KERNEL_CHECK();
 }
@@ -202,6 +250,7 @@
 void bcnn_hip_softmax_forward(const float* x, float* y, int n, int c, int hw) {
     const long long total = (long long)n * hw;
     if (total <= 0) return;
+    trace_kernel("softmax_kernel");
     softmax_kernel<<<stream_grid((size_t)total * 64, 256), 256, 0, current_stream()>>>(x, y, c, hw, (unsigned)total);
     KERNEL_CHECK();
 }
@@ -235,17 +284,38 @@
     KERNEL_CHECK();
 }
 
-void bcnn_hip_cost_metric(int metric, const float* pred, const float* label, const float* grad, int batch, int per,
-                          float* out) {
+static int cost_metric_blocks(int batch, int per) {
     const long long sz = (long long)batch * per;
     int blocks = (int)((sz + 8191) / 8192);
     if (blocks > 64) blocks = 64;
     if (blocks < 1) blocks = 1;
+    return blocks;
+}
+
+void bcnn_hip_cost_metric(int metric, const float* pred, const float* label, const float* grad, int batch, int per,
+                          float* out) {
+    const int blocks = cost_metric_blocks(batch, per);
     double* partials = reinterpret_cast<double*>(scratch(SCRATCH_REDUCE, 2 * 64));
+    trace_kernel("cost_metric_kernel");
     cost_metric_kernel<<<blocks, 1024, 0, current_stream()>>>(metric, pred, label, grad, batch, per, partials);
     KERNEL_CHECK();
+    trace_kernel("cost_metric_final_kernel");
     cost_metric_final_kernel<<<1, 1, 0, current_stream()>>>(metric, partials, blocks, per, out);
     KERNEL_CHECK();
 }
 
-}
+void bcnn_hip_softmax_cost_forward(const float* x, float* prob, const float* label, float* grad, int batch, int classes,
+                                   float* out) {
+    if (batch <= 0 || classes <= 0) return;
+    int blocks = ceil_div(batch, kSoftmaxCostWaves);
+    if (blocks > kSoftmaxCostMaxBlocks) blocks = kSoftmaxCostMaxBlocks;
+    double* partials = reinterpret_cast<double*>(scratch(SCRATCH_REDUCE, 2 * kSoftmaxCostMaxBlocks));
+    trace_kernel("softmax_cost_kernel");
+    softmax_cost_kernel<<<blocks, 256, 0, current_stream()>>>(x, prob, label, grad, batch, classes, partials);
+    KERNEL_CHECK();
+    trace_kernel("cost_metric_final_kernel");
+    cost_metric_final_kernel<<<1, 1, 0, current_stream()>>>(0, partials, blocks, classes, out);
+    KERNEL_CHECK();
+}
+
+}
diff --git a/bcnn_amd/csrc/runtime.hip b/bcnn_amd/csrc/runtime.hip
--- a/bcnn_amd/csrc/runtime.hip
+++ b/bcnn_amd/csrc/runtime.hip
@@ -234,8 +234,31 @@
 }
 
 void bcnn_hip_memcpy_d2h(void* dst, const void* src, size_t bytes) {
+    trace_kernel("memcpy_d2h");
     HIP_CHECK(hipMemcpyAsync(dst, src, bytes, hipMemcpyDeviceToHost, current_stream()));
     HIP_CHECK(hipStreamSynchronize(current_stream()));
+}
+
+struct ReadBack { hipEvent_t done = nullptr; bool pending = false; size_t bytes = 0; };
+static thread_local ReadBack g_read[kMaxDevices];
+void bcnn_hip_read_begin(const void* src, size_t bytes) {
+    ReadBack& r = g_read[current_device()];
+    if (r.pending) HIP_CHECK(hipEventSynchronize(r.done));
+    if (!r.done) HIP_CHECK(hipEventCreateWithFlags(&r.done, hipEventDisableTiming));
+    uint8_t* p = host_stage(STAGE_READ, bytes);
+    trace_kernel("memcpy_d2h");
+    HIP_CHECK(hipMemcpyAsync(p, src, bytes, hipMemcpyDeviceToHost, current_stream()));
+    HIP_CHECK(hipEventRecord(r.done, current_stream()));
+    r.pending = true;
+    r.bytes = bytes;
+}
+
+void bcnn_hip_read_end(void* dst, size_t bytes) {
+    ReadBack& r = g_read[current_device()];
+    if (!r.pending || r.bytes < bytes) return;
+    HIP_CHECK(hipEventSynchronize(r.done));
+    r.pending = false;
+    memcpy(dst, g_stage[current_device()][STAGE_READ].p, bytes);
 }
 
 void bcnn_hip_memcpy_d2d(void* dst, const void* src, size_t bytes) {
diff --git a/bcnn_amd/host/bcnn_core.c b/bcnn_amd/host/bcnn_core.c
--- a/bcnn_amd/host/bcnn_core.c
+++ b/bcnn_amd/host/bcnn_core.c
@@ -274,6 +274,7 @@
 int bcnn_get_batch_size(bcnn_net *net) { return net->batch_size; }
 
 void bcnn_set_input_shape(bcnn_net *net, int width, int height, int channels, int batch_size) {
+    BCNN_WEIGHTS_CHANGED(net);
     net->batch_size = batch_size;
     bcnn_tensor_set_shape(&net->tensors[0], batch_size, channels, height, width, 0);
 }
@@ -415,6 +416,7 @@
 
 static void relink_graph(bcnn_net *net) {
     bcnn_hip_context *hc = hctx(net);
+    BCNN_WEIGHTS_CHANGED(net);
     mark_dead_grad_fills(net);
     for (int i = 0; i < net->num_nodes; ++i) {
         if (net->nodes[i].type != BCNN_LAYER_CONV2D) continue;
@@ -429,6 +431,7 @@
     bcnn_link_conv_maxpool(net);
     bcnn_link_conv_depthwise(net);
     bcnn_link_batchnorm_conv(net);
+    bcnn_link_softmax_cost(net);
     if (hc->fill_chunks_gpu) {
         bcnn_hip_sync();
         bcnn_hip_free(hc->fill_chunks_gpu);
@@ -575,6 +578,7 @@
 
 bcnn_status bcnn_set_mode(bcnn_net *net, bcnn_mode mode) {
     if (net->mode == mode) return BCNN_SUCCESS;
+    BCNN_WEIGHTS_CHANGED(net);
     if (mode == BCNN_MODE_TRAIN && !hctx(net)->detector_training)
         for (int i = 0; i < net->num_nodes; ++i)
             BCNN_CHECK_AND_LOG(net->log_ctx, net->nodes[i].type != BCNN_LAYER_YOLOV3, BCNN_INVALID_PARAMETER,
@@ -622,6 +626,7 @@
 
 void bcnn_forward(bcnn_net *net) {
     bcnn_hip_context *hc = hctx(net);
+    hc->early_pack_token = 0;
     if (net->mode == BCNN_MODE_TRAIN) {
         if (hc->num_fill_chunks < 0) build_fill_table(net);
         bcnn_hip_zero_chunks((const bcnn_hip_fill_chunk *)hc->fill_chunks_gpu, hc->num_fill_chunks);
@@ -652,7 +657,11 @@
     bcnn_hip_context *hc = hctx(net);
     size_t ready_from = hc->arena_size;
     if (hc->comm_active) hc->comm_lo = hc->comm_hi = hc->arena_size;
-    bcnn_prepack_conv_weights(net, 1);
+    if (hc->early_pack_token && hc->early_pack_gen == hc->weights_gen && !BCNN_EXP_ENV("BCNN_NO_PREPACK"))
+        bcnn_hip_conv_prepack_adopt(hc->early_pack_token);
+    else
+        bcnn_prepack_conv_weights(net, 1);
+    hc->early_pack_token = 0;
     hc->in_pass = 2;
     const int side_prev = bcnn_hip_conv_side_stream_mode((hc->no_side_stream || BCNN_EXP_ENV("BCNN_NO_SIDE_STREAM")) ? 0 : 2);
     for (int i = net->num_nodes - 1; i >= 0; --i) {
@@ -820,6 +829,7 @@
 
 void bcnn_update(bcnn_net *net) {
     bcnn_hip_context *hc = hctx(net);
+    BCNN_WEIGHTS_CHANGED(net);
     step_learning_rate(net);
     if (net->learner->optimizer == BCNN_OPTIM_ADAM) {
         for (int i = 0; i < net->num_nodes; ++i)
@@ -944,6 +954,7 @@
     bcnn_tensor *t = &net->tensors[index];
     const size_t bytes = (size_t)bcnn_tensor_size(t) * sizeof(float);
     bcnn_materialize_data(net, index);
+    BCNN_WEIGHTS_CHANGED(net);
     if (t->data && t->data_gpu) bcnn_hip_memcpy_h2d(t->data_gpu, t->data, bytes);
     if (with_grad) bcnn_materialize_gradients(net, -1);
     if (with_grad && t->grad_data && t->grad_data_gpu) bcnn_hip_memcpy_h2d(t->grad_data_gpu, t->grad_data, bytes);
@@ -975,6 +986,7 @@
                            strides[b]);
     }
     bcnn_materialize_data(net, tensor_index);
+    BCNN_WEIGHTS_CHANGED(net);
     if (bcnn_hip_fill_images(t->data_gpu, t->n, t->c, t->h, t->w, num_images, images, widths, heights, strides, (int)fit,
                              norm_coeff, swap_to_bgr, mean_r, mean_g, mean_b) != 0)
         BCNN_ERROR(net->log_ctx, BCNN_INVALID_PARAMETER,
@@ -1095,6 +1107,7 @@
 static void comm_sync_parameters(bcnn_net *net) {
     bcnn_hip_context *hc = hctx(net);
     if (!hc->comm_active || !hc->param_arena_gpu || hc->arena_size == 0) return;
+    BCNN_WEIGHTS_CHANGED(net);
     bcnn_hip_broadcast(hc->param_arena_gpu, hc->arena_size, 0);
     bcnn_hip_comm_join();
 }
diff --git a/bcnn_amd/host/bcnn_internal.h b/bcnn_amd/host/bcnn_internal.h
--- a/bcnn_amd/host/bcnn_internal.h
+++ b/bcnn_amd/host/bcnn_internal.h
@@ -155,6 +155,7 @@
     size_t comm_bucket, comm_lo, comm_hi;
     int in_pass;
     int no_side_stream;
+    unsigned long long weights_gen, early_pack_gen, early_pack_token;
     uint64_t dropout_seed;
     int inference_precision;
     int loader_on_device;
@@ -168,6 +169,7 @@
     int detector_training;
     int detect_capacity;
 } bcnn_hip_context;
+#define BCNN_WEIGHTS_CHANGED(net) (++((bcnn_hip_context *)(net)->hip_ctx)->weights_gen)
 
 struct bcnn_net {
     int batch_size;
@@ -388,8 +390,14 @@
     float *lifted_workspace_gpu;
     size_t lifted_workspace_size;
     void *lifted_record_gpu;
+    int softmax_node;
+    int forward_done;
 #endif
 } bcnn_cost_param;
+
+typedef struct bcnn_softmax_param {
+    int cost_node;
+} bcnn_softmax_param;
 
 typedef struct bcnn_upsample_param {
     int size;
@@ -563,6 +571,7 @@
 
 void bcnn_link_depthwise_batchnorm(bcnn_net *net);
 void bcnn_link_conv_eltwise(bcnn_net *net);
+void bcnn_link_softmax_cost(bcnn_net *net);
 void bcnn_link_conv_maxpool(bcnn_net *net);
 void bcnn_link_conv_depthwise(bcnn_net *net);
 void bcnn_link_batchnorm_conv(bcnn_net *net);
@@ -576,6 +585,7 @@
 void bcnn_materialize_gradients(bcnn_net *net, int tensor);
 void bcnn_drop_pending_gradients(bcnn_net *net);
 void bcnn_prepack_conv_weights(bcnn_net *net, int data_gradient);
+void bcnn_prepack_conv_weights_early(bcnn_net *net);
 int bcnn_grad_sole_writer(bcnn_net *net, int tensor);
 void bcnn_node_sgd_step(bcnn_net *net, bcnn_tensor *weights, bcnn_tensor *biases);
 void bcnn_node_optim_step(bcnn_net *net, bcnn_tensor *weights, bcnn_tensor *biases, float **adam_m_gpu,
diff --git a/bcnn_amd/host/bcnn_layers_hot.c b/bcnn_amd/host/bcnn_layers_hot.c
--- a/bcnn_amd/host/bcnn_layers_hot.c
+++ b/bcnn_amd/host/bcnn_layers_hot.c
@@ -271,13 +271,9 @@
                            p->conv_workspace_gpu, hctx(net)->workspace_size);
 }
 
-void bcnn_prepack_conv_weights(bcnn_net *net, int data_gradient) {
+static int prepack_descriptors(bcnn_net *net, int data_gradient, bcnn_hip_conv_desc *d) {
     int n = 0;
-    if (BCNN_EXP_ENV("BCNN_NO_PREPACK")) return;
-    if (net->num_nodes < 1) return;
     const int none = !data_gradient && bcnn_bf16_inference(net);
-    bcnn_hip_conv_desc *d = (bcnn_hip_conv_desc *)malloc((size_t)net->num_nodes * sizeof(*d));
-    if (!d) return;
     for (int i = 0; i < net->num_nodes; ++i) {
         bcnn_node *node = &net->nodes[i];
         if (node->type != BCNN_LAYER_CONV2D || none) continue;
@@ -290,7 +286,28 @@
         d[n].f = p->num; d[n].k = p->size; d[n].stride = p->stride; d[n].pad = p->pad; d[n].groups = p->num_groups;
         ++n;
     }
+    return n;
+}
+
+void bcnn_prepack_conv_weights(bcnn_net *net, int data_gradient) {
+    if (BCNN_EXP_ENV("BCNN_NO_PREPACK")) return;
+    if (net->num_nodes < 1) return;
+    bcnn_hip_conv_desc *d = (bcnn_hip_conv_desc *)malloc((size_t)net->num_nodes * sizeof(*d));
+    if (!d) return;
+    const int n = prepack_descriptors(net, data_gradient, d);
     bcnn_hip_conv_prepack(d, n, data_gradient);
+    free(d);
+}
+
+void bcnn_prepack_conv_weights_early(bcnn_net *net) {
+    bcnn_hip_context *hc = hctx(net);
+    if (net->mode != BCNN_MODE_TRAIN || hc->in_pass != 1 || hc->early_pack_token) return;
+    if (BCNN_EXP_ENV("BCNN_NO_PREPACK") || BCNN_EXP_ENV("BCNN_NO_EARLY_PREPACK")) return;
+    bcnn_hip_conv_desc *d = (bcnn_hip_conv_desc *)malloc((size_t)net->num_nodes * sizeof(*d));
+    if (!d) return;
+    const int n = prepack_descriptors(net, 1, d);
+    hc->early_pack_token = bcnn_hip_conv_prepack_early(d, n);
+    hc->early_pack_gen = hc->weights_gen;
     free(d);
 }
 
diff --git a/bcnn_amd/host/bcnn_layers_next.c b/bcnn_amd/host/bcnn_layers_next.c
--- a/bcnn_amd/host/bcnn_layers_next.c
+++ b/bcnn_amd/host/bcnn_layers_next.c
@@ -146,8 +146,7 @@
     bcnn_tensor *x = &net->tensors[node->src[0]], *w = &net->tensors[node->src[1]];
     bcnn_tensor *b = &net->tensors[node->src[2]], *y = &net->tensors[node->dst[0]];
     const int B = y->n, S = bcnn_tensor_size3d(x), P = y->c;
-    bcnn_hip_gemm(0, 1, B, P, S, 1.0f, x->data_gpu, S, w->data_gpu, S, 0.0f, y->data_gpu, P);
-    bcnn_hip_add_rowvec(y->data_gpu, b->data_gpu, B, P);
+    bcnn_hip_gemm_bias(0, 1, B, P, S, 1.0f, x->data_gpu, S, w->data_gpu, S, 0.0f, y->data_gpu, b->data_gpu, 0);
     bcnn_hip_activation_forward(y->data_gpu, (size_t)B * P, (int)p->activation, NULL, 1, P);
 }
 
@@ -186,6 +185,10 @@
     const bcnn_tensor s = net->tensors[node.src[0]];
     BCNN_CHECK_STATUS(bcnn_node_new_output(net, &node, s.n, s.c, s.h, s.w, dst_id));
     node.type = BCNN_LAYER_SOFTMAX;
+    node.param_size = sizeof(bcnn_softmax_param);
+    bcnn_softmax_param *param = (bcnn_softmax_param *)calloc(1, node.param_size);
+    param->cost_node = -1;
+    node.param = param;
     node.forward = bcnn_forward_softmax_layer;
     node.backward = bcnn_backward_softmax_layer;
     BCNN_CHECK_STATUS(bcnn_net_add_node(net, node));
@@ -193,8 +196,49 @@
     return BCNN_SUCCESS;
 }
 
+void bcnn_link_softmax_cost(bcnn_net *net) {
+    for (int i = 0; i < net->num_nodes; ++i) {
+        bcnn_node *nd = &net->nodes[i];
+        if (nd->type == BCNN_LAYER_SOFTMAX && nd->param) ((bcnn_softmax_param *)nd->param)->cost_node = -1;
+        if (nd->type == BCNN_LAYER_COST) {
+            ((bcnn_cost_param *)nd->param)->softmax_node = -1;
+            ((bcnn_cost_param *)nd->param)->forward_done = 0;
+        }
+    }
+    if (BCNN_EXP_ENV("BCNN_NO_NODE_FUSION") || BCNN_EXP_ENV("BCNN_HOST_COST_METRIC")) return;
+    for (int c = 1; c < net->num_nodes; ++c) {
+        bcnn_node *cn = &net->nodes[c], *sn = &net->nodes[c - 1];
+        if (cn->type != BCNN_LAYER_COST || sn->type != BCNN_LAYER_SOFTMAX || !sn->param) continue;
+        bcnn_cost_param *cp = (bcnn_cost_param *)cn->param;
+        const int t = sn->dst[0];
+        if (cn->src[0] != t || sn->src[0] == t || cp->loss != BCNN_LOSS_EUCLIDEAN || cp->loss_metric != BCNN_METRIC_ERROR_RATE)
+            continue;
+        int writers = 0, consumers = 0;
+        for (int i = 0; i < net->num_nodes; ++i) {
+            for (int k = 0; k < net->nodes[i].num_dst; ++k) writers += net->nodes[i].dst[k] == t;
+            for (int k = 0; k < net->nodes[i].num_src; ++k) consumers += net->nodes[i].src[k] == t;
+        }
+        const bcnn_tensor *y = &net->tensors[t];
+        if (writers != 1 || consumers != 1 || y->h * y->w != 1 || cn->dst[0] == t || cn->dst[0] == sn->src[0]) continue;
+        ((bcnn_softmax_param *)sn->param)->cost_node = c;
+        cp->softmax_node = c - 1;
+    }
+}
+
 void bcnn_forward_softmax_layer(bcnn_net *net, bcnn_node *node) {
     bcnn_tensor *x = &net->tensors[node->src[0]], *y = &net->tensors[node->dst[0]];
+    const bcnn_softmax_param *sp = (const bcnn_softmax_param *)node->param;
+    if (sp && sp->cost_node >= 0 && hctx(net)->in_pass == 1 && net->mode != BCNN_MODE_PREDICT) {
+        bcnn_node *cn = &net->nodes[sp->cost_node];
+        bcnn_tensor *label = &net->tensors[1], *dst = &net->tensors[cn->dst[0]];
+        if (label->data && label->data_gpu && dst->grad_data_gpu && dst->data_gpu &&
+            bcnn_tensor_size(label) == bcnn_tensor_size(y)) {
+            bcnn_hip_softmax_cost_forward(x->data_gpu, y->data_gpu, label->data_gpu, dst->grad_data_gpu, x->n, x->c,
+                                          dst->data_gpu);
+            ((bcnn_cost_param *)cn->param)->forward_done = 1;
+            return;
+        }
+    }
     bcnn_hip_softmax_forward(x->data_gpu, y->data_gpu, x->n, x->c, x->h * x->w);
 }
 
@@ -276,11 +320,22 @@
     return 0.f;
 }
 
+static void read_loss_over_early_packs(bcnn_net *net, bcnn_tensor *dst) {
+    bcnn_hip_read_begin(dst->data_gpu, sizeof(float));
+    bcnn_prepack_conv_weights_early(net);
+    bcnn_hip_read_end(dst->data, sizeof(float));
+}
+
 void bcnn_forward_cost_layer(bcnn_net *net, bcnn_node *node) {
     bcnn_cost_param *p = (bcnn_cost_param *)node->param;
     bcnn_tensor *pred = &net->tensors[node->src[0]], *label = &net->tensors[1], *dst = &net->tensors[node->dst[0]];
     if (!label->data) return;
     const size_t sz = (size_t)bcnn_tensor_size(pred);
+    if (p->forward_done) {
+        p->forward_done = 0;
+        read_loss_over_early_packs(net, dst);
+        return;
+    }
     if (p->loss == BCNN_LOSS_LIFTED_STRUCT) {
         if (pred->grad_data_gpu && label->data_gpu && net->mode != BCNN_MODE_PREDICT) {
             const size_t need = bcnn_hip_lifted_struct_workspace_size(pred->n, pred->c);
@@ -311,7 +366,7 @@
     }
     bcnn_hip_cost_metric((int)p->loss_metric, pred->data_gpu, label->data_gpu, dst->grad_data_gpu, pred->n,
                          pred->w * pred->h * pred->c, dst->data_gpu);
-    bcnn_hip_memcpy_d2h(dst->data, dst->data_gpu, sizeof(float));
+    read_loss_over_early_packs(net, dst);
 }
 
 void bcnn_backward_cost_layer(bcnn_net *net, bcnn_node *node) {
diff --git a/bcnn_amd/host/bcnn_weights_io.c b/bcnn_amd/host/bcnn_weights_io.c
--- a/bcnn_amd/host/bcnn_weights_io.c
+++ b/bcnn_amd/host/bcnn_weights_io.c
@@ -162,6 +162,7 @@
 bcnn_status bcnn_load_weights(bcnn_net *net, const char *filename) {
     BCNN_CHECK_AND_LOG(net->log_ctx, filename, BCNN_INVALID_PARAMETER, "Can not open file %s\n", "(null)");
     const int format = model_format(filename);
+    BCNN_WEIGHTS_CHANGED(net);
     for (int i = 0; format == 1 && i < net->num_nodes; ++i)
         BCNN_CHECK_AND_LOG(net->log_ctx,
                            net->nodes[i].type != BCNN_LAYER_DILATED_CONV2D ||
diff --git a/include/bcnn_hip.h b/include/bcnn_hip.h
--- a/include/bcnn_hip.h
+++ b/include/bcnn_hip.h
@@ -62,6 +62,8 @@
 
 void bcnn_hip_gemm(int trans_a, int trans_b, int m, int n, int k, float alpha, const float *a_d,
                    int lda, const float *b_d, int ldb, float beta, float *c_d, int ldc);
+void bcnn_hip_gemm_bias(int trans_a, int trans_b, int m, int n, int k, float alpha, const float *a_d, int lda,
+                        const float *b_d, int ldb, float beta, float *c_d, const float *bias_row_d, int force_splits);
 void bcnn_hip_im2col(const float *im_d, int channels, int height, int width, int ksize, int pad,
                      int stride, float *col_d);
 void bcnn_hip_col2im(const float *col_d, int channels, int height, int width, int ksize, int pad,
@@ -129,6 +131,10 @@
 void bcnn_hip_conv_prepack(const bcnn_hip_conv_desc *layers, int count, int data_gradient);
 void bcnn_hip_conv_prepack_reset(void);
 void bcnn_hip_conv_prepack_discard(void);
+void bcnn_hip_read_begin(const void *src_d, size_t bytes);
+void bcnn_hip_read_end(void *dst_h, size_t bytes);
+unsigned long long bcnn_hip_conv_prepack_early(const bcnn_hip_conv_desc *layers, int count);
+void bcnn_hip_conv_prepack_adopt(unsigned long long token);
 
 void bcnn_hip_maxpool_forward(const float *x_d, float *y_d, int *indexes_d, int n, int c, int h, int w,
                               int out_h, int out_w, int size, int stride);
@@ -333,6 +339,8 @@
                            int min_h, int min_w);
 void bcnn_hip_add_rowvec(float *y_d, const float *v_d, int rows, int cols);
 void bcnn_hip_softmax_forward(const float *x_d, float *y_d, int n, int c, int hw);
+void bcnn_hip_softmax_cost_forward(const float *x_d, float *prob_d, const float *label_d, float *grad_d, int batch,
+                                   int classes, float *out_d);
 
 void bcnn_hip_concat_forward(int num_src, const float *const *src_d, const int *src_size3d, float *dst_d,
                              int dst_size3d, int n);
```

Measured after the change: 14200 images/s (median of 6 runs). About the same (+0.4%).
